# iwbn/flow-supervisor

Measured on AMD Instinct MI355X. Metric: image-pairs/s fwd+bwd, 12 GRU iters, 436x1024, higher is better.
Workload: dtype f32 (bf16x3 products); 1 GPU; RAFT full, 440x1024 (Sintel 436x1024 padded), 12 GRU iters, 4 pairs/GPU, train step = fwd + sequence loss + bwd + RCCL all-reduce + clip + AdamW; global_batch=4, parallelism=dp1, launch=hipGraph replay of the whole step

## Files before the change

flow_supervisor_amd/_lib.py:

```python
import ctypes
import functools
import os
from ctypes import POINTER, Structure, c_double, c_float, c_int, c_int64, c_void_p

import torch

_HERE = os.path.dirname(os.path.abspath(__file__))
LIB_PATH = os.environ.get("FSRAFT_LIB_PATH") or os.path.join(_HERE, "libfsraft.so")
_lib = None

c_float_p = c_void_p


class ConvDesc(Structure):
    _fields_ = [
        ("src", c_void_p * 3), ("srcC", c_int * 3), ("srcld", c_int * 3), ("nsrc", c_int),
        ("wpk", c_void_p), ("bias", c_void_p), ("wpk_split", c_void_p),
        ("B", c_int), ("H", c_int), ("W", c_int), ("KH", c_int), ("KW", c_int), ("N", c_int),
        ("dst", c_void_p * 3), ("dst_bs", c_int64 * 3), ("dst_ps", c_int64 * 3), ("dst_cs", c_int64 * 3),
        ("dst_n0", c_int * 3), ("dst_acc", c_int * 3), ("ndst", c_int),
        ("relu", c_int), ("alpha", c_float),
        ("epi", c_int),
        ("h", c_void_p), ("ldh", c_int), ("z", c_void_p), ("ldz", c_int),
        ("aux1", c_void_p), ("ld1", c_int), ("aux2", c_void_p), ("ld2", c_int), ("hid", c_int),
        ("pre", c_void_p), ("ldpre", c_int),
        ("rmask", c_void_p * 3), ("ldmask", c_int * 3), ("maskc", c_int * 3),
        ("wpk_frag", c_void_p), ("pad_h1", c_int), ("pad_w1", c_int),
        ("ws", c_void_p), ("ws_floats", c_int64),
    ]


class PackJob(Structure):
    _fields_ = [
        ("w", c_void_p * 3), ("rows", c_int * 3), ("npiece", c_int),
        ("wpk", c_void_p),
        ("cin_full", c_int), ("kh", c_int), ("kw", c_int),
        ("srcC", c_int * 3), ("srcOff", c_int * 3), ("nsrc", c_int),
        ("mode", c_int), ("flags", c_int),
        ("scale", c_float), ("accumulate", c_int),
    ]


_PP = POINTER(c_void_p)
_IP = POINTER(c_int)
_S = c_void_p

SIGNATURES = {
    "fsraft_corr_build": [c_void_p, c_void_p, _PP, c_int, c_int, c_int, c_int, c_int, _S],
    "fsraft_corr_unpool_bwd": [_PP, c_int, c_int, c_int, c_int, _S],
    "fsraft_corr_lookup_fwd": [_PP, c_int, c_void_p, c_int64, c_int64, c_int64, c_void_p, c_int, c_int, c_int, c_int, c_int, _S],
    "fsraft_corr_lookup_bwd": [_PP, c_int, c_void_p, c_int64, c_int64, c_int64, c_void_p, c_int, c_int, c_int, c_int, c_int, _S],
    "fsraft_altcorr_fwd": [c_void_p, c_void_p, c_void_p, c_void_p, c_int, c_int, c_int, c_int, c_int, c_int, c_int, c_int, _S],
    "fsraft_altcorr_bwd": [c_void_p, c_void_p, c_void_p, c_void_p, c_void_p, c_void_p, c_int, c_int, c_int, c_int, c_int, c_int, c_int, c_int, _S],
    "fsraft_upsample_fwd": [c_void_p, c_int64, c_int64, c_int64, c_void_p, c_void_p, c_int, c_int, c_int, _S],
    "fsraft_upsample_bwd": [c_void_p, c_int64, c_int64, c_int64, c_void_p, c_void_p, c_void_p, c_void_p, c_void_p, c_int, c_int, c_int, _S],
    "fsraft_upflow8_fwd": [c_void_p, c_void_p, c_int, c_int, c_int, c_int, _S],
    "fsraft_upflow8_bwd": [c_void_p, c_void_p, c_int, c_int, c_int, c_int, _S],
    "fsraft_conv_ktot": [_IP, c_int, c_int, c_int],
    "fsraft_conv_forward": [POINTER(ConvDesc), _S],
    "fsraft_conv_forward_stats": [POINTER(ConvDesc), c_void_p, c_void_p, c_int, POINTER(c_int), _S],
    "fsraft_conv_wgrad": [c_void_p, c_int, c_int, _PP, _IP, _IP, c_int, c_void_p, c_void_p, c_int, c_int, c_int, c_int, c_int, _S],
    "fsraft_conv_wgrad_multi": [_PP, c_int, c_int, c_int, _PP, _IP, _IP, c_int, c_void_p, c_void_p, c_int, c_int, c_int, c_int, c_int, _S],
    "fsraft_conv_small_fwd": [c_void_p, c_int, c_int, c_void_p, c_void_p, c_void_p, c_int64, c_int64, c_int64, c_int, c_int, c_int, c_int, c_int, c_int, _S],
    "fsraft_conv_small_wgrad": [_PP, _PP, c_int, c_int, c_int, c_int, c_void_p, c_void_p, c_int, c_int, c_int, c_int, c_int, c_int, _S],
    "fsraft_conv_small_dgrad": [c_void_p, c_int, c_void_p, c_void_p, c_int, c_void_p, c_int, c_int, c_int, c_int, c_int, c_int, c_int, c_int, _S],
    "fsraft_pack_conv_weights": [POINTER(PackJob), c_int, _S],
    "fsraft_pack_conv_weight": [c_void_p, c_void_p, c_int, c_int, c_int, c_int, _IP, c_int, c_int, c_int, _S],
    "fsraft_set_rec_mfma16": [c_int],
    "fsraft_set_build_kernel": [c_int],
    "fsraft_set_dvol_policy": [c_int],
    "fsraft_set_dvol_box": [c_int],
    "fsraft_set_ktile_exact": [c_int],
    "fsraft_set_lookup_policy": [c_int],
    "fsraft_set_upsample_kernel": [c_int],
    "fsraft_conv_workspace": [c_void_p, c_int64],
    "fsraft_set_arithmetic": [c_int],
    "fsraft_get_arithmetic": [],
    "fsraft_set_tuning": [c_int, c_int],
    "fsraft_adamw_flat": [c_void_p, c_void_p, c_void_p, c_void_p, c_int64, c_void_p, c_void_p, c_float, c_void_p, c_double, c_double, c_float,
                          c_float, c_void_p, c_void_p, _S],
    "fsraft_stream_capture_id": [_S, c_void_p],
    "fsraft_stem_slots": [],
    "fsraft_stem7x7s2_fwd": [c_void_p, c_void_p, c_void_p, c_void_p, c_int, c_int, c_int, c_int, _S],
    "fsraft_stem7x7s2_wgrad": [c_void_p, c_void_p, c_void_p, c_void_p, c_int, c_int, c_int, c_int, _S],
    "fsraft_set_lookup_qb": [c_int],
    "fsraft_set_build_split": [c_int],
    "fsraft_set_gemm_split": [c_int],
    "fsraft_gemm_tn_split": [c_void_p, c_int64, c_int64, c_void_p, c_int64, c_int64, c_void_p, c_int64, c_int64, c_int, c_int, c_int, c_int, c_float, c_int, _S],
    "fsraft_gemm_f32": [c_void_p, c_int64, c_int64, c_void_p, c_int64, c_int64, c_void_p, c_int64, c_int64, c_int, c_int, c_int, c_int, c_int, c_float, c_int, _S],
    "fsraft_nchw_to_nhwc": [c_void_p, c_void_p, c_int, c_int, c_int, c_int, c_int, c_int, _S],
    "fsraft_nhwc_to_nchw": [c_void_p, c_void_p, c_int, c_int, c_int, c_int, c_int, c_int, _S],
    "fsraft_im2col7": [c_void_p, c_int64, c_int64, c_int64, c_void_p, c_int, c_int, c_int, c_int, _S],
    "fsraft_col2im7": [c_void_p, c_int, c_void_p, c_int, c_int, c_int, c_int, _S],
    "fsraft_flow_to_nhwc": [c_void_p, c_int64, c_int64, c_int64, c_void_p, c_int, c_int, c_int, c_int, _S],
    "fsraft_nhwc_to_flow": [c_void_p, c_int, c_int, c_void_p, c_int, c_int, c_int, _S],
    "fsraft_relu_bwd": [c_void_p, c_int, c_void_p, c_int, c_int64, c_int, _S],
    "fsraft_gru_bwd1": [c_void_p, c_void_p, c_void_p, c_void_p, c_void_p, c_void_p, c_int, c_void_p, c_void_p, c_void_p, c_void_p, c_int64, c_int, _S],
    "fsraft_gru_bwd2": [c_void_p, c_void_p, c_void_p, c_void_p, c_int, c_void_p, c_void_p, c_int64, c_int, _S],
    "fsraft_col_sum": [c_void_p, c_int, c_int64, c_int, c_void_p, c_float, _S],
    "fsraft_softmax_rows": [c_void_p, c_int64, c_int, _S],
    "fsraft_softmax_rows_bwd": [c_void_p, c_void_p, c_int64, c_int, _S],
    "fsraft_softmax_rows_rec": [c_void_p, c_int64, c_int, _S],
    "fsraft_softmax_rows_bwd_rec": [c_void_p, c_void_p, c_int64, c_int, _S],
    "fsraft_softmax_rows_pos": [c_void_p, c_void_p, c_int64, c_int64, c_int, c_int, c_int, c_int, c_int, _S],
    "fsraft_softmax_rows_pos_bwd": [c_void_p, c_void_p, c_void_p, c_int64, c_int64, c_int, c_int, c_int, c_int, _S],
    "fsraft_gma_mix_fwd": [c_void_p, c_int, c_void_p, c_int, c_void_p, c_void_p, c_int, c_int64, c_int, _S],
    "fsraft_gma_mix_bwd": [c_void_p, c_int, c_void_p, c_int, c_void_p, c_void_p, c_int, c_void_p, c_int, c_void_p, c_int64, c_int, _S],
    "fsraft_inorm_relu_fwd": [c_void_p, c_void_p, c_void_p, c_int64, c_int, c_float, c_int, _S],
    "fsraft_inorm_relu_bwd": [c_void_p, c_void_p, c_void_p, c_void_p, c_int64, c_int, c_int, _S],
    "fsraft_affine_relu_fwd": [c_void_p, c_void_p, c_void_p, c_void_p, c_int64, c_int, c_int, c_int, _S],
    "fsraft_affine_relu_bwd": [c_void_p, c_void_p, c_void_p, c_void_p, c_void_p, c_void_p, c_void_p, c_int64, c_int, c_int, c_int, _S],
    "fsraft_sequence_loss": [_PP, _PP, POINTER(c_float), c_int, c_int, c_void_p, c_void_p, c_float, c_float, c_int, c_int, c_int, c_void_p, _S],
    "fsraft_corr_pool_pyramid": [_PP, c_int, c_int64, c_int, c_int, _S],
    "fsraft_corr_pool_pyramid_same": [_PP, c_int, c_int64, c_int, c_int, _S],
    "fsraft_corr_lookup_fwd_same": [_PP, c_int, c_void_p, c_int64, c_int64, c_int64, c_void_p, c_int, c_int, c_int, c_int, c_int, _S],
    "fsraft_corr_unpool_same_bwd": [_PP, c_int, c_int64, c_int, c_int, _S],
    "fsraft_corr_lookup_bwd_same": [_PP, c_int, c_void_p, c_int64, c_int64, c_int64, c_void_p, c_int, c_int, c_int, c_int, c_int, _S],
    "fsraft_corr_lookup_dcoords_same": [_PP, c_int, c_void_p, c_int64, c_int64, c_int64, c_void_p, c_int, c_void_p, c_int64, c_int64, c_int64,
                                        c_int, c_int, c_int, c_int, _S],
    "fsraft_set_norm_blocks": [c_int],
    "fsraft_get_tuning": [c_int],
    "fsraft_conv_last_route": [c_int],
    "fsraft_set_wgrad_wide": [c_int],
    "fsraft_conv_wgrad_last_tile": [],
    "fsraft_space_to_depth2": [c_void_p, c_void_p, c_int, c_int, c_int, c_int, c_int, _S],
    "fsraft_forward_interpolate": [c_void_p, c_void_p, c_int, c_int, _S],
    "fsraft_flow_metrics_scratch_bytes": [c_int, c_int, c_int],
    "fsraft_flow_metrics": [c_void_p, c_int64, c_int64, c_int64, c_void_p, c_int64, c_int64, c_int64, c_void_p, c_int64, c_int64,
                            c_int, c_int, c_int, c_void_p, c_void_p, c_void_p, c_int64, _S],
    "fsraft_range_map_scratch_bytes": [c_int, c_int, c_int],
    "fsraft_range_map": [c_void_p, c_int64, c_int64, c_int64, c_int, c_int, c_int, c_int, c_void_p, c_void_p, c_int64, _S],
    "fsraft_census_scratch_bytes": [c_int, c_int, c_int],
    "fsraft_census_fwd": [c_void_p, c_int64, c_int64, c_int64, c_int, c_void_p, c_int64, c_int64, c_int64, c_int, c_int, _IP,
                          c_void_p, c_int64, c_int64, c_int64, c_void_p, c_int64, c_int64, c_int, c_int, c_int,
                          c_void_p, c_void_p, c_void_p, c_void_p, c_int64, _S],
    "fsraft_census_bwd": [c_void_p, c_int64, c_int64, c_int64, c_int, c_void_p, c_int64, c_int64, c_int64, c_int, c_int, _IP,
                          c_void_p, c_int64, c_int64, c_int64, c_void_p, c_void_p, c_void_p, c_void_p, c_int, c_int, c_int,
                          c_void_p, _S],
    "fsraft_smoothness_scratch_bytes": [c_int, c_int, c_int],
    "fsraft_smoothness": [c_void_p, c_int64, c_int64, c_int64, c_int, c_int, _IP, c_void_p, c_int64, c_int64, c_int64,
                          c_int, c_int, c_int, c_int, c_float, c_int, c_void_p, c_void_p, c_void_p, c_int64, _S],
    "fsraft_inorm_relu_cl_fwd": [c_void_p, c_void_p, c_void_p, c_void_p, c_void_p, c_void_p, c_int, c_int, c_int, c_float, c_int, c_int, c_int, _S],
    "fsraft_inorm_relu_cl_bwd": [c_void_p, c_void_p, c_void_p, c_void_p, c_void_p, c_void_p, c_void_p, c_void_p, c_int, c_int, c_int,
                                 c_int, c_int, _S],
    "fsraft_affine_relu_cl_fwd": [c_void_p, c_void_p, c_void_p, c_void_p, c_void_p, c_int64, c_int, c_int, c_int, c_int, _S],
    "fsraft_affine_relu_cl_bwd": [c_void_p, c_void_p, c_void_p, c_void_p, c_void_p, c_void_p, c_void_p, c_void_p, c_void_p, c_int, c_int,
                                  c_int, c_int, c_int, _S],
    "fsraft_axpby": [c_void_p, c_void_p, c_float, c_float, c_int64, _S],
    "fsraft_sum_n": [_PP, c_int, c_void_p, c_int64, c_int, _S],
    "fsraft_bn_fold": [c_void_p, c_void_p, c_void_p, c_void_p, c_void_p, c_float, c_int, c_void_p, c_void_p, c_void_p, c_void_p, _S],
    "fsraft_bn_fold_bwd": [c_void_p, c_int, c_int, c_void_p, c_void_p, c_void_p, c_void_p, c_void_p, c_void_p, _S],
    "fsraft_vol_layout": [c_int, c_int, c_int, _IP],
    "fsraft_corr_build_tiled": [c_void_p, c_void_p, c_void_p, c_int, c_int, c_int, c_int, c_int, _S],
    "fsraft_corr_build_rec": [c_void_p, c_void_p, c_void_p, c_int, c_int, c_int, c_int, c_int, _S],
    "fsraft_corr_lookup_tiled_fwd": [c_void_p, c_int, c_void_p, c_int64, c_int64, c_int64, c_void_p, c_int, c_int, c_int, c_int, c_int, _S],
    "fsraft_corr_lookup_tiled_dcoords": [c_void_p, c_int, c_void_p, c_int64, c_int64, c_int64, c_void_p, c_void_p, c_int64, c_int64, c_int64,
                                         c_int, c_int, c_int, c_int, c_int, _S],
    "fsraft_corr_lookup_dcoords": [_PP, c_int, c_void_p, c_int64, c_int64, c_int64, c_void_p, c_int, c_void_p, c_int64, c_int64, c_int64,
                                   c_int, c_int, c_int, c_int, _S],
    "fsraft_corr_dvol_build": [_PP, _PP, POINTER(c_int64), c_int, c_void_p, c_int, c_int, c_int, c_int, c_int, c_int, c_int, c_int, c_int64,
                               c_int64, c_void_p, c_void_p, _S],
    "fsraft_set_alt_tile": [c_int],
    "fsraft_altcorr_fused_fwd": [c_void_p, _PP, c_int, c_void_p, c_int64, c_int64, c_int64, c_int, c_void_p, c_int, c_int, c_int, c_int, c_int, _S],
    "fsraft_altcorr_fused_dcoords": [c_void_p, _PP, c_int, c_void_p, c_int64, c_int64, c_int64, c_int, c_void_p, c_void_p, c_int64, c_int64,
                                     c_int64, c_int, c_int, c_int, c_int, c_int, _S],
    "fsraft_altcorr_mfma_fwd": [c_void_p, _PP, c_void_p, _PP, c_int, c_void_p, c_int64, c_int64, c_int64, c_int, c_void_p, c_int, c_int, c_int, c_int, c_int, _S],
    "fsraft_corr_f2cat": [c_void_p, c_void_p, c_int, c_int, c_int, c_int, c_int, _S],
    "fsraft_corr_dfmap2": [c_void_p, c_void_p, c_int, c_int, c_int, c_int, c_int, _S],
    "fsraft_corr_f2cat_rec": [c_void_p, c_void_p, c_int, c_int, c_int, c_int, c_int, _S],
    "fsraft_to_records": [c_void_p, c_int64, c_void_p, c_int64, c_int64, c_int, _S],
    "fsraft_gemm_rec_tn": [c_void_p, c_int64, c_int64, c_void_p, c_int64, c_int64, c_void_p, c_int64, c_int64, c_int, c_int, c_int, c_int,
                           c_float, c_int, c_int, _S],
    "fsraft_gemm_rec_nt": [c_void_p, c_int64, c_int64, c_void_p, c_int64, c_int64, c_void_p, c_int64, c_int64, c_int, c_int, c_int, c_int,
                           c_float, c_int, c_int, _S],
    "fsraft_gemm_rec_nt_list": [c_void_p, c_int64, c_int64, c_void_p, c_int64, c_int64, c_void_p, c_int64, c_int64, c_int, c_int, c_int, c_int,
                                c_float, c_int, c_int, c_void_p, c_void_p, c_int, c_int, _S],
    "fsraft_gemm_rec_tn_list": [c_void_p, c_int64, c_int64, c_void_p, c_int64, c_int64, c_void_p, c_int64, c_int64, c_int, c_int, c_int, c_int,
# ... 119 lines not shown
```

flow_supervisor_amd/core/extractor.py:

```python
import torch
import torch.nn as nn
import torch.nn.functional as F

from .. import ops
from .._lib import on_tensor_device


class _InstNormRelu(torch.autograd.Function):

    @staticmethod
    def forward(ctx, x, eps, relu):
        from .. import _lib as L
        x = x.contiguous()
        N, C, H, W = x.shape
        y = torch.empty_like(x)
        stats = torch.empty(N * C, 2, device=x.device, dtype=torch.float32)
        L.check(L.load().fsraft_inorm_relu_fwd(L.ptr(x), L.ptr(y), L.ptr(stats), N * C, H * W, float(eps), int(relu),
                                               L.stream()), "inorm_relu_fwd")
        ctx.save_for_backward(x, stats)
        ctx.relu = relu
        return y

    @staticmethod
    def backward(ctx, g):
# ... 181 lines not shown

def _conv_key(conv):
    from .. import ops
    w = conv.weight
    return (w.data_ptr(), w._version, ops.exact_mode())


def _queue_conv_packs(plan, conv):
    from .. import ops
    wd = conv.weight.detach()
    N, C, KH, KW = wd.shape
    exact = ops.exact_mode()
    fs = plan.pack([wd], [C], 10)
    f = plan.pack([wd], [C], 0) if (exact or N <= 32) else fs
    ds = plan.pack([wd], [C], 11)
    d = plan.pack([wd], [C], 1) if (exact or C <= 32) else ds
    ff = plan.pack([wd], [C], 10, frag=True) if (KH, KW) == (3, 3) and 32 < C <= 64 else None
    df = plan.pack([wd], [C], 11, frag=True) if (KH, KW) == (3, 3) and 32 < N <= 64 else None
    return (f, fs, d, ds, ff, df)


def _prepare_packs(root):
    from .. import ops
    todo = []
    for m in root.modules():
        if isinstance(m, _Block) and _pair_shape_ok(m):
            w3, wsc = m.conv1.weight, m.downsample[0].weight
            key = (w3.data_ptr(), w3._version, wsc.data_ptr(), wsc._version, ops.exact_mode())
            c = m.__dict__.get("_fs_pair_packs")
            if (c is None or c[0] != key) and w3.is_cuda and w3.dtype == torch.float32:
                todo.append(("pair", m, key))
        if (isinstance(m, nn.Conv2d) and m.stride == (1, 1) and m.kernel_size in ((1, 1), (3, 3)) and m.groups == 1
                and m.weight.is_cuda and m.weight.dtype == torch.float32):
            c = m.__dict__.get("_fs_packs")
            key = _conv_key(m)
            if c is None or c[0] != key:
                todo.append(("conv", m, key))
    if not todo:
        return
    with torch.no_grad():
        plan = ops.PackPlan(todo[0][1].conv1.weight.device if todo[0][0] == "pair" else todo[0][1].weight.device)
        hs = []
        exact = ops.exact_mode()
        for kind, m, key in todo:
            if kind == "conv":
                hs.append(_queue_conv_packs(plan, m))
                continue
            w3, ws = m.conv1.weight.detach(), m.downsample[0].weight.detach()
            N, C = w3.shape[:2]
            a = plan.pack([w3], [4 * C], 10, cin_full=C, s2d=True)
            b = plan.pack([w3], [4 * C], 11, cin_full=C, s2d=True)
            a0 = plan.pack([w3], [4 * C], 0, cin_full=C, s2d=True) if (exact or N <= 32) else a
            b0 = plan.pack([w3], [4 * C], 1, cin_full=C, s2d=True) if (exact or 4 * C <= 32) else b
            Ns, Cs = ws.shape[:2]
            c_ = plan.pack([ws], [Cs], 10)
            d_ = plan.pack([ws], [Cs], 11)
            c0 = plan.pack([ws], [Cs], 0) if (exact or Ns <= 32) else c_
            d0 = plan.pack([ws], [Cs], 1) if (exact or Cs <= 32) else d_
            hs.append(((a0, a, b0, b), (c0, c_, d0, d_)))
        out = plan.run()
        for (kind, m, key), h in zip(todo, hs):
            if kind == "conv":
                m.__dict__["_fs_packs"] = (key,) + tuple(None if i is None else out[i] for i in h)
            else:
                m.__dict__["_fs_pair_packs"] = (key, tuple(out[i] for i in h[0]), tuple(out[i] for i in h[1]))


def _weight_packs(conv):
    c = conv.__dict__.get("_fs_packs")
    if c is None or c[0] != _conv_key(conv):
        _prepare_packs(conv)
        c = conv.__dict__["_fs_packs"]
    return c


class _ConvCL(torch.autograd.Function):

    @staticmethod
    def forward(ctx, x, weight, bias, packs, link=None, sums=None):
        from .. import ops
        ctx.link = link if _is_cl(x) else None
        if ctx.link is not None:
            ctx.link.armed = True
        x = _as_cl(x)
        B, C, H, W = x.shape
        N, _, KH, KW = weight.shape
        out = torch.empty(B, H, W, N, device=x.device, dtype=torch.float32)
        acc = ops.zeros(2, B * 8, N, device=x.device) if (sums is not None and bias is None and STATS_IN_EPILOGUE) else None
        carried = ops.conv_forward([ops.V(x.permute(0, 2, 3, 1), C)], packs[1], bias, B, H, W, KH, KW, N, [ops.Dst.nhwc(out)],
                                   wpk_split=packs[2], wpk_frag=packs[5], stats=acc)
        if sums is not None:
            sums.acc = acc if carried else None
        ctx.save_for_backward(x, weight)
        ctx.packs = packs
        ctx.has_bias = bias is not None
        return out.permute(0, 3, 1, 2)

    @staticmethod
    def backward(ctx, g):
        from .. import ops
        x, weight = ctx.saved_tensors
        B, C, H, W = x.shape
        N, _, KH, KW = weight.shape
        g = _as_cl(g)
        gv = ops.V(g.permute(0, 2, 3, 1), N)
        dx = dw = db = None
        if ctx.needs_input_grad[0]:
            dres = ctx.link.dres if ctx.link is not None else None
            if dres is not None and dres.shape == x.shape and _is_cl(dres) and dres.dtype == torch.float32:
                ctx.link.dres = None
                ops.conv_forward([gv], ctx.packs[3], None, B, H, W, KH, KW, C, [ops.Dst.nhwc(dres.permute(0, 2, 3, 1), acc=True)],
                                 wpk_split=ctx.packs[4], wpk_frag=ctx.packs[6])
                dx = dres
            else:
                if dres is not None:
                    ctx.link.dres = None
                dxb = torch.empty(B, H, W, C, device=x.device, dtype=torch.float32)
                ops.conv_forward([gv], ctx.packs[3], None, B, H, W, KH, KW, C, [ops.Dst.nhwc(dxb)], wpk_split=ctx.packs[4],
# ... 68 lines not shown
    for ky, (ty, sy) in enumerate(_S2D_TAP):
        for kx, (tx, sx) in enumerate(_S2D_TAP):
            w[:, sy, sx, :, ty, tx] = w3[:, :, ky, kx]
    return w.reshape(N, 4 * C, 2, 2)


def _s2d_weight_grad(dw, C):
    N = dw.shape[0]
    d = dw.reshape(N, 2, 2, C, 2, 2)
    out = dw.new_empty(N, C, 3, 3)
    for ky, (ty, sy) in enumerate(_S2D_TAP):
        for kx, (tx, sx) in enumerate(_S2D_TAP):
            out[:, :, ky, kx] = d[:, sy, sx, :, ty, tx]
    return out


def _pair_shape_ok(block):
    c1 = getattr(block, "conv1", None)
    ds = block.downsample[0] if getattr(block, "downsample", None) is not None else None
    return (block.n == 2 and c1 is not None and ds is not None and c1.kernel_size == (3, 3) and c1.stride == (2, 2)
            and c1.padding == (1, 1) and c1.dilation == (1, 1) and c1.groups == 1 and ds.kernel_size == (1, 1)
            and ds.stride == (2, 2) and ds.padding == (0, 0) and ds.groups == 1)


def _pair_packs(block):
    from .. import ops
    w3, wsc = block.conv1.weight, block.downsample[0].weight
    key = (w3.data_ptr(), w3._version, wsc.data_ptr(), wsc._version, ops.exact_mode())
    c = block.__dict__.get("_fs_pair_packs")
    if c is None or c[0] != key:
        _prepare_packs(block)
        c = block.__dict__["_fs_pair_packs"]
    return c


class _StridedPairFn(torch.autograd.Function):

    @staticmethod
    def forward(ctx, x, w3, wsc, packs, pre=False):
        from .. import ops
        x = _as_cl(x)
        ctx.pre = pre
        if pre:
            B, C4, h, w = x.shape
            C, H, W = C4 // 4, 2 * h, 2 * w
            xs = x.permute(0, 2, 3, 1)
        else:
            B, C, H, W = x.shape
            h, w = H // 2, W // 2
            xs = ops.space_to_depth2(x.permute(0, 2, 3, 1))
        N, Ns = w3.shape[0], wsc.shape[0]
        y1 = torch.empty(B, h, w, N, device=x.device, dtype=torch.float32)
        ys = torch.empty(B, h, w, Ns, device=x.device, dtype=torch.float32)
        p, q = packs[1], packs[2]
        ops.conv_forward([ops.V(xs, 4 * C)], p[0], None, B, h, w, 2, 2, N, [ops.Dst.nhwc(y1)], wpk_split=p[1])
        ops.conv_forward([ops.V(xs, C, 0)], q[0], None, B, h, w, 1, 1, Ns, [ops.Dst.nhwc(ys)], wpk_split=q[1])
        ctx.save_for_backward(xs, w3, wsc)
        ctx.packs = packs
        return y1.permute(0, 3, 1, 2), ys.permute(0, 3, 1, 2)

    @staticmethod
    def backward(ctx, g1, gs):
        from .. import ops
        xs, w3, wsc = ctx.saved_tensors
        B, h, w, C4 = xs.shape
        C, N, Ns = C4 // 4, w3.shape[0], wsc.shape[0]
        p, q = ctx.packs[1], ctx.packs[2]
        g1v = ops.V(_as_cl(g1).permute(0, 2, 3, 1), N)
        gsv = ops.V(_as_cl(gs).permute(0, 2, 3, 1), Ns)
        dx = dw3 = dwsc = None
        if ctx.needs_input_grad[0]:
            dxs = torch.empty(B, h, w, C4, device=xs.device, dtype=torch.float32)
            ops.conv_forward([g1v], p[2], None, B, h, w, 2, 2, C4, [ops.Dst.nhwc(dxs)], wpk_split=p[3], pad=(0, 0))
            ops.conv_forward([gsv], q[2], None, B, h, w, 1, 1, C, [ops.Dst.nhwc(dxs, 0, 0, True)], wpk_split=q[3])
            dx = (dxs if ctx.pre else ops.space_to_depth2(dxs, inverse=True)).permute(0, 3, 1, 2)
        items = []
        if ctx.needs_input_grad[1]:
            dwpk = ops.zeros(N, ops.conv_ktot([C4], 2, 2), device=xs.device)
            ops.conv_wgrad(g1v, [ops.V(xs, C4)], dwpk, B, h, w, 2, 2)
            dw3 = torch.empty(N, C, 3, 3, device=xs.device, dtype=torch.float32)
            items.append((dwpk, [dw3], [C4], [0], C, 2, 2, 1.0, True))
        if ctx.needs_input_grad[2]:
            dwpk = ops.zeros(Ns, ops.conv_ktot([C], 1, 1), device=xs.device)
            ops.conv_wgrad(gsv, [ops.V(xs, C, 0)], dwpk, B, h, w, 1, 1)
            dwsc = torch.empty(Ns, C, 1, 1, device=xs.device, dtype=torch.float32)
            items.append((dwpk, [dwsc], [C], [0], C, 1, 1, 1.0, False))
        ops.unpack_weight_grads(items, xs.device)
        return dx, dw3, dwsc, None, None


def _norm_act(norm, y, cbias, relu, res=None):
    if isinstance(norm, nn.InstanceNorm2d):
        return _InstNormReluCL.apply(y, norm.eps, relu, res)
    return _FrozenBNReluCL.apply(y, cbias, norm.weight, norm.bias, norm.running_mean, norm.running_var, norm.eps, relu, res)


def _pair_ok_shape(block, C, H, W):
    import os
    return (S2D_UNITS and _pair_shape_ok(block) and H % 2 == 0
            and W % 2 == 0 and C % 4 == 0 and _cl_norm_ok(torch.empty(0, block.conv1.out_channels)))


def _pair_ok(block, x):
    return _pair_ok_shape(block, x.shape[1], x.shape[2], x.shape[3])


S2D_EMIT = True


class _S2D:
    __slots__ = ("t",)

    def __init__(self, t):
        self.t = t


def _conv_norm(conv, norm, x, relu, to_cl=False, res=None, link=None, res_link=None, s2d=False):
    fused = x.is_cuda and x.dtype == torch.float32 and not torch.is_autocast_enabled()
    if isinstance(norm, nn.InstanceNorm2d) and not norm.affine and not norm.track_running_stats:
        if fused:
            sums = _NormSums() if (to_cl or _is_cl(x)) else None
            y = _conv(conv, x, None, link, stem_cl=to_cl, sums=sums)
            if (to_cl or _is_cl(x)) and _cl_norm_ok(y):
                return _InstNormReluCL.apply(y, norm.eps, relu, res, res_link, sums, s2d)
            assert not s2d
            y = _InstNormRelu.apply(y, norm.eps, relu)
            return y if res is None else F.relu(res + y)
        y = F.conv2d(x, conv.weight, None, conv.stride, conv.padding, conv.dilation, conv.groups) if conv.bias is not None else conv(x)
        y = norm(y)
    elif isinstance(norm, nn.BatchNorm2d) and not norm.training and norm.track_running_stats and norm.affine and fused:
        y = _conv(conv, x, None, link, stem_cl=to_cl)
        if (to_cl or _is_cl(x)) and _cl_norm_ok(y):
            return _FrozenBNReluCL.apply(y, conv.bias, norm.weight, norm.bias, norm.running_mean, norm.running_var, norm.eps, relu, res,
                                         res_link, s2d)
# ... 162 lines not shown
```

flow_supervisor_amd/csrc/conv_common.hpp:

```cpp
#pragma once
#include "gemm_core.hpp"
#include "gemm_core_split.hpp"
#include "gemm_rec.hpp"
#include <cstddef>
#include <type_traits>

struct ConvKnobs {
  int conv_tile = 0;
  int wgrad_tile = 0;
  int wgrad_blocks = 512;
  int conv_split = 1;
  int wgrad_split = 2;
  int conv_buf = 1;
  int xcd_swizzle = 0;
  int wgrad_buf = 1;
  int conv_n256 = 0;
  int wgrad_multi = 1;
  int wgrad_blocks_multi = 2048;
  int conv_uniform = 1;
  int conv_w8 = 1;
  int conv_w8_min = 64;
  int wgrad_w8 = 0;
  int wgrad_pack = 1;
  int wgrad_blocks_pack = 1024;
  int conv_n64 = 1;
  int conv_n64_min_m = 65536;
  int conv_halo = 1;
  int conv_halo_min_m = 65536;
  int wgrad_xcd = 1;
  int conv_patch = 1;
  int wgrad_patch = 1;
  int conv_patch64 = 1;
  int wgrad_patch1 = 8192;
  int conv_patch_min_m = 8192;
  int conv_ksplit = -1;
};
__attribute__((visibility("hidden"))) extern ConvKnobs knob;
__attribute__((visibility("hidden"))) extern __thread int t_route[2];

namespace {
struct Src { const float* p; int C; int ld; };
struct Dst { float* p; int64_t bs, ps, cs; int n0; int accumulate; };

struct ConvArgs {
  Src src[3]; int nsrc;
  const float* wpk; int Ktot;
  const float* bias;
  int B, H, W, KH, KW, N;
  int PH, PW;
  Dst dst[3]; int ndst;
  int relu; float alpha;
  const float* h; int ldh;
  const float* z; int ldz;
  float* aux1; int ld1;
  float* aux2; int ld2;
  int hid;
  const float* pre; int ldpre;
  const float* rmask[3]; int ldmask[3]; int maskc[3];
  float* st_sum; float* st_sq; int st_slots;
  int swz;
  int ksplit;
};

constexpr int KTAB_MAX = 512;
struct ConvArgsT {
  ConvArgs a;
  const float* ubase; int uld;
  unsigned ktab[KTAB_MAX];
};

enum { EPI_PLAIN = 0, EPI_ZR = 2, EPI_Q = 3 };

#define FS_RSRC_FLAGS 0x00020000
#define FS_OOB 0x80000000u

__device__ __forceinline__ unsigned uni(unsigned v) { return __builtin_amdgcn_readfirstlane(v); }
template <class T>
__device__ __forceinline__ const T* uni_ptr(const T* p) {
  const uint64_t u = reinterpret_cast<uint64_t>(p);
  return reinterpret_cast<const T*>((uint64_t)uni((unsigned)(u >> 32)) << 32 | uni((unsigned)u));
}
__device__ __forceinline__ __amdgpu_buffer_rsrc_t make_rsrc(const void* p, unsigned bytes) {
  const uint64_t u = reinterpret_cast<uint64_t>(p);
  const unsigned lo = __builtin_amdgcn_readfirstlane((unsigned)u), hi = __builtin_amdgcn_readfirstlane((unsigned)(u >> 32));
  void* q = reinterpret_cast<void*>((uint64_t)hi << 32 | lo);
  return __builtin_amdgcn_make_buffer_rsrc(q, 0, __builtin_amdgcn_readfirstlane(bytes), FS_RSRC_FLAGS);
}

using SWCfg128 = SplitTnCfg<128, 128, 2, 2, 2>;
using SWCfg128S = SplitTnCfg<128, 128, 2, 2, 1>;
using SWCfg128W8 = SplitTnCfg<128, 128, 2, 4, 1, 512>;
using SWCfgPack = SplitTnCfg<64, 192, 2, 2, 1>;
using SWCfgW256 = SplitTnCfg<256, 256, 2, 4, 2, 512>;
using SWCfgW128 = SplitTnCfg<128, 256, 2, 4, 2, 512>;
using Cfg128 = GemmCfg<128, 128, 32, 2, 2, 2, 2>;
using Cfg64 = GemmCfg<128, 64, 32, 4, 1, 2, 2>;
using CfgM64 = GemmCfg<64, 128, 32, 1, 4, 2, 2>;
using Cfg6464 = GemmCfg<64, 64, 32, 2, 2, 2, 2>;
using WCfg6464 = GemmCfg<64, 64, 32, 2, 2, 0, 0>;
using Cfg6464K16 = GemmCfg<64, 64, 16, 2, 2, 2, 2>;
using CfgM64K16 = GemmCfg<64, 128, 16, 1, 4, 2, 2>;

using SCfg128 = SplitCfg<128, 128, 2, 2>;
using SCfgN256 = SplitCfg<64, 256, 1, 4, 2, true>;
using SCfg256W16 = SplitCfg<256, 128, 4, 4, 2, true, 1024>;
using SCfg128W8 = SplitCfg<128, 128, 2, 4, 2, true, 512>;
using SCfg256N64 = SplitCfg<256, 64, 4, 2, 2, true, 512>;
using SCfgM64 = SplitCfg<64, 128, 1, 4, 2, true>;
using Cfg32 = GemmCfg<128, 32, 32, 4, 1, 2, 2>;
using WCfg128 = GemmCfg<128, 128, 32, 2, 2, 0, 0>;
using WCfg32 = GemmCfg<32, 128, 32, 1, 4, 0, 0>;

template <class Cfg>
constexpr int route_gemm() {
  return std::is_same_v<Cfg, Cfg32> ? 1 : std::is_same_v<Cfg, Cfg64> ? 2 : std::is_same_v<Cfg, CfgM64> ? 3 :
         std::is_same_v<Cfg, Cfg128> ? 4 : std::is_same_v<Cfg, Cfg6464> ? 5 : std::is_same_v<Cfg, Cfg6464K16> ? 6 :
         std::is_same_v<Cfg, CfgM64K16> ? 7 : 0;
}
template <class Cfg>
constexpr int route_split() {
  return std::is_same_v<Cfg, SCfgN256> ? 30 : std::is_same_v<Cfg, SCfg256N64> ? 31 : std::is_same_v<Cfg, SCfg256W16> ? 32 :
         std::is_same_v<Cfg, SCfg128W8> ? 33 : std::is_same_v<Cfg, SCfgM64> ? 34 : std::is_same_v<Cfg, SCfg128> ? 35 : 0;
}

int conv_ktot(const int* C, int nsrc, int taps) {
  int k = 0;
  for (int s = 0; s < nsrc; ++s) k += taps * (((C[s] + 31) / 32) * 32);
  return k;
}

template <class F>
void with_epi(int epi, F&& f) {
  if (epi == EPI_PLAIN) f(std::integral_constant<int, EPI_PLAIN>{});
  else if (epi == EPI_ZR) f(std::integral_constant<int, EPI_ZR>{});
  else f(std::integral_constant<int, EPI_Q>{});
}

bool fill_srcs(Src (&dst)[3], const float* const* p, const int* C, const int* ld, int nsrc) {
  for (int s = 0; s < 3; ++s) {
    dst[s] = Src{s < nsrc ? p[s] : p[0], s < nsrc ? C[s] : 0, s < nsrc ? ld[s] : 4};
    if (s < nsrc && (!p[s] || ld[s] % 4 != 0)) return false;
  }
  return true;
}

int64_t wgrad_chunk(int target, int64_t tiles, int64_t M, int words) {
  int64_t want = (target + tiles - 1) / tiles;
  if (want < 1) want = 1;
  int64_t chunk = (M + want - 1) / want;
  if (chunk < 256) chunk = 256;
  if (chunk > 32 * (words - 2)) chunk = 32 * (words - 2);
  return (chunk + 31) / 32 * 32;
}

}
```

flow_supervisor_amd/csrc/conv_igemm.hip:

```cpp
#include "conv_common.hpp"

namespace {

__device__ __forceinline__ void tile_of_block(int swz, int& bx, int& by) {
  if (!swz) return;
  const int nx = gridDim.x, T = nx * gridDim.y, i = by * nx + bx;
  const int x = i & 7, q = T >> 3, r = T & 7;
  const int t = x * q + (x < r ? x : r) + (i >> 3);
  bx = t % nx; by = t / nx;
}

template <class Cfg>
struct ConvALoader {
  static constexpr int BM = Cfg::BM, BK = Cfg::BK, LD = Cfg::LDA;
  static constexpr int F4 = BK / 4;
  static constexpr int NF4 = BM * F4 / 256;
  static constexpr int NREG = NF4 * 4;
  static constexpr int NCH = NF4;
  const float* p0; const float* p1; const float* p2;
  int C0, C1, C2, ld0, ld1, ld2;
  int cpt0, cpt1, cpt2;
  int taps, KW, PH, PW, H, W;
  int py[NF4], px[NF4];
  int64_t pb[NF4];
// ... 446 lines not shown
#pragma unroll
  for (int i = 0; i < Cfg::TM; ++i)
#pragma unroll
    for (int j = 0; j < Cfg::TN; ++j)
#pragma unroll
      for (int r = 0; r < 16; ++r) acc[i][j][r] = 0.f;
  gemm_mainloop<Cfg>(lds, a.Ktot / Cfg::BK, la, lb, acc);
  conv_epilogue<Cfg, EPI>(a, acc, m0, n0);
}

template <class Cfg, int EPI, int BUF = 0>
__global__ __launch_bounds__(Cfg::NT) void conv_igemm_split_kernel(const std::conditional_t<BUF != 0, ConvArgsT, ConvArgs> args) {
  static_assert(Cfg::NT == 256 || BUF != 0, "wider workgroups use the buffer-addressed loaders");
  __shared__ __attribute__((aligned(16))) char lds[Cfg::LDS_ALLOC];
  const ConvArgs& a = [&]() -> const ConvArgs& { if constexpr (BUF != 0) return args.a; else return args; }();
  const int HW = a.H * a.W;
  const int M = a.B * HW;
  int bx = blockIdx.x, by = blockIdx.y;
  tile_of_block(a.swz, bx, by);
  const int n0 = bx * Cfg::BN, m0 = by * Cfg::BM;
  f32x16 acc[Cfg::TM][Cfg::TN];
#pragma unroll
  for (int i = 0; i < Cfg::TM; ++i)
#pragma unroll
    for (int j = 0; j < Cfg::TN; ++j)
#pragma unroll
      for (int r = 0; r < 16; ++r) acc[i][j][r] = 0.f;
  if constexpr (BUF != 0) {
    const int PH = a.PH, PW = a.PW, taps = a.KH * a.KW;
    const auto* ktab = (const unsigned __attribute__((address_space(4)))*)(
        (const char __attribute__((address_space(4)))*)__builtin_amdgcn_kernarg_segment_ptr() + offsetof(ConvArgsT, ktab));
    int kt0 = 0, KTs = a.Ktot / 32;
    if (a.ksplit > 1) {
      const int per = (KTs + a.ksplit - 1) / a.ksplit;
      kt0 = (int)blockIdx.z * per;
      KTs = min(per, KTs - kt0);
      ktab += kt0 * (BUF >= 2 ? 2 : 1);
    }
    unsigned tapmask[Cfg::NCH_A], pofs[Cfg::NCH_A];
#pragma unroll
    for (int j = 0; j < Cfg::NCH_A; ++j) {
      const int m = m0 + ((threadIdx.x + Cfg::NT * j) >> 3);
      unsigned mask = 0;
      if (m < M) {
        const int pix = m % HW, y = pix / a.W, x = pix % a.W;
        for (int t = 0; t < taps; ++t) {
          const int yy = y + t / a.KW - PH, xx = x + t % a.KW - PW;
          if ((unsigned)yy < (unsigned)a.H && (unsigned)xx < (unsigned)a.W) mask |= 1u << t;
        }
      }
      tapmask[j] = mask; pofs[j] = m < M ? m : 0;
    }
    BufWeightLoader<Cfg> lb;
    lb.base = uni_ptr(reinterpret_cast<const char*>(a.wpk) + (int64_t)n0 * a.Ktot * 4 + (int64_t)kt0 * 128);
    lb.nbytes = 0x7fffffffu;
#pragma unroll
    for (int j = 0; j < BufWeightLoader<Cfg>::NCH; ++j) {
      const int e = threadIdx.x + Cfg::NT * j;
      lb.voff[j] = (e >> 3) < a.N - n0 ? (unsigned)((e >> 3) * a.Ktot * 4 + (e & 7) * 16) : FS_OOB;
    }
    if constexpr (BUF >= 2) {
      BufConvALoaderU<Cfg> la;
      la.base = uni_ptr(args.ubase); la.ktab = ktab; la.kq16 = (threadIdx.x & 7) * 16;
      const unsigned ldb = uni((unsigned)args.uld * 4u);
#pragma unroll
      for (int j = 0; j < Cfg::NCH_A; ++j) { la.tapmask[j] = tapmask[j]; la.voff0[j] = pofs[j] * ldb + la.kq16; }
      split_mainloop<Cfg, BufConvALoaderU<Cfg>, BufWeightLoader<Cfg>, true>(lds, KTs, la, lb, acc);
    } else {
      BufConvALoader<Cfg> la;
      la.ld0x4 = uni(a.src[0].ld * 4); la.ld1x4 = uni(a.src[1].ld * 4); la.ld2x4 = uni(a.src[2].ld * 4);
      la.b0 = uni_ptr(a.src[0].p - (int64_t)(PH * a.W + PW) * a.src[0].ld); la.nb0 = 0x7fffffffu;
      la.b1 = uni_ptr(a.src[1].p - (int64_t)(PH * a.W + PW) * a.src[1].ld); la.nb1 = 0x7fffffffu;
      la.b2 = uni_ptr(a.src[2].p - (int64_t)(PH * a.W + PW) * a.src[2].ld); la.nb2 = 0x7fffffffu;
      la.ktab = ktab;
      la.kq16 = (threadIdx.x & 7) * 16;
#pragma unroll
      for (int j = 0; j < Cfg::NCH_A; ++j) { la.tapmask[j] = tapmask[j]; la.pofs[j] = pofs[j]; }
      split_mainloop<Cfg, BufConvALoader<Cfg>, BufWeightLoader<Cfg>, true>(lds, KTs, la, lb, acc);
    }
    if constexpr (EPI == EPI_PLAIN && Cfg::LDS_ALLOC >= Cfg::BM * (Cfg::BN + 4) * 4) {
      if (a.ksplit > 1) {
        conv_epilogue_lds<Cfg, EPI_PLAIN>(a, acc, m0, n0, reinterpret_cast<float*>(lds), true, 0, 0, 0, (int64_t)blockIdx.z * M);
        return;
      }
    }
  } else {
  SplitConvALoader<Cfg> la;
  la.p0 = a.src[0].p; la.C0 = a.src[0].C; la.ld0 = a.src[0].ld; la.cpt0 = (a.src[0].C + 31) / 32;
  la.p1 = a.src[1].p; la.C1 = a.src[1].C; la.ld1 = a.src[1].ld; la.cpt1 = a.nsrc > 1 ? (a.src[1].C + 31) / 32 : 0;
  la.p2 = a.src[2].p; la.C2 = a.src[2].C; la.ld2 = a.src[2].ld; la.cpt2 = a.nsrc > 2 ? (a.src[2].C + 31) / 32 : 0;
  if (a.nsrc < 2) { la.p1 = a.src[0].p; la.C1 = 0; la.ld1 = 4; la.cpt1 = 1; }
  if (a.nsrc < 3) { la.p2 = a.src[0].p; la.C2 = 0; la.ld2 = 4; la.cpt2 = 1; }
  la.taps = a.KH * a.KW; la.KW = a.KW; la.PH = a.PH; la.PW = a.PW; la.H = a.H; la.W = a.W;
#pragma unroll
  for (int j = 0; j < SplitConvALoader<Cfg>::NCH; ++j) {
    const int m = m0 + ((threadIdx.x + 256 * j) >> 3);
    if (m < M) {
      const int pix = m % HW;
      la.py[j] = pix / a.W; la.px[j] = pix % a.W; la.pofs[j] = m;
    } else {
      la.py[j] = -(1 << 20); la.px[j] = 0; la.pofs[j] = 0;
    }
  }
  SplitWeightLoader<Cfg> lb{reinterpret_cast<const char*>(a.wpk) + (int64_t)n0 * a.Ktot * 4, (int64_t)a.Ktot * 4, a.N - n0};
  split_mainloop<Cfg>(lds, a.Ktot / 32, la, lb, acc);
  }
  if constexpr (Cfg::LDS_ALLOC >= Cfg::BM * (Cfg::BN + 4) * 4) {
    if (EPI != EPI_PLAIN || epilogue_rows_ok(a)) {
      conv_epilogue_lds<Cfg, EPI>(a, acc, m0, n0, reinterpret_cast<float*>(lds));
      return;
    }
  }
// ... 119 lines not shown
          const int px = x0 + (r & 3) + 8 * (r >> 2) + 4 * lh;
          const float v = (py < a.H && px < a.W) ? acc[mt][nt][r] : 0.f;
          s1 += v; s2 += v * v;
        }
      }
      s1 += __shfl_xor(s1, 32, 64); s2 += __shfl_xor(s2, 32, 64);
      const int col = wn * (32 * TN) + nt * 32 + l31;
      if (lh == 0) { red[(wm * 2 + 0) * (64 * TN) + col] = s1; red[(wm * 2 + 1) * (64 * TN) + col] = s2; }
    }
    __syncthreads();
    if ((int)threadIdx.x < 64 * TN && (int)threadIdx.x < a.N) {
      const int col = threadIdx.x;
      const int slot = (int)((blockIdx.y * gridDim.x + blockIdx.x) % (unsigned)a.st_slots);
      const int64_t o = ((int64_t)b * a.st_slots + slot) * a.N + col;
      atomicAdd(a.st_sum + o, red[col] + red[2 * (64 * TN) + col]);
      atomicAdd(a.st_sq + o, red[(64 * TN) + col] + red[3 * (64 * TN) + col]);
    }
  }
  float* outb = a.out + (int64_t)b * a.obs;
#pragma unroll
  for (int mt = 0; mt < 2; ++mt) {
    const int py = y0 + 2 * wm + mt;
    if (py >= a.H) continue;
#pragma unroll
    for (int nt = 0; nt < TN; ++nt) {
      const int n = wn * (32 * TN) + nt * 32 + l31;
      if (n >= a.N) continue;
      const float bv = a.bias ? a.bias[n] : 0.f;
      float old[16];
#pragma unroll
      for (int r = 0; r < 16; ++r) {
        const int px = x0 + (r & 3) + 8 * (r >> 2) + 4 * lh, pc = px < a.W ? px : a.W - 1;
        old[r] = a.acc ? outb[(int64_t)(py * a.W + pc) * a.ops + n] : 0.f;
      }
#pragma unroll
      for (int r = 0; r < 16; ++r) {
        const int px = x0 + (r & 3) + 8 * (r >> 2) + 4 * lh;
        if (px >= a.W) continue;
        float v = acc[mt][nt][r] + bv;
        if (a.relu) v = fmaxf(v, 0.f);
        outb[(int64_t)(py * a.W + px) * a.ops + n] = v + old[r];
      }
    }
  }
}

template <int CG, int TN>
int launch_halo(const HaloArgs& h, hipStream_t s) {
  dim3 grid(ceil_div(h.W, HALO_TW), ceil_div(h.H, HALO_TH), h.B);
  hipLaunchKernelGGL((conv3x3_halo_kernel<CG, TN>), grid, dim3(256), 0, s, h);
  return fs_launch_status();
}

bool build_ktab(const ConvArgs& a, ConvArgsT& t) {
  const int taps = a.KH * a.KW, KT = a.Ktot / 32;
  const int64_t M = (int64_t)a.B * a.H * a.W;
  if (KT > KTAB_MAX || taps > 15) return false;
  int kt = 0;
  for (int s = 0; s < a.nsrc; ++s) {
    const int C = a.src[s].C, ld = a.src[s].ld, cpt = (C + 31) / 32;
    if (M * ld * 4 >= (int64_t)FS_OOB) return false;
    for (int i = 0; i < taps * cpt; ++i, ++kt) {
        const int tap = i / cpt, c = i % cpt;
        const int64_t soff = ((int64_t)((tap / a.KW) * a.W + tap % a.KW) * ld + c * 32) * 4;
        if (soff % 16 != 0 || soff / 16 > 0xffff) return false;
        const int crem = C - c * 32 < 32 ? C - c * 32 : 32;
        t.ktab[kt] = (unsigned)(soff / 16) | (unsigned)tap << 16 | (unsigned)s << 20 | (unsigned)crem << 22;
      }
  }
  if (kt != KT) return false;
  t.a = a;
  return true;
}

bool build_ktab_uniform(const ConvArgs& a, ConvArgsT& t) {
  const int taps = a.KH * a.KW, KT = a.Ktot / 32, PH = a.PH, PW = a.PW;
  const int64_t M = (int64_t)a.B * a.H * a.W;
  if (!knob.conv_uniform || 2 * KT > KTAB_MAX || taps > 15) return false;
  const int ld = a.src[0].ld;
  const float* lo = a.src[0].p;
  for (int s = 0; s < a.nsrc; ++s) {
    if (a.src[s].ld != ld) return false;
    if (a.src[s].p < lo) lo = a.src[s].p;
  }
  const float* base = lo - (int64_t)(PH * a.W + PW) * ld;
  int kt = 0;
  for (int s = 0; s < a.nsrc; ++s) {
    const int C = a.src[s].C, cpt = (C + 31) / 32;
    const int64_t delta = (a.src[s].p - lo) * 4;
    for (int tap = 0; tap < taps; ++tap)
      for (int c = 0; c < cpt; ++c, ++kt) {
        const int64_t soff = delta + ((int64_t)((tap / a.KW) * a.W + tap % a.KW) * ld + c * 32) * 4;
        if (soff + M * ld * 4 + 256 >= (int64_t)FS_OOB) return false;
        const int crem = C - c * 32 < 32 ? C - c * 32 : 32;
        t.ktab[2 * kt] = (unsigned)soff;
        t.ktab[2 * kt + 1] = (unsigned)tap | (unsigned)crem << 4;
      }
  }
  if (kt != KT) return false;
  t.a = a; t.ubase = base; t.uld = ld;
  return true;
}


template <int EPI>
__global__ __launch_bounds__(256) void conv_finish_kernel(const ConvArgs a, const float* __restrict__ ws, int S, int ldw) {
  const int HW = a.H * a.W;
  const int64_t M = (int64_t)a.B * HW;
  const int C4 = (a.N + 3) / 4;
  for (int64_t e = (int64_t)blockIdx.x * 256 + threadIdx.x; e < M * C4; e += (int64_t)gridDim.x * 256) {
    const int64_t m = e / C4;
    const int n = (int)(e % C4) * 4;
    const int nv = a.N - n < 4 ? a.N - n : 4;
    f32x4 v = {0.f, 0.f, 0.f, 0.f};
    if (a.bias) {
#pragma unroll
      for (int i = 0; i < 4; ++i) v[i] = i < nv ? a.bias[n + i] : 0.f;
    }
    for (int s = 0; s < S; ++s) {
      const f32x4 p = gload4(ws + ((int64_t)s * M + m) * ldw + n);
#pragma unroll
      for (int i = 0; i < 4; ++i) v[i] += p[i];
    }
    if (EPI == EPI_PLAIN) {
      int di = 0;
      if (a.ndst > 1 && n >= a.dst[1].n0) di = 1;
      if (a.ndst > 2 && n >= a.dst[2].n0) di = 2;
      float* dp = di == 0 ? a.dst[0].p : di == 1 ? a.dst[1].p : a.dst[2].p;
      const int64_t dbs = di == 0 ? a.dst[0].bs : di == 1 ? a.dst[1].bs : a.dst[2].bs;
      const int64_t dps = di == 0 ? a.dst[0].ps : di == 1 ? a.dst[1].ps : a.dst[2].ps;
      const int64_t dcs = di == 0 ? a.dst[0].cs : di == 1 ? a.dst[1].cs : a.dst[2].cs;
      const int dn0 = di == 0 ? a.dst[0].n0 : di == 1 ? a.dst[1].n0 : a.dst[2].n0;
      const bool dacc = (di == 0 ? a.dst[0].accumulate : di == 1 ? a.dst[1].accumulate : a.dst[2].accumulate) != 0;
      const float* mk = di == 0 ? a.rmask[0] : di == 1 ? a.rmask[1] : a.rmask[2];
      const int ldm = di == 0 ? a.ldmask[0] : di == 1 ? a.ldmask[1] : a.ldmask[2];
      const int mkc = di == 0 ? a.maskc[0] : di == 1 ? a.maskc[1] : a.maskc[2];
      const int64_t b = m / HW, pix = m - b * HW;
      float* o = dp + b * dbs + pix * dps + (int64_t)(n - dn0) * dcs;
      for (int i = 0; i < nv; ++i) {
        float r = v[i] * a.alpha;
        if (a.relu) r = fmaxf(r, 0.f);
        if (dacc) r += o[i * dcs];
        if (mk && n - dn0 + i < mkc && mk[m * ldm + (n - dn0) + i] <= 0.f) r = 0.f;
        o[i * dcs] = r;
      }
    } else if (EPI == EPI_ZR) {
      const bool isz = n < a.hid;
      const int c = isz ? n : n - a.hid;
      if (a.pre) v += gload4(a.pre + m * a.ldpre + n);
#pragma unroll
      for (int i = 0; i < 4; ++i) v[i] = 1.0f / (1.0f + expf(-v[i]));
      if (isz) {
        *reinterpret_cast<f32x4*>(a.dst[0].p + m * a.dst[0].ps + c) = v;
// ... 37 lines not shown
  if (S > 1) {
    const int per = (KT + S - 1) / S;
    S = (KT + per - 1) / per;
  }
  return S < 2 ? 1 : S;
}

template <class Cfg>
int launch_conv_split(const ConvArgs& a, int epi, hipStream_t s) {
  const int M = a.B * a.H * a.W;
  dim3 grid(ceil_div(a.N, Cfg::BN), ceil_div(M, Cfg::BM));
  ConvArgsT t;
  const int swz = knob.xcd_swizzle || (grid.x >= 2 && (int64_t)grid.x * grid.y >= 2048);
  const bool buf = knob.conv_buf == 2 || (knob.conv_buf == 1 && Cfg::BM == 64) || Cfg::BN == 256 || Cfg::NT != 256;
  if constexpr (Cfg::LDS_ALLOC >= Cfg::BM * (Cfg::BN + 4) * 4) {
    const int ldw = (a.N + 3) / 4 * 4;
    const bool gru_ok = epi == EPI_PLAIN || (a.N % 4 == 0 && (!a.pre || a.ldpre % 4 == 0));
    const int S = (buf && g_conv_ws && gru_ok && (Cfg::BM == 64 || (Cfg::BM == 128 && Cfg::NT == 512) || knob.conv_ksplit >= 2)) ? pick_ksplit((int64_t)grid.x * grid.y, a.Ktot / 32, a.N, M, ldw, Cfg::BM) : 1;
    if (S > 1) {
      const bool uni_tab = build_ktab_uniform(a, t);
      if (uni_tab || build_ktab(a, t)) {
        ConvArgs& p = t.a;
        p.swz = 0;
        p.ksplit = S;
        p.dst[0] = Dst{g_conv_ws, (int64_t)a.H * a.W * ldw, ldw, 1, 0, 0};
        p.dst[1] = p.dst[2] = p.dst[0];
        p.ndst = 1; p.bias = nullptr; p.relu = 0; p.alpha = 1.0f;
        for (int i = 0; i < 3; ++i) p.rmask[i] = nullptr;
        dim3 g3(grid.x, grid.y, S);
        t_route[0] = route_split<Cfg>() + 100;
        if (uni_tab) hipLaunchKernelGGL((conv_igemm_split_kernel<Cfg, EPI_PLAIN, 2>), g3, dim3(Cfg::NT), 0, s, t);
        else hipLaunchKernelGGL((conv_igemm_split_kernel<Cfg, EPI_PLAIN, 1>), g3, dim3(Cfg::NT), 0, s, t);
        int rc = fs_launch_status();
        if (rc) return rc;
        const int64_t work = (int64_t)M * (ldw / 4);
        const int fb = (int)((work + 255) / 256 < 4096 ? (work + 255) / 256 : 4096);
        with_epi(epi, [&](auto e) { hipLaunchKernelGGL(conv_finish_kernel<decltype(e)::value>, dim3(fb), dim3(256), 0, s, a, g_conv_ws, S, ldw); });
        return fs_launch_status();
      }
    }
  }
  if (buf && build_ktab_uniform(a, t)) {
    t.a.swz = swz;
    t_route[0] = route_split<Cfg>();
    with_epi(epi, [&](auto e) { hipLaunchKernelGGL((conv_igemm_split_kernel<Cfg, decltype(e)::value, 2>), grid, dim3(Cfg::NT), 0, s, t); });
    return fs_launch_status();
  }
  if (buf && build_ktab(a, t)) {
    t.a.swz = swz;
    t_route[0] = route_split<Cfg>();
    with_epi(epi, [&](auto e) { hipLaunchKernelGGL((conv_igemm_split_kernel<Cfg, decltype(e)::value, 1>), grid, dim3(Cfg::NT), 0, s, t); });
    return fs_launch_status();
  }
  if constexpr (Cfg::NT != 256) {
    return -1;
  } else {
  t_route[0] = route_split<Cfg>();
  with_epi(epi, [&](auto e) { hipLaunchKernelGGL((conv_igemm_split_kernel<Cfg, decltype(e)::value>), grid, dim3(256), 0, s, a); });
  return fs_launch_status();
  }
}

template <class Cfg>
int launch_conv_split_plain(const ConvArgs& a, hipStream_t s) {
  const int M = a.B * a.H * a.W;
  dim3 grid(ceil_div(a.N, Cfg::BN), ceil_div(M, Cfg::BM));
  ConvArgsT t;
  if (build_ktab_uniform(a, t)) {
    t_route[0] = route_split<Cfg>();
    hipLaunchKernelGGL((conv_igemm_split_kernel<Cfg, EPI_PLAIN, 2>), grid, dim3(Cfg::NT), 0, s, t);
    return fs_launch_status();
  }
  if (build_ktab(a, t)) {
    t_route[0] = route_split<Cfg>();
    hipLaunchKernelGGL((conv_igemm_split_kernel<Cfg, EPI_PLAIN, 1>), grid, dim3(Cfg::NT), 0, s, t);
    return fs_launch_status();
  }
  return -1;
}

template <class Cfg>
int launch_conv(const ConvArgs& a, int epi, hipStream_t s) {
  const int M = a.B * a.H * a.W;
  dim3 grid(ceil_div(a.N, Cfg::BN), ceil_div(M, Cfg::BM));
  t_route[0] = route_gemm<Cfg>();
  with_epi(epi, [&](auto e) { hipLaunchKernelGGL((conv_igemm_kernel<Cfg, decltype(e)::value>), grid, dim3(256), 0, s, a); });
  return fs_launch_status();
}

#include "conv_patch.inc"

}

extern "C" int fsraft_conv_ktot(const int* srcC, int nsrc, int KH, int KW) {
  if (!srcC || nsrc < 1 || nsrc > 3) return -1;
  return conv_ktot(srcC, nsrc, KH * KW);
}

namespace {
struct StatReq { float* sum; float* sq; int slots; bool done; };
thread_local StatReq t_stat{nullptr, nullptr, 0, false};
template <class Args>
void attach_stats(Args& p, bool want) {
  if (want) { p.st_sum = t_stat.sum; p.st_sq = t_stat.sq; p.st_slots = t_stat.slots; }
}
}

extern "C" int fsraft_conv_forward(const fsraft_conv_desc* d, hipStream_t stream) {
  if (!d || d->nsrc < 1 || d->nsrc > 3 || d->ndst < 1 || d->ndst > 3 || !d->wpk || d->N < 1) return FS_ERR_ARG;
  const bool want_stats = t_stat.sum != nullptr && d->epi == EPI_PLAIN && d->ndst == 1 && !d->relu && d->alpha == 1.0f && !d->dst_acc[0] &&
                          !d->rmask[0] && !d->bias && d->dst_n0[0] == 0 && d->N % 4 == 0;
  if (d->ws && (((uintptr_t)d->ws & 15) || d->ws_floats < 0)) return FS_ERR_ARG;
  t_route[0] = 0;
  g_conv_ws = d->ws ? d->ws : t_reg_ws;
  g_conv_ws_floats = d->ws ? d->ws_floats : t_reg_ws_floats;
  ConvArgs a{};
  if (!fill_srcs(a.src, d->src, d->srcC, d->srcld, d->nsrc)) return FS_ERR_ARG;
  for (int s = 0; s < d->nsrc; ++s) if (d->srcC[s] < 1) return FS_ERR_ARG;
  a.nsrc = d->nsrc;
  a.wpk = d->wpk; a.Ktot = conv_ktot(d->srcC, d->nsrc, d->KH * d->KW); a.bias = d->bias;
  a.B = d->B; a.H = d->H; a.W = d->W; a.KH = d->KH; a.KW = d->KW; a.N = d->N;
  a.PH = d->pad_h1 ? d->pad_h1 - 1 : d->KH / 2; a.PW = d->pad_w1 ? d->pad_w1 - 1 : d->KW / 2;
  if (a.PH < 0 || a.PH >= d->KH || a.PW < 0 || a.PW >= d->KW) return FS_ERR_ARG;
  for (int i = 0; i < 3; ++i) {
    const int j = i < d->ndst ? i : 0;
    a.dst[i] = Dst{d->dst[j], d->dst_bs[j], d->dst_ps[j], d->dst_cs[j], d->dst_n0[j], d->dst_acc[j]};
    if (i < d->ndst && !d->dst[i]) return FS_ERR_ARG;
  }
  a.ndst = d->ndst; a.relu = d->relu; a.alpha = d->alpha;
  a.h = d->h; a.ldh = d->ldh; a.z = d->z; a.ldz = d->ldz; a.aux1 = d->aux1; a.ld1 = d->ld1; a.aux2 = d->aux2; a.ld2 = d->ld2;
  a.hid = d->hid;
  a.pre = d->epi == EPI_PLAIN ? nullptr : d->pre; a.ldpre = d->ldpre;
  if (a.pre && (d->ldpre % 4 != 0 || ((uintptr_t)d->pre & 15))) return FS_ERR_ARG;
  for (int i = 0; i < 3; ++i) {
    const bool on = d->epi == EPI_PLAIN && i < d->ndst && d->rmask[i] != nullptr;
    a.rmask[i] = on ? d->rmask[i] : nullptr; a.ldmask[i] = d->ldmask[i]; a.maskc[i] = d->maskc[i];
    if (on && (d->ldmask[i] % 4 != 0 || ((uintptr_t)d->rmask[i] & 15))) return FS_ERR_ARG;
  }
  a.swz = knob.xcd_swizzle;
  if (d->epi == EPI_ZR && (!d->h || !d->aux1 || !d->aux2 || d->hid * 2 != d->N)) return FS_ERR_ARG;
  if (d->epi == EPI_Q && (!d->h || !d->z || !d->aux1)) return FS_ERR_ARG;
  if (d->epi != EPI_PLAIN && d->epi != EPI_ZR && d->epi != EPI_Q) return FS_ERR_ARG;
  if (knob.conv_patch && knob.conv_patch64 && knob.conv_split == 1 && d->wpk_split && d->epi == EPI_PLAIN && d->KH == 3 && d->KW == 3 &&
      d->N > 32 && d->N <= 64 && (int64_t)d->B * d->H * d->W >= knob.conv_patch_min_m) {
    ConvArgs p = a;
    p.wpk = d->wpk_split;
    attach_stats(p, want_stats);
    const int rc = launch_conv_patch(p, d->epi, stream);
    if (rc >= 0) { t_stat.done = want_stats; return rc; }
  }
  if (knob.conv_halo && knob.conv_split == 1 && d->wpk_frag && d->epi == EPI_PLAIN && d->nsrc == 1 && d->KH == 3 && d->KW == 3 &&
      a.PH == 1 && a.PW == 1 &&
      d->srcC[0] % 4 == 0 && d->srcC[0] > 32 && d->srcC[0] <= 64 && d->N <= 128 && d->N > 32 && d->ndst == 1 &&
      d->dst_cs[0] == 1 && d->dst_n0[0] == 0 && !(d->dst_acc[0] && d->relu) && !a.rmask[0] && d->alpha == 1.0f &&
      (int64_t)d->B * d->H * d->W >= knob.conv_halo_min_m && (int64_t)d->H * d->W * d->srcld[0] * 4 < 0x7fffffff) {
    HaloArgs h{d->src[0], d->srcld[0], d->srcC[0], reinterpret_cast<const char*>(d->wpk_frag), d->bias,
               d->dst[0], d->dst_bs[0], d->dst_ps[0], d->N, d->B, d->H, d->W, d->relu, d->dst_acc[0], nullptr, nullptr, 0};
    attach_stats(h, want_stats);
    t_stat.done = want_stats;
    t_route[0] = d->N > 64 ? 21 : 20;
    return d->N > 64 ? launch_halo<2, 2>(h, stream) : launch_halo<2, 1>(h, stream);
  }
  if (d->N <= 32 && d->epi == EPI_PLAIN) return launch_conv<Cfg32>(a, d->epi, stream);
  if (d->N <= 64 && d->epi == EPI_PLAIN && !(knob.conv_split && d->wpk_split && knob.conv_buf)) return launch_conv<Cfg64>(a, d->epi, stream);
  const int M = d->B * d->H * d->W;
  if (knob.conv_split && d->wpk_split && d->N > 32) {
    a.wpk = d->wpk_split;
    const bool narrow = knob.conv_buf != 0 || (int64_t)ceil_div(d->N, 128) * ceil_div(M, 128) < 400;
    if (knob.conv_patch && knob.conv_split == 1 && d->KH * d->KW > 1 && d->N > 64 && M >= knob.conv_patch_min_m) {
      ConvArgs p = a;
      attach_stats(p, want_stats);
      const int rc = launch_conv_patch(p, d->epi, stream);
      if (rc >= 0) { t_stat.done = want_stats; return rc; }
    }
    if (knob.conv_split == 5 || (knob.conv_split == 1 && knob.conv_n256 && d->N >= 256 &&
                              ceil_div(d->N, 256) * 256 <= ceil_div(d->N, 128) * 128))
      return launch_conv_split<SCfgN256>(a, d->epi, stream);
    if (knob.conv_split == 1 && knob.conv_n64 && d->N <= 64 && d->epi == EPI_PLAIN && M >= knob.conv_n64_min_m) {
      const int rc = launch_conv_split_plain<SCfg256N64>(a, stream);
      if (rc >= 0) return rc;
    }
    if (knob.conv_split == 1 && ((knob.conv_w8 == 1 && d->N >= 192 && d->N <= 512 && M >= 16384) || knob.conv_w8 == 2) && d->N >= 192) {
      const int rc = launch_conv_split<SCfg256W16>(a, d->epi, stream);
      if (rc >= 0) return rc;
    }
    if (knob.conv_w8 && knob.conv_split == 1 && (int64_t)ceil_div(d->N, 128) * ceil_div(M, 128) >= knob.conv_w8_min) {
      const int rc = launch_conv_split<SCfg128W8>(a, d->epi, stream);
      if (rc >= 0) return rc;
    }
    if (knob.conv_split == 3) return launch_conv_split<SCfgM64>(a, d->epi, stream);
    if (knob.conv_split == 4) return launch_conv_split<SCfg128>(a, d->epi, stream);
    return narrow ? launch_conv_split<SCfgM64>(a, d->epi, stream) : launch_conv_split<SCfg128>(a, d->epi, stream);
  }
  if (knob.conv_tile == 3) return launch_conv<Cfg6464>(a, d->epi, stream);
  if (knob.conv_tile == 4) return launch_conv<Cfg6464K16>(a, d->epi, stream);
  if (knob.conv_tile == 5) return launch_conv<CfgM64K16>(a, d->epi, stream);
  if (knob.conv_tile == 2) return launch_conv<CfgM64>(a, d->epi, stream);
  if (knob.conv_tile == 1) return launch_conv<Cfg128>(a, d->epi, stream);
  if ((int64_t)ceil_div(d->N, 128) * ceil_div(M, 128) < 512) return launch_conv<CfgM64>(a, d->epi, stream);
  return launch_conv<Cfg128>(a, d->epi, stream);
}

extern "C" int fsraft_conv_forward_stats(const fsraft_conv_desc* d, float* sum, float* sq, int slots, int* done, hipStream_t stream) {
  if (!sum || !sq || slots < 1 || !done) return FS_ERR_ARG;
  t_stat = StatReq{sum, sq, slots, false};
  const int rc = fsraft_conv_forward(d, stream);
  *done = (rc == FS_OK && t_stat.done) ? 1 : 0;
  t_stat = StatReq{nullptr, nullptr, 0, false};
  return rc;
}


extern "C" int fsraft_conv_workspace(float* ws, int64_t floats) {
  if (ws && (((uintptr_t)ws & 15) || floats < 0)) return FS_ERR_ARG;
  t_reg_ws = ws;
  t_reg_ws_floats = ws ? floats : 0;
  return FS_OK;
}
```

flow_supervisor_amd/csrc/conv_pack.hip:

```cpp
#include "conv_common.hpp"

namespace {

struct PackArgs {
  float* w;
  float* wpk;
  int Cout, Cin, taps;
  int C[3]; int nsrc;
  int Ktot, rows;
  int mode, accumulate;
  int split;
};

__device__ __forceinline__ void store_packed(const PackArgs& a, int64_t e, float v) {
  if (!a.split) { a.wpk[e] = v; return; }
  const __bf16 h = (__bf16)v;
  const __bf16 l = (__bf16)(v - (float)h);
  __bf16* rec = reinterpret_cast<__bf16*>(a.wpk) + (e >> 5) * 64;
  rec[e & 31] = h;
  rec[32 + (e & 31)] = l;
}

__global__ __launch_bounds__(256) void pack_weight_kernel(PackArgs a) {
  const int64_t total = (int64_t)a.rows * a.Ktot;
// ... 31 lines not shown
struct PackJobs { fsraft_pack_job j[PACK_JOBS]; };

__device__ __forceinline__ float* pack_elem(const PackJob& j, int n, int s, int c, int t) {
  int p = 0;
  while (p + 1 < j.npiece && n >= j.rows[p]) { n -= j.rows[p]; ++p; }
  float* w = j.w[p];
  if (j.flags & 2) {
    const int C = j.cin_full;
    const int sp = c / C, c0 = c % C;
    const int ky = 2 * (t >> 1) + (sp >> 1) - 1, kx = 2 * (t & 1) + (sp & 1) - 1;
    if (ky < 0 || kx < 0) return nullptr;
    return w + ((int64_t)n * C + c0) * 9 + ky * 3 + kx;
  }
  return w + ((int64_t)n * j.cin_full + j.srcOff[s] + c) * (j.kh * j.kw) + t;
}

__device__ __forceinline__ void pack_store(const PackJob& j, int Ktot, int rows, int n, int k, float v) {
  const int64_t e = (int64_t)n * Ktot + k;
  if (j.mode < 10) { j.wpk[e] = v; return; }
  const __bf16 h = (__bf16)v;
  const __bf16 l = (__bf16)(v - (float)h);
  __bf16* out = reinterpret_cast<__bf16*>(j.wpk);
  if (!(j.flags & 1)) {
    __bf16* rec = out + (e >> 5) * 64;
    rec[e & 31] = h;
    rec[32 + (e & 31)] = l;
    return;
  }
  const int nb = (rows + 31) / 32, kt = k >> 5, q = k & 31;
  const int64_t base = (((int64_t)kt * nb + (n >> 5)) * 2) ;
  const int sidx = (q >> 4) & 1, kh2 = (q >> 3) & 1, dw = (q >> 1) & 3, half = q & 1;
  const int64_t dh = ((((base + 0) * 2 + sidx) * 2 + kh2) * 32 + (n & 31)) * 4 + dw;
  const int64_t dl = ((((base + 1) * 2 + sidx) * 2 + kh2) * 32 + (n & 31)) * 4 + dw;
  out[dh * 2 + half] = h;
  out[dl * 2 + half] = l;
}

__global__ __launch_bounds__(256) void pack_jobs_kernel(PackJobs tab) {
  const PackJob& j = tab.j[blockIdx.y];
  const int taps = j.kh * j.kw;
  int cout = 0;
  for (int p = 0; p < j.npiece; ++p) cout += j.rows[p];
  if (j.mode == 3) {
    for (int e = blockIdx.x * 256 + threadIdx.x; e < cout; e += gridDim.x * 256) {
      int n = e, p = 0;
      while (p + 1 < j.npiece && n >= j.rows[p]) { n -= j.rows[p]; ++p; }
      j.wpk[e] = j.w[p][n];
    }
    return;
  }
  int cin = 0;
  for (int s = 0; s < j.nsrc; ++s) cin += j.srcC[s];
  const int m = j.mode % 10;
  int Ktot, rows;
  if (m == 1) { Ktot = taps * ((cout + 31) / 32 * 32); rows = cin; }
  else { Ktot = 0; for (int s = 0; s < j.nsrc; ++s) Ktot += taps * ((j.srcC[s] + 31) / 32 * 32); rows = cout; }
  const int rows_out = (j.flags & 1) ? (rows + 31) / 32 * 32 : rows;
  const int64_t total = (int64_t)rows_out * Ktot;
  for (int64_t e = (int64_t)blockIdx.x * 256 + threadIdx.x; e < total; e += (int64_t)gridDim.x * 256) {
    const int n = (int)(e / Ktot);
    int k = (int)(e % Ktot);
    if (m == 1) {
      const int cpad = (cout + 31) / 32 * 32;
      const int tp = k / cpad, c = k % cpad;
      float v = 0.f;
      if (c < cout && n < rows) {
        int s = 0, cs = n;
        while (s + 1 < j.nsrc && cs >= j.srcC[s]) { cs -= j.srcC[s]; ++s; }
        const float* q = pack_elem(j, c, s, cs, taps - 1 - tp);
        if (q) v = *q;
      }
      pack_store(j, Ktot, rows, n, k, v);
    } else {
      const int k0 = k;
      int s = 0;
      for (; s < j.nsrc; ++s) {
        const int span = taps * ((j.srcC[s] + 31) / 32 * 32);
        if (k < span) break;
        k -= span;
      }
      const int cpad = (j.srcC[s] + 31) / 32 * 32;
      const int t = k / cpad, c = k % cpad;
      const bool ok = c < j.srcC[s] && n < rows;
      float* q = ok ? pack_elem(j, n, s, c, t) : nullptr;
      if (m == 0) pack_store(j, Ktot, rows, n, k0, q ? *q : 0.f);
      else if (q) *q = j.accumulate ? *q + j.scale * j.wpk[e] : j.scale * j.wpk[e];
    }
  }
}

}

extern "C" int fsraft_pack_conv_weights(const fsraft_pack_job* jobs, int njobs, hipStream_t stream) {
  if (njobs < 0 || (njobs && !jobs)) return FS_ERR_ARG;
  for (int i = 0; i < njobs; ++i) {
    const fsraft_pack_job& j = jobs[i];
    const int m = j.mode;
    if (!(m == 0 || m == 1 || m == 2 || m == 3 || m == 10 || m == 11) || !j.wpk || j.npiece < 1 || j.npiece > 3) return FS_ERR_ARG;
    for (int p = 0; p < j.npiece; ++p) if (!j.w[p] || j.rows[p] < 1) return FS_ERR_ARG;
    if (m == 3) continue;
    if (j.nsrc < 1 || j.nsrc > 3 || j.kh < 1 || j.kw < 1 || j.cin_full < 1) return FS_ERR_ARG;
    if ((j.flags & 1) && m < 10) return FS_ERR_ARG;
    if ((j.flags & 2) && (j.kh != 2 || j.kw != 2 || j.nsrc != 1 || j.srcC[0] != 4 * j.cin_full || j.srcOff[0] != 0)) return FS_ERR_ARG;
    if (!(j.flags & 2)) for (int s = 0; s < j.nsrc; ++s) if (j.srcC[s] < 1 || j.srcOff[s] < 0 || j.srcOff[s] + j.srcC[s] > j.cin_full) return FS_ERR_ARG;
  }
  for (int i0 = 0; i0 < njobs; i0 += PACK_JOBS) {
    PackJobs tab{};
    const int n = njobs - i0 < PACK_JOBS ? njobs - i0 : PACK_JOBS;
    int64_t most = 0;
    for (int i = 0; i < n; ++i) {
      tab.j[i] = jobs[i0 + i];
      const fsraft_pack_job& j = tab.j[i];
      int64_t cout = 0, cin = 0;
      for (int p = 0; p < j.npiece; ++p) cout += j.rows[p];
      for (int s = 0; s < j.nsrc; ++s) cin += (j.srcC[s] + 31) / 32 * 32;
      const int64_t tot = j.mode == 3 ? cout : ((cout + 31) / 32 * 32) * ((cin + 31) / 32 * 32) * j.kh * j.kw;
      most = tot > most ? tot : most;
    }
    int blocks = (int)((most + 1023) / 1024);
    blocks = blocks < 1 ? 1 : (blocks > 512 ? 512 : blocks);
    hipLaunchKernelGGL(pack_jobs_kernel, dim3(blocks, n), dim3(256), 0, stream, tab);
  }
  return fs_launch_status();
}

extern "C" int fsraft_pack_conv_weight(float* w_oihw, float* wpk, int Cout, int Cin, int KH, int KW, const int* srcC,
                                       int nsrc, int mode, int accumulate, hipStream_t stream) {
  if (!w_oihw || !wpk || mode < 0 || (mode > 2 && mode != 10 && mode != 11)) return FS_ERR_ARG;
  PackArgs a{};
  a.split = mode >= 10;
  if (mode >= 10) mode -= 10;
  if (a.split && mode > 1) return FS_ERR_ARG;
  a.w = w_oihw; a.wpk = wpk; a.Cout = Cout; a.Cin = Cin; a.taps = KH * KW; a.mode = mode; a.accumulate = accumulate;
  if (mode == 1) {
    a.nsrc = 1; a.C[0] = Cout; a.C[1] = a.C[2] = 0;
    a.Ktot = a.taps * (((Cout + 31) / 32) * 32);
    a.rows = Cin;
  } else {
    if (!srcC || nsrc < 1 || nsrc > 3) return FS_ERR_ARG;
    int tot = 0;
    for (int s = 0; s < 3; ++s) { a.C[s] = s < nsrc ? srcC[s] : 0; tot += a.C[s]; }
    if (tot != Cin) return FS_ERR_ARG;
    a.nsrc = nsrc;
    a.Ktot = conv_ktot(srcC, nsrc, a.taps);
    a.rows = Cout;
  }
  const int64_t total = (int64_t)a.rows * a.Ktot;
  int blocks = (int)((total + 255) / 256 < 4096 ? (total + 255) / 256 : 4096);
  hipLaunchKernelGGL(pack_weight_kernel, dim3(blocks), dim3(256), 0, stream, a);
  return fs_launch_status();
}
```

flow_supervisor_amd/csrc/conv_tuning.hip:

```cpp
#include "conv_common.hpp"
#include <climits>

ConvKnobs knob;
__thread int t_route[2] = {0, 0};

namespace {
const struct { int key; int ConvKnobs::*member; } KNOB_TABLE[] = {
    {FSRAFT_KEY_CONV_TILE, &ConvKnobs::conv_tile},
    {FSRAFT_KEY_WGRAD_TILE, &ConvKnobs::wgrad_tile},
    {FSRAFT_KEY_WGRAD_BLOCKS, &ConvKnobs::wgrad_blocks},
    {FSRAFT_KEY_CONV_ARITH, &ConvKnobs::conv_split},
    {FSRAFT_KEY_WGRAD_ARITH, &ConvKnobs::wgrad_split},
    {FSRAFT_KEY_CONV_BUF, &ConvKnobs::conv_buf},
    {FSRAFT_KEY_XCD_SWIZZLE, &ConvKnobs::xcd_swizzle},
    {FSRAFT_KEY_WGRAD_BUF, &ConvKnobs::wgrad_buf},
    {FSRAFT_KEY_CONV_N256, &ConvKnobs::conv_n256},
    {FSRAFT_KEY_WGRAD_MULTI, &ConvKnobs::wgrad_multi},
    {FSRAFT_KEY_WGRAD_BLOCKS_MULTI, &ConvKnobs::wgrad_blocks_multi},
    {FSRAFT_KEY_CONV_UNIFORM, &ConvKnobs::conv_uniform},
    {FSRAFT_KEY_CONV_W8, &ConvKnobs::conv_w8},
    {FSRAFT_KEY_CONV_W8_MIN, &ConvKnobs::conv_w8_min},
    {FSRAFT_KEY_WGRAD_W8, &ConvKnobs::wgrad_w8},
    {FSRAFT_KEY_WGRAD_PACK, &ConvKnobs::wgrad_pack},
    {FSRAFT_KEY_WGRAD_BLOCKS_PACK, &ConvKnobs::wgrad_blocks_pack},
    {FSRAFT_KEY_CONV_N64, &ConvKnobs::conv_n64},
    {FSRAFT_KEY_CONV_N64_MIN_M, &ConvKnobs::conv_n64_min_m},
    {FSRAFT_KEY_CONV_HALO, &ConvKnobs::conv_halo},
    {FSRAFT_KEY_CONV_HALO_MIN_M, &ConvKnobs::conv_halo_min_m},
    {FSRAFT_KEY_WGRAD_XCD, &ConvKnobs::wgrad_xcd},
    {FSRAFT_KEY_CONV_PATCH, &ConvKnobs::conv_patch},
    {FSRAFT_KEY_WGRAD_PATCH, &ConvKnobs::wgrad_patch},
    {FSRAFT_KEY_CONV_PATCH64, &ConvKnobs::conv_patch64},
    {FSRAFT_KEY_WGRAD_PATCH1, &ConvKnobs::wgrad_patch1},
    {FSRAFT_KEY_CONV_PATCH_MIN_M, &ConvKnobs::conv_patch_min_m},
    {FSRAFT_KEY_CONV_KSPLIT, &ConvKnobs::conv_ksplit},
};

int* knob_of(int key) {
  for (const auto& e : KNOB_TABLE)
    if (e.key == key) return &(knob.*e.member);
  return nullptr;
}
}

extern "C" int fsraft_set_tuning(int key, int value) {
  int* k = knob_of(key);
  if (!k) return FS_ERR_ARG;
  *k = value;
  return FS_OK;
}

extern "C" int fsraft_get_tuning(int key) {
  const int* k = knob_of(key);
  return k ? *k : INT_MIN;
}

extern "C" int fsraft_conv_last_route(int which) {
  return which == 0 || which == 1 ? t_route[which] : -1;
}

extern "C" int fsraft_set_arithmetic(int mode) {
  if (mode != 0 && mode != 1) return FS_ERR_ARG;
  knob.conv_split = mode ? 1 : 0;
  knob.wgrad_split = mode ? 2 : 0;
  fsraft_set_build_split(mode);
  fsraft_set_gemm_split(mode);
  return FS_OK;
}
extern "C" int fsraft_get_arithmetic(void) { return knob.conv_split != 0 ? 1 : 0; }
```

flow_supervisor_amd/csrc/conv_wgrad.hip:

```cpp
#include "conv_common.hpp"

namespace {

struct WgradArgs {
  const float* dy; int ldy; int Cout;
  Src src[3]; int nsrc;
  float* dwpk; int Ktot;
  int B, H, W, KH, KW;
  int kchunk;
  float* dbias;
  int xcd_xt, xcd_yt, xcd_groups;
  int bx0, by0;
};

constexpr int WGRAD_MAX_SEG = 16;
struct WgradArgsM {
  WgradArgs a;
  int nseg, zs;
  const float* dys[WGRAD_MAX_SEG];
  const float* srcs[3][WGRAD_MAX_SEG];
};

template <class Cfg>
struct ShiftedXLoader {
  static constexpr int BN = Cfg::BN, BK = Cfg::BK, LD = Cfg::LDB;
  static constexpr int F4 = BN / 4;
  static constexpr int NF4 = BK * F4 / 256;
  static constexpr int NREG = NF4 * 4;
  static constexpr int NCH = NF4;
  const float* p; int ld, cvalid;
  int dy, dx, H, W, HW; int64_t M; int64_t m_begin, m_end;
  __device__ __forceinline__ bool fetch_chunk(int kt, float (&r)[NREG], int j) const {
    const int e = threadIdx.x + 256 * j;
    const int k = e / F4, c4 = e % F4;
    const int64_t m = m_begin + (int64_t)kt * BK + k;
    const int64_t mm = m < m_end ? m : m_begin;
    const int64_t b = mm / HW; const int pix = (int)(mm % HW);
    const int yy = pix / W + dy, xx = pix % W + dx;
    const bool ok = m < m_end && c4 * 4 < cvalid && yy >= 0 && yy < H && xx >= 0 && xx < W;
    const f32x4 v = gload4(p + (ok ? (b * HW + (int64_t)yy * W + xx) * ld + c4 * 4 : 0));
    r[4 * j + 0] = v[0]; r[4 * j + 1] = v[1]; r[4 * j + 2] = v[2]; r[4 * j + 3] = v[3];
    return ok;
  }
  __device__ __forceinline__ void store_chunk(float* t, const float (&r)[NREG], int j, bool ok) const {
    const int e = threadIdx.x + 256 * j;
    const int k = e / F4, c4 = e % F4;
    f32x4 v = {r[4 * j + 0], r[4 * j + 1], r[4 * j + 2], r[4 * j + 3]};
    const f32x4 z = {0.f, 0.f, 0.f, 0.f};
    *reinterpret_cast<f32x4*>(t + k * LD + c4 * 4) = ok ? v : z;
  }
};

template <class Cfg>
struct DyLoader {
  static constexpr int BM = Cfg::BM, BK = Cfg::BK, LD = Cfg::LDA;
  static constexpr int F4 = BM / 4;
  static constexpr int NF4 = BK * F4 / 256;
  static constexpr int NREG = NF4 * 4;
  static_assert((BK * F4) % 256 == 0, "dy tile must divide over 256 threads");
  static constexpr int NCH = NF4;
  const float* p; int ld, cvalid; int64_t m_begin, m_end;
  __device__ __forceinline__ bool fetch_chunk(int kt, float (&r)[NREG], int j) const {
    const int e = threadIdx.x + 256 * j;
    const int k = e / F4, c4 = e % F4;
    const int64_t m = m_begin + (int64_t)kt * BK + k;
// ... 40 lines not shown
    const f32x4 v = gload4(ok ? p + (mm + dy * W + dx) * ld + c4 * 4 : g_fsraft_zero16);
    r[4 * j + 0] = v[0]; r[4 * j + 1] = v[1]; r[4 * j + 2] = v[2]; r[4 * j + 3] = v[3];
  }
};

constexpr int WGRAD_MASK_WORDS = 2048;
template <class Cfg>
struct BufDyLoader {
  static constexpr int NCH = Cfg::NCH_A, NREG = NCH * 4;
  const float* base; unsigned ld4; int npix;
  unsigned voff[NCH]; int krow[NCH];
  __device__ __forceinline__ void fetch_tile(int kt, float (&r)[NREG]) const {
    const int ku = __builtin_amdgcn_readfirstlane(kt);
    const __amdgpu_buffer_rsrc_t rs = make_rsrc(base, 0x7fffffffu);
    const unsigned soff = (unsigned)ku * 32u * ld4;
    const int left = npix - ku * 32;
#pragma unroll
    for (int j = 0; j < NCH; ++j) {
      const unsigned voffj = voff[j] | (krow[j] < left ? 0u : FS_OOB);
      const u32x4 v = __builtin_amdgcn_raw_buffer_load_b128(rs, voffj, soff, 0);
      const f32x4 f = __builtin_bit_cast(f32x4, v);
      r[4 * j + 0] = f[0]; r[4 * j + 1] = f[1]; r[4 * j + 2] = f[2]; r[4 * j + 3] = f[3];
    }
  }
};
template <class Cfg>
struct BufShiftedXLoader {
  static constexpr int NCH = Cfg::NCH_B, NREG = NCH * 4;
  const float* base; unsigned ld4; const unsigned* mask;
  unsigned voff[NCH]; int krow[NCH];
  __device__ __forceinline__ void fetch_tile(int kt, float (&r)[NREG]) const {
    const int ku = __builtin_amdgcn_readfirstlane(kt);
    const unsigned w = __builtin_amdgcn_readfirstlane(mask[ku]);
    const __amdgpu_buffer_rsrc_t rs = make_rsrc(base, 0x7fffffffu);
    const unsigned soff = (unsigned)ku * 32u * ld4;
#pragma unroll
    for (int j = 0; j < NCH; ++j) {
      const unsigned voffj = voff[j] | ((__builtin_amdgcn_ubfe(w, (unsigned)krow[j], 1u) ^ 1u) << 31);
      const u32x4 v = __builtin_amdgcn_raw_buffer_load_b128(rs, voffj, soff, 0);
      const f32x4 f = __builtin_bit_cast(f32x4, v);
      r[4 * j + 0] = f[0]; r[4 * j + 1] = f[1]; r[4 * j + 2] = f[2]; r[4 * j + 3] = f[3];
    }
  }
};


constexpr int WGRAD_WIDE_WORDS = 512;
template <class Cfg>
struct BufWideXLoader : BufShiftedXLoader<Cfg> {
  int e0;
  __device__ __forceinline__ int elem(int c) const { return e0 + 8 * (Cfg::BN / 4) * c; }
};

struct XGroup { int s, tap, ci0, kofs, cpad; };
template <int GW>
__device__ __forceinline__ XGroup wgrad_xgroup(const WgradArgs& a, int t, int taps) {
  int s = 0, kofs = 0;
  for (;; ++s) {
    const int ct = (a.src[s].C + GW - 1) / GW;
    if (t < taps * ct) break;
    t -= taps * ct;
    kofs += taps * ((a.src[s].C + 31) / 32) * 32;
  }
  const int C = s == 0 ? a.src[0].C : s == 1 ? a.src[1].C : a.src[2].C;
  const int ct = (C + GW - 1) / GW, cpad = ((C + 31) / 32) * 32;
  const int tap = t / ct, ci0 = (t % ct) * GW;
  return XGroup{s, tap, ci0, kofs + tap * cpad + ci0, cpad};
}

template <class Cfg, bool BUF = false, bool MULTI = false>
__global__ __launch_bounds__(Cfg::NT) void conv_wgrad_split_kernel(const std::conditional_t<MULTI, WgradArgsM, WgradArgs> args) {
  static_assert(Cfg::NT == 256 || BUF, "512-thread workgroups use the buffer-addressed loaders");
  constexpr bool WIDE = Cfg::BN == 256;
  static_assert(!WIDE || (BUF && Cfg::NT == 512), "the 256-column x tile is loaded by two halves of 256 threads");
  constexpr int GW = WIDE ? 128 : Cfg::BN;
  __shared__ __attribute__((aligned(16))) char lds[Cfg::LDS_BYTES];
  __shared__ unsigned pixmask[BUF ? (WIDE ? 2 * WGRAD_WIDE_WORDS : WGRAD_MASK_WORDS) : 1];
  const WgradArgs& a = [&]() -> const WgradArgs& { if constexpr (MULTI) return args.a; else return args; }();
  int bx = blockIdx.x, by = blockIdx.y, zblock = blockIdx.z, seg = 0;
  if (a.xcd_xt > 0) {
    const int span = 8 * a.xcd_xt, r = blockIdx.x / span, rem = blockIdx.x - r * span;
    const int g = r * 8 + (rem & 7);
    if (g >= a.xcd_groups) return;
    if (a.xcd_yt > 0) { bx = rem >> 3; by = g % a.xcd_yt; zblock = g / a.xcd_yt; }
    else { const int tile = rem >> 3, x0 = -a.xcd_yt; bx = tile % x0; by = tile / x0; zblock = g; }
  }
  if constexpr (MULTI) { seg = zblock / args.zs; zblock -= seg * args.zs; seg = __builtin_amdgcn_readfirstlane(seg); }
  bx += a.bx0; by += a.by0;
  const int HW = a.H * a.W;
  const int64_t M = (int64_t)a.B * HW;
  const int taps = a.KH * a.KW;
  const int wave = __builtin_amdgcn_readfirstlane((int)(threadIdx.x >> 6));
  const int xh = WIDE ? wave >> 2 : 0, oh = WIDE ? ((wave % Cfg::WN) * (Cfg::TN * 32)) >> 7 : 0;
  const XGroup gl = wgrad_xgroup<GW>(a, WIDE ? 2 * bx + xh : bx, taps);
  const XGroup go = WIDE ? wgrad_xgroup<GW>(a, 2 * bx + oh, taps) : gl;
  const int s = gl.s;
  Src sc = s == 0 ? a.src[0] : s == 1 ? a.src[1] : a.src[2];
  const float* dyp = a.dy;
  if constexpr (MULTI) {
    typedef const float* fptr;
    const auto* karg = (const char __attribute__((address_space(4)))*)__builtin_amdgcn_kernarg_segment_ptr();
    dyp = ((const fptr __attribute__((address_space(4)))*)(karg + offsetof(WgradArgsM, dys)))[seg];
    sc.p = ((const fptr __attribute__((address_space(4)))*)(karg + offsetof(WgradArgsM, srcs)))[s * WGRAD_MAX_SEG + seg];
  }
  const int tap = gl.tap, ci0 = gl.ci0;
  const int co0 = by * Cfg::BM;
  const int64_t mb = (int64_t)zblock * a.kchunk;
  const int64_t me = mb + a.kchunk < M ? mb + a.kchunk : M;
  if (mb >= M) return;
  const int coleft = ((a.Cout + 3) / 4) * 4 - co0;
  const int cleft = ((sc.C + 3) / 4) * 4 - ci0;
  const int dyy = tap / a.KW - a.KH / 2, dxx = tap % a.KW - a.KW / 2;
  const int KT = (int)((me - mb + 31) / 32);
  f32x16 acc[Cfg::TM][Cfg::TN];
#pragma unroll
  for (int i = 0; i < Cfg::TM; ++i)
#pragma unroll
    for (int j = 0; j < Cfg::TN; ++j)
#pragma unroll
      for (int r = 0; r < 16; ++r) acc[i][j][r] = 0.f;
  float colsum[4] = {0.f, 0.f, 0.f, 0.f};
  const bool want_bias = a.dbias != nullptr && bx == 0;
  if constexpr (BUF) {
    constexpr int MT = WIDE ? 256 : Cfg::NT;
    unsigned* pm = pixmask + xh * WGRAD_WIDE_WORDS;
    for (int i = threadIdx.x % MT; i < KT * 32; i += MT) {
      const int64_t m = mb + i;
      bool ok = m < me;
      if (ok) {
        const int pix = (int)(m % HW), yy = pix / a.W + dyy, xx = pix % a.W + dxx;
        ok = (unsigned)yy < (unsigned)a.H && (unsigned)xx < (unsigned)a.W;
      }
      const unsigned long long bal = __ballot(ok);
      if ((threadIdx.x & 63) == 0) { pm[i >> 5] = (unsigned)bal; pm[(i >> 5) + 1] = (unsigned)(bal >> 32); }
    }
    __syncthreads();
    BufDyLoader<Cfg> la;
    la.base = uni_ptr(dyp + co0 + mb * a.ldy); la.ld4 = uni((unsigned)a.ldy * 4u); la.npix = (int)(me - mb);
    const int cva = coleft < Cfg::BM ? coleft : Cfg::BM;
#pragma unroll
    for (int j = 0; j < BufDyLoader<Cfg>::NCH; ++j) {
      const int e = threadIdx.x + Cfg::NT * j, k = e / (Cfg::BM / 4), c4 = e % (Cfg::BM / 4);
      la.krow[j] = k; la.voff[j] = c4 * 4 < cva ? (unsigned)(k * a.ldy + c4 * 4) * 4u : FS_OOB;
    }
    std::conditional_t<WIDE, BufWideXLoader<Cfg>, BufShiftedXLoader<Cfg>> lb;
    lb.base = uni_ptr(sc.p + ci0 + (mb + dyy * a.W + dxx) * sc.ld); lb.ld4 = uni((unsigned)sc.ld * 4u); lb.mask = pm;
    const int cvb = cleft < GW ? cleft : GW;
    if constexpr (WIDE) {
      const int t8 = threadIdx.x & 255, c4 = t8 & 31;
#pragma unroll
      for (int j = 0; j < BufShiftedXLoader<Cfg>::NCH; ++j) {
        const int k = (t8 >> 5) + 8 * j;
        lb.krow[j] = k; lb.voff[j] = c4 * 4 < cvb ? (unsigned)(k * sc.ld + c4 * 4) * 4u : FS_OOB;
      }
      lb.e0 = (t8 >> 5) * (Cfg::BN / 4) + xh * 32 + c4;
    } else {
#pragma unroll
      for (int j = 0; j < BufShiftedXLoader<Cfg>::NCH; ++j) {
        const int e = threadIdx.x + Cfg::NT * j, k = e / (Cfg::BN / 4), c4 = e % (Cfg::BN / 4);
        lb.krow[j] = k; lb.voff[j] = c4 * 4 < cvb ? (unsigned)(k * sc.ld + c4 * 4) * 4u : FS_OOB;
      }
    }
    if (want_bias) split_mainloop_tn<Cfg, BufDyLoader<Cfg>, decltype(lb), true, WIDE>(lds, KT, la, lb, acc, colsum);
    else split_mainloop_tn<Cfg, BufDyLoader<Cfg>, decltype(lb), false, WIDE>(lds, KT, la, lb, acc);
  } else {
  SplitDyLoader<Cfg> la{dyp + co0, a.ldy, coleft < Cfg::BM ? coleft : Cfg::BM, mb, me};
  SplitShiftedXLoader<Cfg> lb{sc.p + ci0, sc.ld, cleft < Cfg::BN ? cleft : Cfg::BN, dyy, dxx, a.H, a.W, HW, mb, me};
  if (want_bias) split_mainloop_tn<Cfg, SplitDyLoader<Cfg>, SplitShiftedXLoader<Cfg>, true>(lds, KT, la, lb, acc, colsum);
  else split_mainloop_tn<Cfg>(lds, KT, la, lb, acc);
  }
  if (want_bias) {
    constexpr int Q = Cfg::BM / 4, G = Cfg::NT / Q;
    float* part = reinterpret_cast<float*>(lds);
    __syncthreads();
#pragma unroll
    for (int q = 0; q < 4; ++q) part[(threadIdx.x / Q) * Cfg::BM + 4 * (threadIdx.x % Q) + q] = colsum[q];
    __syncthreads();
    if (threadIdx.x < Cfg::BM) {
      float s = 0.f;
#pragma unroll
      for (int g = 0; g < G; ++g) s += part[g * Cfg::BM + threadIdx.x];
      if (co0 + threadIdx.x < a.Cout) atomicAdd(a.dbias + co0 + threadIdx.x, s);
    }
  }
#pragma unroll
  for (int nt = 0; nt < Cfg::TN; ++nt) {
    const int n = acc_col<Cfg>(nt) & (GW - 1);
    if (go.ci0 + n >= go.cpad) continue;
#pragma unroll
    for (int mt = 0; mt < Cfg::TM; ++mt)
#pragma unroll
      for (int r = 0; r < 16; ++r) {
        const int co = co0 + acc_row<Cfg>(mt, r);
        if (co < a.Cout) atomicAdd(a.dwpk + (int64_t)co * a.Ktot + go.kofs + n, acc[mt][nt][r]);
      }
  }
}

constexpr int WGRAD_PACK_WORDS = 256;
constexpr int WGRAD_PACK_SLOTS = 8;

template <class Cfg>
struct BufPackedXLoader {
  static constexpr int NCH = Cfg::NCH_B, NREG = NCH * 4;
  const float* base; unsigned ld4; const unsigned* mask;
  unsigned voff[NCH]; int krow[NCH]; int slot[NCH];
  __device__ __forceinline__ void fetch_tile(int kt, float (&r)[NREG]) const {
    const int ku = __builtin_amdgcn_readfirstlane(kt);
    const __amdgpu_buffer_rsrc_t rs = make_rsrc(base, 0x7fffffffu);
    const unsigned soff = (unsigned)ku * 32u * ld4;
#pragma unroll
    for (int j = 0; j < NCH; ++j) {
      const unsigned w = mask[ku * WGRAD_PACK_SLOTS + slot[j]];
      const unsigned voffj = voff[j] | ((__builtin_amdgcn_ubfe(w, (unsigned)krow[j], 1u) ^ 1u) << 31);
      const u32x4 v = __builtin_amdgcn_raw_buffer_load_b128(rs, voffj, soff, 0);
      const f32x4 f = __builtin_bit_cast(f32x4, v);
      r[4 * j + 0] = f[0]; r[4 * j + 1] = f[1]; r[4 * j + 2] = f[2]; r[4 * j + 3] = f[3];
    }
  }
};

template <class Cfg>
__global__ __launch_bounds__(Cfg::NT) void conv_wgrad_pack_kernel(const WgradArgs a) {
  __shared__ __attribute__((aligned(16))) char lds[Cfg::LDS_BYTES];
  __shared__ unsigned pixmask[WGRAD_PACK_WORDS * WGRAD_PACK_SLOTS];
  const int HW = a.H * a.W;
  const int64_t M = (int64_t)a.B * HW;
  const int taps = a.KH * a.KW;
  const Src sc = a.src[0];
  const int cpad = ((sc.C + 31) / 32) * 32;
  int TP = Cfg::BN / cpad;
  if (TP > WGRAD_PACK_SLOTS) TP = WGRAD_PACK_SLOTS;
  int bx = blockIdx.x, by = blockIdx.y, bz = blockIdx.z;
  if (a.xcd_xt > 0) {
    const int span = 8 * a.xcd_xt, r = blockIdx.x / span, rem = blockIdx.x - r * span;
    const int g = r * 8 + (rem & 7);
    if (g >= a.xcd_groups) return;
    bx = rem >> 3; by = g % a.xcd_yt; bz = g / a.xcd_yt;
  }
  const int tap0 = bx * TP;
  const int ntap = taps - tap0 < TP ? taps - tap0 : TP;
// ... 97 lines not shown
  const int tap = t / ct, ci0 = (t % ct) * Cfg::BN;
  const int cpad = ((sc.C + 31) / 32) * 32;
  kofs += tap * cpad + ci0;
  const int co0 = blockIdx.y * Cfg::BM;
  const int64_t mb = (int64_t)blockIdx.z * a.kchunk;
  const int64_t me = mb + a.kchunk < M ? mb + a.kchunk : M;
  if (mb >= M) return;

  const int coleft = ((a.Cout + 3) / 4) * 4 - co0;
  DyLoader<Cfg> la{a.dy + co0, a.ldy, coleft < Cfg::BM ? coleft : Cfg::BM, mb, me};
  const int cleft = ((sc.C + 3) / 4) * 4 - ci0;
  ShiftedXLoader<Cfg> lb{sc.p + ci0, sc.ld, cleft < Cfg::BN ? cleft : Cfg::BN,
                         tap / a.KW - a.KH / 2, tap % a.KW - a.KW / 2, a.H, a.W, HW, M, mb, me};

  f32x16 acc[Cfg::TM][Cfg::TN];
#pragma unroll
  for (int i = 0; i < Cfg::TM; ++i)
#pragma unroll
    for (int j = 0; j < Cfg::TN; ++j)
#pragma unroll
      for (int r = 0; r < 16; ++r) acc[i][j][r] = 0.f;

  gemm_mainloop<Cfg>(lds, (int)((me - mb + Cfg::BK - 1) / Cfg::BK), la, lb, acc);

#pragma unroll
  for (int nt = 0; nt < Cfg::TN; ++nt) {
    const int n = acc_col<Cfg>(nt);
    if (ci0 + n >= cpad) continue;
#pragma unroll
    for (int mt = 0; mt < Cfg::TM; ++mt)
#pragma unroll
      for (int r = 0; r < 16; ++r) {
        const int co = co0 + acc_row<Cfg>(mt, r);
        if (co < a.Cout) atomicAdd(a.dwpk + (int64_t)co * a.Ktot + kofs + n, acc[mt][nt][r]);
      }
  }
}

}

#include "wgrad_patch.inc"

namespace {
int g_wgrad_wide = 1;
__thread int t_wgrad_tile = 0;

struct WidePlan {
  int bm;
  int pairs, groups;
  int yw;
  int64_t chunk;
};

WidePlan wide_plan(int Cout, const int* srcC, int nsrc, int taps, int64_t M, int nseg, int64_t chunk128) {
  WidePlan p{};
  if (g_wgrad_wide == 0 || Cout <= 32) return p;
  for (int s = 0; s < nsrc; ++s) p.groups += taps * ceil_div(srcC[s], 128);
  p.pairs = p.groups / 2;
  if (p.pairs == 0) return p;
  const int bm = Cout >= 256 ? 256 : 128;
  const int yw = bm == 256 ? Cout / 256 : ceil_div(Cout, 128);
  const int64_t tiles = (int64_t)p.pairs * yw * nseg, s128 = (M + chunk128 - 1) / chunk128;
  int64_t want = 512 / tiles;
  if (want > s128) want = s128;
  if (tiles * want > 256) want = 256 * (tiles * want / 256) / tiles;
  if (want < 1) want = 1;
  int64_t chunk = (M + want - 1) / want;
  if (chunk < 256) chunk = 256;
  chunk = (chunk + 31) / 32 * 32;
  if (chunk > 32 * (WGRAD_WIDE_WORDS - 2) || chunk * 4 * 2048 >= 0x7fffffff) return p;
  if (g_wgrad_wide == 1) {
    if (tiles * ((M + chunk - 1) / chunk) < 192 || chunk < 512) return p;
  }
  p.bm = bm; p.yw = yw; p.chunk = chunk;
  return p;
}

template <class Cfg, bool MULTI, class A>
int launch_split(A m, int xt, int yt, int zs, int nseg, int bx0, int by0, int64_t chunk, int xcd, hipStream_t stream) {
  WgradArgs& a = [&]() -> WgradArgs& { if constexpr (MULTI) return m.a; else return m; }();
  a.kchunk = (int)chunk; a.bx0 = bx0; a.by0 = by0;
  a.xcd_xt = a.xcd_yt = a.xcd_groups = 0;
  if constexpr (MULTI) { m.zs = zs; m.nseg = nseg; }
  dim3 grid(xt, yt, zs * nseg);
  if (xcd == 3) {
    a.xcd_xt = xt * yt; a.xcd_yt = -xt; a.xcd_groups = zs * nseg;
    grid = dim3((unsigned)(ceil_div(a.xcd_groups, 8) * 8 * xt * yt), 1, 1);
  } else if (xcd) {
    a.xcd_xt = xt; a.xcd_yt = yt; a.xcd_groups = yt * zs * nseg;
    grid = dim3((unsigned)(ceil_div(a.xcd_groups, 8) * 8 * xt), 1, 1);
  }
  hipLaunchKernelGGL((conv_wgrad_split_kernel<Cfg, true, MULTI>), grid, dim3(Cfg::NT), 0, stream, m);
  return fs_launch_status();
}

template <bool MULTI, class A>
int launch_wide(const A& m, const WidePlan& p, int Cout, int64_t M, int nseg, int64_t chunk128, int xcd, hipStream_t stream) {
  const int zsw = (int)((M + p.chunk - 1) / p.chunk), zs = (int)((M + chunk128 - 1) / chunk128);
  int rc = p.bm == 256 ? launch_split<SWCfgW256, MULTI>(m, p.pairs, p.yw, zsw, nseg, 0, 0, p.chunk, xcd, stream)
                       : launch_split<SWCfgW128, MULTI>(m, p.pairs, p.yw, zsw, nseg, 0, 0, p.chunk, xcd, stream);
  if (rc) return rc;
  const int y128 = ceil_div(Cout, 128), ydone = p.bm == 256 ? 2 * p.yw : p.yw;
  if (ydone < y128) rc = launch_split<SWCfg128S, MULTI>(m, p.groups, y128 - ydone, zs, nseg, 0, ydone, chunk128, xcd, stream);
  if (rc) return rc;
  if (p.groups & 1) rc = launch_split<SWCfg128S, MULTI>(m, 1, ydone, zs, nseg, p.groups - 1, 0, chunk128, xcd, stream);
  t_wgrad_tile = p.bm << 16 | 256;
  return rc;
}
}

extern "C" int fsraft_set_wgrad_wide(int mode) {
  if (mode < 0 || mode > 2) return FS_ERR_ARG;
  g_wgrad_wide = mode;
  return FS_OK;
}
extern "C" int fsraft_conv_wgrad_last_tile(void) { return t_wgrad_tile; }

extern "C" int fsraft_conv_wgrad(const float* dy, int ldy, int Cout, const float* const* src, const int* srcC,
                                 const int* srcld, int nsrc, float* dwpk, float* dbias, int B, int H, int W, int KH,
                                 int KW, hipStream_t stream) {
  if (!dy || !src || !dwpk || nsrc < 1 || nsrc > 3 || ldy % 4 != 0) return FS_ERR_ARG;
  t_route[1] = 0; t_wgrad_tile = 0;
  WgradArgs a{};
  a.dy = dy; a.ldy = ldy; a.Cout = Cout;
  const bool small_m = Cout <= 32;
  const bool t64 = !small_m && knob.wgrad_tile == 3;
  const int bn = t64 ? 64 : 128, bm = small_m ? 32 : (t64 ? 64 : 128);
  if (!fill_srcs(a.src, src, srcC, srcld, nsrc)) return FS_ERR_ARG;
  int xt128 = 0;
  for (int s = 0; s < nsrc; ++s) xt128 += KH * KW * ceil_div(srcC[s], bn);
  a.nsrc = nsrc; a.dwpk = dwpk; a.Ktot = conv_ktot(srcC, nsrc, KH * KW);
  a.B = B; a.H = H; a.W = W; a.KH = KH; a.KW = KW;
  const int64_t M = (int64_t)B * H * W;
  if (knob.wgrad_patch && knob.wgrad_patch1 && knob.wgrad_split != 0 && KH == 3 && KW == 3 && Cout > 32 && M >= knob.wgrad_patch1) {
    WgradArgsM m{};
    m.a = a; m.a.dbias = dbias;
    m.nseg = 1;
    m.dys[0] = dy;
    for (int s = 0; s < nsrc; ++s) m.srcs[s][0] = src[s];
    const int rc = launch_wgrad_patch(m, stream);
    if (rc >= 0) return rc;
  }
  if (knob.wgrad_pack && knob.wgrad_split != 0 && knob.wgrad_buf && nsrc == 1 && srcC[0] <= 96 && KH * KW > 1 &&
      (int64_t)(32 * (WGRAD_PACK_WORDS - 2) + 2 * W + 2) * srcld[0] * 4 < 0x7fffffff) {
    const int cpad = ceil_div(srcC[0], 32) * 32;
    int tp = SWCfgPack::BN / cpad;
    if (tp > WGRAD_PACK_SLOTS) tp = WGRAD_PACK_SLOTS;
    const int xt = ceil_div(KH * KW, tp), yt = ceil_div(Cout, SWCfgPack::BM);
    const int64_t chunk = wgrad_chunk(knob.wgrad_blocks_pack, (int64_t)xt * yt, M, WGRAD_PACK_WORDS);
    a.kchunk = (int)chunk;
    a.dbias = dbias;
    dim3 grid(xt, yt, (unsigned)((M + chunk - 1) / chunk));
    if (knob.wgrad_xcd == 2) {
      a.xcd_xt = xt; a.xcd_yt = yt; a.xcd_groups = yt * (int)grid.z;
      grid = dim3((unsigned)(ceil_div(a.xcd_groups, 8) * 8 * xt), 1, 1);
    }
    t_route[1] = 6; t_wgrad_tile = SWCfgPack::BM << 16 | SWCfgPack::BN;
    hipLaunchKernelGGL((conv_wgrad_pack_kernel<SWCfgPack>), grid, dim3(SWCfgPack::NT), 0, stream, a);
    return fs_launch_status();
  }
  const int ytiles = ceil_div(Cout, bm);
  const int64_t chunk = wgrad_chunk(knob.wgrad_blocks, (int64_t)xt128 * ytiles, M, WGRAD_MASK_WORDS);
  a.kchunk = (int)chunk;
  const int zs = (int)((M + chunk - 1) / chunk);
  dim3 grid(xt128, ytiles, zs);
  a.dbias = dbias;
  const bool wbuf = knob.wgrad_buf && chunk <= 32 * (WGRAD_MASK_WORDS - 2) && (int64_t)chunk * 4 * 2048 < 0x7fffffff;
  if (!small_m && !t64 && knob.wgrad_split == 1) {
    t_route[1] = 4; t_wgrad_tile = 128 << 16 | 128;
    if (wbuf) hipLaunchKernelGGL((conv_wgrad_split_kernel<SWCfg128, true>), grid, dim3(256), 0, stream, a);
    else hipLaunchKernelGGL((conv_wgrad_split_kernel<SWCfg128>), grid, dim3(256), 0, stream, a);
    return fs_launch_status();
  }
  if (!small_m && !t64 && knob.wgrad_split == 2) {
    t_route[1] = 5;
    t_wgrad_tile = 128 << 16 | 128;
    if (wbuf) {
      const WidePlan p = wide_plan(Cout, srcC, nsrc, KH * KW, M, 1, chunk);
      if (p.bm) return launch_wide<false>(a, p, Cout, M, 1, chunk, 0, stream);
    }
    if (wbuf)hipLaunchKernelGGL((conv_wgrad_split_kernel<SWCfg128S, true>), grid, dim3(256), 0, stream, a);
    else hipLaunchKernelGGL((conv_wgrad_split_kernel<SWCfg128S>), grid, dim3(256), 0, stream, a);
    return fs_launch_status();
  }
  if (dbias) { const int rc = fsraft_col_sum(dy, ldy, M, Cout, dbias, 1.0f, stream); if (rc) return rc; }
  t_route[1] = small_m ? 1 : t64 ? 2 : 3;
  t_wgrad_tile = bm << 16 | bn;
  if (small_m) hipLaunchKernelGGL((conv_wgrad_kernel<WCfg32>), grid, dim3(256), 0, stream, a);
  else if (t64) hipLaunchKernelGGL((conv_wgrad_kernel<WCfg6464>), grid, dim3(256), 0, stream, a);
  else hipLaunchKernelGGL((conv_wgrad_kernel<WCfg128>), grid, dim3(256), 0, stream, a);
  return fs_launch_status();
}

extern "C" int fsraft_conv_wgrad_multi(const float* const* dy, int nseg, int ldy, int Cout, const float* const* src,
                                       const int* srcC, const int* srcld, int nsrc, float* dwpk, float* dbias, int B,
                                       int H, int W, int KH, int KW, hipStream_t stream) {
  if (!dy || !src || !dwpk || nseg < 1 || nsrc < 1 || nsrc > 3 || ldy % 4 != 0) return FS_ERR_ARG;
  t_route[1] = 0; t_wgrad_tile = 0;
  const int64_t M = (int64_t)B * H * W;
  const bool fast = knob.wgrad_multi && nseg > 1 && Cout > 32 && knob.wgrad_tile != 3 && knob.wgrad_split == 2 && knob.wgrad_buf;
  for (int base = 0; base < nseg; base += WGRAD_MAX_SEG) {
    const int n = nseg - base < WGRAD_MAX_SEG ? nseg - base : WGRAD_MAX_SEG;
    if (!fast || n == 1) {
      for (int i = 0; i < n; ++i) {
        const int rc = fsraft_conv_wgrad(dy[base + i], ldy, Cout, src + (size_t)(base + i) * nsrc, srcC, srcld, nsrc, dwpk,
                                         dbias, B, H, W, KH, KW, stream);
        if (rc) return rc;
      }
      continue;
    }
    WgradArgsM m{};
    WgradArgs& a = m.a;
    a.dy = dy[base]; a.ldy = ldy; a.Cout = Cout;
    if (!fill_srcs(a.src, src + (size_t)base * nsrc, srcC, srcld, nsrc)) return FS_ERR_ARG;
    int xt128 = 0;
    for (int s = 0; s < nsrc; ++s) xt128 += KH * KW * ceil_div(srcC[s], 128);
    for (int i = 0; i < n; ++i) {
      if (!dy[base + i]) return FS_ERR_ARG;
      m.dys[i] = dy[base + i];
      for (int s = 0; s < nsrc; ++s) {
        if (!src[(size_t)(base + i) * nsrc + s]) return FS_ERR_ARG;
        m.srcs[s][i] = src[(size_t)(base + i) * nsrc + s];
      }
    }
    a.nsrc = nsrc; a.dwpk = dwpk; a.Ktot = conv_ktot(srcC, nsrc, KH * KW);
    a.B = B; a.H = H; a.W = W; a.KH = KH; a.KW = KW; a.dbias = dbias;
    if (knob.wgrad_patch && KH * KW > 1) {
      m.nseg = n;
      const int rc = launch_wgrad_patch(m, stream);
      if (rc == 0) continue;
      if (rc > 0) return rc;
    }
    const int ytiles = ceil_div(Cout, 128);
    const int64_t chunk = wgrad_chunk(knob.wgrad_blocks_multi, (int64_t)xt128 * ytiles * n, M, WGRAD_MASK_WORDS);
    if ((int64_t)chunk * 4 * 2048 >= 0x7fffffff) return FS_ERR_ARG;
    if (!knob.wgrad_w8) {
      const WidePlan p = wide_plan(Cout, srcC, nsrc, KH * KW, M, n, chunk);
      if (p.bm) {
        t_route[1] = 8;
        const int rc = launch_wide<true>(m, p, Cout, M, n, chunk, knob.wgrad_xcd, stream);
        if (rc) return rc;
        continue;
      }
    }
    t_wgrad_tile = 128 << 16 | 128;
    a.kchunk = (int)chunk;
    m.zs = (int)((M + chunk - 1) / chunk);
    m.nseg = n;
    dim3 grid(xt128, ytiles, m.zs * n);
    if (knob.wgrad_xcd == 3) {
      m.a.xcd_xt = xt128 * ytiles; m.a.xcd_yt = -xt128; m.a.xcd_groups = m.zs * n;
      grid = dim3((unsigned)(ceil_div(m.a.xcd_groups, 8) * 8 * xt128 * ytiles), 1, 1);
    } else if (knob.wgrad_xcd) {
      m.a.xcd_xt = xt128; m.a.xcd_yt = ytiles; m.a.xcd_groups = ytiles * m.zs * n;
      grid = dim3((unsigned)(ceil_div(m.a.xcd_groups, 8) * 8 * xt128), 1, 1);
    }
    t_route[1] = knob.wgrad_w8 ? 9 : 8;
    if (knob.wgrad_w8) hipLaunchKernelGGL((conv_wgrad_split_kernel<SWCfg128W8, true, true>), grid, dim3(512), 0, stream, m);
    else hipLaunchKernelGGL((conv_wgrad_split_kernel<SWCfg128S, true, true>), grid, dim3(256), 0, stream, m);
    const int rc = fs_launch_status();
    if (rc) return rc;
  }
  return FS_OK;
}
```

flow_supervisor_amd/ops.py:

```python
import ctypes
import math
import os

import torch
import torch.optim.optimizer as _optimizer_module

from . import _lib as L


def _lib():
    return L.load()


def parameters_updated(params):
    ps = [p for p in params if isinstance(p, torch.Tensor)]
    if ps:
        torch._C._autograd._unsafe_set_version_counter(ps, [p._version + 1 for p in ps])


def _after_optimizer_step(opt, args, kwargs):
    parameters_updated([p for g in opt.param_groups if g.get("fused") for p in g["params"]])


_optimizer_module.register_optimizer_step_post_hook(_after_optimizer_step)
# ... 918 lines not shown
    L.check(_lib().fsraft_flow_to_nhwc(L.ptr(flow), bs, cs, ps, L.ptr(dst), dst.shape[-1], coff, B, H * W, L.stream()),
            "flow_to_nhwc")


def nhwc_to_flow(src, coff, dflow, accumulate):
    B, _, H, W = dflow.shape
    L.check(_lib().fsraft_nhwc_to_flow(L.ptr(src), src.shape[-1], coff, L.ptr(dflow), B, H * W, int(accumulate),
                                       L.stream()), "nhwc_to_flow")


def relu_bwd_(g, y, C):
    M = g.numel() // g.shape[-1]
    L.check(_lib().fsraft_relu_bwd(L.ptr(g), g.shape[-1], L.ptr(y), y.shape[-1], M, C, L.stream()), "relu_bwd")


def gru_bwd1(dhn, z, q, h, dzr, dq, dh, hid, dzr_sum=None, dq_sum=None, dhn2=None):
    M = dhn.numel() // hid
    L.check(_lib().fsraft_gru_bwd1(L.ptr(dhn), L.ptr(dhn2), L.ptr(z), L.ptr(q), L.ptr(h), L.ptr(dzr), dzr.shape[-1], L.ptr(dq),
                                   L.ptr(dh), L.ptr(dzr_sum), L.ptr(dq_sum), M, hid, L.stream()), "gru_bwd1")


def gru_bwd2(drh, r, h, dzr, dh, hid, dzr_sum=None):
    M = drh.numel() // hid
    L.check(_lib().fsraft_gru_bwd2(L.ptr(drh), L.ptr(r), L.ptr(h), L.ptr(dzr), dzr.shape[-1], L.ptr(dh), L.ptr(dzr_sum), M, hid,
                                   L.stream()), "gru_bwd2")


def col_sum_(x, C, out, scale=1.0):
    M = x.numel() // x.shape[-1]
    L.check(_lib().fsraft_col_sum(L.ptr(x), x.shape[-1], M, C, L.ptr(out), float(scale), L.stream()), "col_sum")


def sum_n_(tensors, out, accumulate=False):
    n = tensors[0].numel()
    for t in tensors:
        L.require_cuda_f32(t)
        if t.numel() != n or not t.is_contiguous():
            raise ValueError("sum_n_: contiguous tensors of one size")
    if out.numel() < n or not out.is_contiguous():
        raise ValueError("sum_n_: out too small / not contiguous")
    pp, keep = L.ptr_array(tensors)
    L.check(_lib().fsraft_sum_n(pp, len(tensors), L.ptr(out), n, int(accumulate), L.stream()), "sum_n")
    return out


def axpby_(x, y, a=1.0, b=1.0):
    L.check(_lib().fsraft_axpby(L.ptr(x), L.ptr(y), float(a), float(b), x.numel(), L.stream()), "axpby")


def conv_ktot(srcC, KH, KW):
    return _lib().fsraft_conv_ktot(L.int_array(srcC), len(srcC), KH, KW)


def pack_weight(w, srcC, mode):
    L.require_cuda_f32(w)
    w = w.contiguous()
    Cout, Cin, KH, KW = w.shape
    if mode % 10 == 0:
        rows, kt = Cout, conv_ktot(srcC, KH, KW)
    else:
        rows, kt = Cin, conv_ktot([Cout], KH, KW)
    wpk = torch.empty(rows, kt, device=w.device, dtype=torch.float32)
    L.check(_lib().fsraft_pack_conv_weight(L.ptr(w), L.ptr(wpk), Cout, Cin, KH, KW, L.int_array(srcC), len(srcC), mode,
                                           0, L.stream()), "pack_conv_weight")
    return wpk


class PackPlan:

    def __init__(self, device):
        self.device = device
        self.jobs = []
        self.total = 0
        self.keep = []

    def _job(self, ws, cin_full, kh, kw, srcC, srcOff, mode, flags=0, scale=1.0, accumulate=False):
        j = L.PackJob()
        for i, w in enumerate(ws):
            L.require_cuda_f32(w)
            assert w.is_contiguous()
            j.w[i] = w.data_ptr()
            j.rows[i] = w.shape[0]
        j.npiece = len(ws)
        j.cin_full, j.kh, j.kw = cin_full, kh, kw
        for i, (c, o) in enumerate(zip(srcC, srcOff)):
            j.srcC[i], j.srcOff[i] = c, o
        j.nsrc = len(srcC)
        j.mode, j.flags, j.scale, j.accumulate = mode, flags, scale, int(accumulate)
        self.keep.append(ws)
        return j

    def pack(self, ws, srcC, mode, srcOff=None, kh=None, kw=None, cin_full=None, frag=False, s2d=False):
        w0 = ws[0]
        cin_full = w0.shape[1] if cin_full is None else cin_full
        kh = (2 if s2d else w0.shape[2]) if kh is None else kh
        kw = (2 if s2d else w0.shape[3]) if kw is None else kw
        srcOff = [sum(srcC[:i]) for i in range(len(srcC))] if srcOff is None else srcOff
        cout = sum(w.shape[0] for w in ws)
        if mode % 10 == 0:
            rows, kt = cout, conv_ktot(srcC, kh, kw)
        else:
            rows, kt = sum(srcC), conv_ktot([cout], kh, kw)
        if frag:
            rows = (rows + 31) // 32 * 32
        j = self._job(ws, cin_full, kh, kw, srcC, srcOff, mode, (1 if frag else 0) | (2 if s2d else 0))
        self.jobs.append((j, self.total, (rows, kt)))
        self.total += (rows * kt + 63) // 64 * 64
        return len(self.jobs) - 1

    def bias(self, bs):
        j = self._job(bs, 1, 1, 1, [1], [0], 3)
        n = sum(b.shape[0] for b in bs)
        self.jobs.append((j, self.total, (n,)))
        self.total += (n + 63) // 64 * 64
        return len(self.jobs) - 1

    def run(self):
        buf = torch.empty(max(self.total, 1), device=self.device, dtype=torch.float32)
        arr = (L.PackJob * max(len(self.jobs), 1))()
        outs = []
        for i, (j, off, shape) in enumerate(self.jobs):
            n = 1
            for v in shape:
                n *= v
            t = buf[off:off + n].view(shape)
            j.wpk = t.data_ptr()
            arr[i] = j
            outs.append(t)
        if self.jobs:
            L.check(_lib().fsraft_pack_conv_weights(arr, len(self.jobs), L.stream()), "pack_conv_weights")
        self.keep = []
        return outs


def unpack_weight_grads(items, device):
    if not items:
        return
    arr = (L.PackJob * len(items))()
    plan = PackPlan(device)
    for i, (dwpk, gs, srcC, srcOff, cin_full, kh, kw, scale, s2d) in enumerate(items):
        j = plan._job(gs, cin_full, kh, kw, srcC, srcOff, 2, 2 if s2d else 0, scale)
        j.wpk = dwpk.data_ptr()
        arr[i] = j
    L.check(_lib().fsraft_pack_conv_weights(arr, len(items), L.stream()), "unpack_conv_weights")


def exact_mode():
    return _lib().fsraft_get_tuning(3) == 0


def set_arithmetic(split):
    global SPLIT_VOLUME_BWD
    L.check(_lib().fsraft_set_arithmetic(1 if split else 0), "set_arithmetic")
    SPLIT_VOLUME_BWD = bool(split)


def pack_pair(w, srcC, dgrad=False):
    m = 1 if dgrad else 0
    split = pack_weight(w, srcC, 10 + m)
    rows = w.shape[1] if dgrad else w.shape[0]
    return (pack_weight(w, srcC, m) if (exact_mode() or rows <= 32) else split), split


def fragment_order(wps):
    N, ktot = wps.shape
    kt, nb = ktot // 32, (N + 31) // 32
    w = wps.contiguous().view(torch.int32)
    if nb * 32 != N:
        w = torch.cat([w, w.new_zeros(nb * 32 - N, ktot)])
    w = w.view(nb, 32, kt, 2, 2, 2, 4).permute(2, 0, 3, 4, 5, 1, 6).contiguous()
    return w.view(torch.float32).view(kt, nb, 4, 64, 4)


def unpack_weight_grad(dwpk, shape, srcC, out=None, accumulate=False):
    Cout, Cin, KH, KW = shape
    if out is None:
        out = torch.empty(shape, device=dwpk.device, dtype=torch.float32)
        accumulate = False
    L.check(_lib().fsraft_pack_conv_weight(L.ptr(out), L.ptr(dwpk), Cout, Cin, KH, KW, L.int_array(srcC), len(srcC), 2,
                                           int(accumulate), L.stream()), "unpack_conv_weight")
    return out


class V:
    __slots__ = ("t", "off", "C", "ld")

    def __init__(self, t, C=None, off=0):
        self.t, self.off, self.ld = t, off, t.shape[-1]
        self.C = (t.shape[-1] - off) if C is None else C
        assert off % 4 == 0 and self.ld % 4 == 0, "channel slices must stay 16-byte aligned"

    @property
    def ptr(self):
        return self.t.data_ptr() + 4 * self.off


class Dst:
    __slots__ = ("t", "off", "bs", "ps", "cs", "n0", "acc", "mask")

    def __init__(self, t, off, bs, ps, cs, n0=0, acc=False):
        self.t, self.off, self.bs, self.ps, self.cs, self.n0, self.acc = t, off, bs, ps, cs, n0, acc
        self.mask = None

    def masked(self, v):
        self.mask = v
        return self

    @staticmethod
    def nhwc(buf, coff=0, n0=0, acc=False):
        B, H, W, ld = buf.shape
        return Dst(buf, coff, H * W * ld, ld, 1, n0, acc)

    @staticmethod
    def nchw(buf, n0=0, acc=False):
        B, C, H, W = buf.shape
        return Dst(buf, 0, C * H * W, 1, H * W, n0, acc)


_CONV_WS = {}
CONV_WS_FLOATS = 24 << 20
CONV_WS_MAX_PIXELS = 16384


def _conv_workspace(device, pixels):
    if pixels > CONV_WS_MAX_PIXELS:
        return None
    key = (torch.device(device).index or 0, torch.cuda.current_stream(device).cuda_stream)
    ws = _CONV_WS.get(key)
    if ws is None:
        ws = _CONV_WS.setdefault(key, torch.empty(CONV_WS_FLOATS, device=device, dtype=torch.float32))
    return ws


def conv_forward(srcs, wpk, bias, B, H, W, KH, KW, N, dsts, relu=False, alpha=1.0, epi=0, h=None, z=None,
                 aux1=None, aux2=None, hid=0, wpk_split=None, pre=None, wpk_frag=None, pad=None, stats=None):
    d = L.ConvDesc()
    for i, v in enumerate(srcs):
        d.src[i] = v.ptr; d.srcC[i] = v.C; d.srcld[i] = v.ld
    d.nsrc = len(srcs)
    d.wpk = wpk.data_ptr()
    d.wpk_split = wpk_split.data_ptr() if wpk_split is not None else None
    d.wpk_frag = wpk_frag.data_ptr() if wpk_frag is not None else None
    if pad is not None:
        d.pad_h1, d.pad_w1 = pad[0] + 1, pad[1] + 1
    d.bias = bias.data_ptr() if bias is not None else None
    d.B, d.H, d.W, d.KH, d.KW, d.N = B, H, W, KH, KW, N
    for i, ds in enumerate(dsts):
        d.dst[i] = ds.t.data_ptr() + 4 * ds.off
        d.dst_bs[i], d.dst_ps[i], d.dst_cs[i] = ds.bs, ds.ps, ds.cs
        d.dst_n0[i] = ds.n0; d.dst_acc[i] = int(ds.acc)
        if ds.mask is not None:
            d.rmask[i] = ds.mask.ptr; d.ldmask[i] = ds.mask.ld; d.maskc[i] = ds.mask.C
    d.ndst = len(dsts)
    d.relu = int(relu); d.alpha = float(alpha); d.epi = epi
    if h is not None:
        d.h = h.data_ptr(); d.ldh = h.shape[-1]
    if z is not None:
        d.z = z.data_ptr(); d.ldz = z.shape[-1]
    if aux1 is not None:
        d.aux1 = aux1.data_ptr(); d.ld1 = aux1.shape[-1]
    if aux2 is not None:
        d.aux2 = aux2.data_ptr(); d.ld2 = aux2.shape[-1]
    d.hid = hid
    if pre is not None:
        d.pre = pre.data_ptr(); d.ldpre = pre.shape[-1]
    ws = _conv_workspace(dsts[0].t.device, B * H * W)
    if ws is not None:
        d.ws = ws.data_ptr(); d.ws_floats = ws.numel()
    t = TIMER
    e0 = t.begin() if t else None
    carried = None
    if stats is not None:
        done = ctypes.c_int(0)
        L.check(_lib().fsraft_conv_forward_stats(ctypes.byref(d), L.ptr(stats[0]), L.ptr(stats[1]), stats.shape[1] // B, ctypes.byref(done),
                                                 L.stream()), "conv_forward_stats")
        carried = bool(done.value)
    else:
        L.check(_lib().fsraft_conv_forward(ctypes.byref(d), L.stream()), "conv_forward")
    if t:
        cin = sum(v.C for v in srcs)
        t.end("conv_igemm", e0, 2.0 * B * H * W * N * cin * KH * KW, 4.0 * B * H * W * (cin + N),
              tag=f"{B}x{H}x{W} {KH}x{KW} {'+'.join(str(v.C) for v in srcs)}->{N} epi{epi}{' relu' if relu else ''}{' masked' if any(ds.mask is not None for ds in dsts) else ''}")
    return carried


def conv_wgrad(dy, srcs, dwpk, B, H, W, KH, KW, dbias=None):
    arr = (ctypes.c_void_p * len(srcs))(*[v.ptr for v in srcs])
    pp = ctypes.cast(arr, L._PP)
    e0w = TIMER.begin() if TIMER else None
    L.check(_lib().fsraft_conv_wgrad(ctypes.c_void_p(dy.ptr), dy.ld, dy.C, pp, L.int_array([v.C for v in srcs]),
                                     L.int_array([v.ld for v in srcs]), len(srcs), L.ptr(dwpk), L.ptr(dbias), B, H, W,
                                     KH, KW, L.stream()), "conv_wgrad")
    if TIMER:
        cin = sum(v.C for v in srcs)
        TIMER.end("conv_wgrad", e0w, 2.0 * B * H * W * dy.C * cin * KH * KW, 4.0 * B * H * W * (cin + dy.C),
                  tag=f"{B}x{H}x{W} {KH}x{KW} {'+'.join(str(v.C) for v in srcs)}->{dy.C} x1")


def conv_wgrad_multi(dys, srcs, dwpk, B, H, W, KH, KW, dbias=None):
    n, nsrc = len(dys), len(srcs[0])
    dy0 = dys[0]
    a_dy = (ctypes.c_void_p * n)(*[v.ptr for v in dys])
    a_src = (ctypes.c_void_p * (n * nsrc))(*[v.ptr for sl in srcs for v in sl])
    e0w = TIMER.begin() if TIMER else None
    L.check(_lib().fsraft_conv_wgrad_multi(ctypes.cast(a_dy, L._PP), n, dy0.ld, dy0.C, ctypes.cast(a_src, L._PP),
                                           L.int_array([v.C for v in srcs[0]]), L.int_array([v.ld for v in srcs[0]]), nsrc,
                                           L.ptr(dwpk), L.ptr(dbias), B, H, W, KH, KW, L.stream()), "conv_wgrad_multi")
    if TIMER:
        cin = sum(v.C for v in srcs[0])
        TIMER.end("conv_wgrad", e0w, 2.0 * n * B * H * W * dy0.C * cin * KH * KW, 4.0 * n * B * H * W * (cin + dy0.C),
                  tag=f"{B}x{H}x{W} {KH}x{KW} {'+'.join(str(v.C) for v in srcs[0])}->{dy0.C} x{n}")


def stem_fwd(x, w, bias=None):
    L.require_cuda_f32(x, w)
    B, C, H, W = x.shape
    N = w.shape[0]
    if C != 3 or tuple(w.shape[1:]) != (3, 7, 7) or not x.is_contiguous():
        raise RuntimeError("stem_fwd: x [B,3,H,W] contiguous and w [N,3,7,7] expected")
    out = torch.empty(B, (H - 1) // 2 + 1, (W - 1) // 2 + 1, N, device=x.device, dtype=torch.float32)
    t = TIMER
    e0 = t.begin() if t else None
    L.check(_lib().fsraft_stem7x7s2_fwd(L.ptr(x), L.ptr(w.contiguous()), L.ptr(bias), L.ptr(out), B, H, W, N, L.stream()), "stem7x7s2_fwd")
    if t:
        t.end("stem", e0, 2.0 * out.numel() * 147, 4.0 * (x.numel() + out.numel()))
    return out


def stem_wgrad(x, dy):
    L.require_cuda_f32(x, dy)
    B, C, H, W = x.shape
    N = dy.shape[-1]
    if not (x.is_contiguous() and dy.is_contiguous()) or tuple(dy.shape[:3]) != (B, (H - 1) // 2 + 1, (W - 1) // 2 + 1):
        raise RuntimeError("stem_wgrad: contiguous x [B,3,H,W] and dy [B,Ho,Wo,N] expected")
    lib = _lib()
    scratch = torch.empty(lib.fsraft_stem_slots() * 64 * 192, device=x.device, dtype=torch.float32)
    dw = torch.empty(N, 3, 7, 7, device=x.device, dtype=torch.float32)
    t = TIMER
    e0 = t.begin() if t else None
    L.check(lib.fsraft_stem7x7s2_wgrad(L.ptr(x), L.ptr(dy), L.ptr(dw), L.ptr(scratch), B, H, W, N, L.stream()), "stem7x7s2_wgrad")
    if t:
        t.end("stem", e0, 2.0 * dy.numel() * 147, 4.0 * (x.numel() + dy.numel()))
    return dw


def conv_small_fwd(x, w_oihw, bias, out_nchw):
    B, N, H, W = out_nchw.shape
    t = TIMER
    e0 = t.begin() if t else None
# ... 149 lines not shown
```

include/fsraft.h:

```cpp
#ifndef FSRAFT_H
#define FSRAFT_H

#include <stdint.h>

#ifdef __cplusplus
extern "C" {
#endif

#ifndef __HIP_PLATFORM_AMD__
typedef struct ihipStream_t* hipStream_t;
#endif

#define FSRAFT_OK 0
#define FSRAFT_ERR_ARG 1
#define FSRAFT_ERR_LAUNCH 2

int fsraft_corr_build(const float* fmap1, const float* fmap2, float* const* levels, int num_levels,
                      int B, int C, int H, int W, hipStream_t stream);

int fsraft_corr_pool_pyramid(float* const* levels, int num_levels, int64_t rows, int H2, int W2, hipStream_t stream);
int fsraft_corr_pool_pyramid_same(float* const* levels, int num_levels, int64_t rows, int H2, int W2, hipStream_t stream);
int fsraft_corr_lookup_fwd_same(float* const* levels, int num_levels, const float* coords, int64_t coords_bs,
                                int64_t coords_cs, int64_t coords_ps, float* out, int nhwc_out, int B, int H, int W,
                                int radius, hipStream_t stream);
// ... 26 lines not shown

int fsraft_corr_lookup_fwd(float* const* levels, int num_levels, const float* coords, int64_t coords_bs,
                           int64_t coords_cs, int64_t coords_ps, float* out, int nhwc_out, int B, int H, int W,
                           int radius, hipStream_t stream);
int fsraft_corr_lookup_bwd(float* const* dlevels, int num_levels, const float* coords, int64_t coords_bs,
                           int64_t coords_cs, int64_t coords_ps, const float* dout, int nhwc_in, int B, int H, int W,
                           int radius, hipStream_t stream);
int fsraft_corr_lookup_dcoords(float* const* levels, int num_levels, const float* coords, int64_t coords_bs, int64_t coords_cs,
                               int64_t coords_ps, const float* dout, int nhwc_in, float* dcoords, int64_t dbs, int64_t dcs,
                               int64_t dps, int B, int H, int W, int radius, hipStream_t stream);

int fsraft_altcorr_fwd(const float* fmap1, const float* fmap2, const float* coords, float* corr, int B, int N, int H1,
                       int W1, int H2, int W2, int C, int radius, hipStream_t stream);
int fsraft_altcorr_bwd(const float* fmap1, const float* fmap2, const float* coords, const float* corr_grad,
                       float* fmap1_grad, float* fmap2_grad, int B, int N, int H1, int W1, int H2, int W2, int C,
                       int radius, hipStream_t stream);

int fsraft_altcorr_fused_fwd(const float* fmap1, const float* const* fmap2_levels, int num_levels, const float* coords,
                             int64_t coords_bs, int64_t coords_cs, int64_t coords_ps, int add_grid, float* out, int B, int H, int W,
                             int C, int radius, hipStream_t stream);
int fsraft_altcorr_fused_dcoords(const float* fmap1, const float* const* fmap2_levels, int num_levels, const float* coords,
                                 int64_t coords_bs, int64_t coords_cs, int64_t coords_ps, int add_grid, const float* dout,
                                 float* dcoords, int64_t dbs, int64_t dcs, int64_t dps, int B, int H, int W, int C, int radius,
                                 hipStream_t stream);

int fsraft_altcorr_mfma_fwd(const void* f1r, const void* const* f2r_levels, const float* fmap1, const float* const* fmap2_levels,
                            int num_levels, const float* coords, int64_t coords_bs, int64_t coords_cs, int64_t coords_ps,
                            int add_grid, float* out, int B, int H, int W, int C, int radius, hipStream_t stream);

int fsraft_upsample_fwd(const float* flow, int64_t flow_bs, int64_t flow_cs, int64_t flow_ps,
                        const float* mask_nhwc, float* up, int N, int H, int W, hipStream_t stream);
int fsraft_upsample_bwd(const float* flow, int64_t flow_bs, int64_t flow_cs, int64_t flow_ps,
                        const float* mask_nhwc, const float* dup, float* dmask_nhwc, float* dflow, float* scratch,
                        int N, int H, int W, hipStream_t stream);
int fsraft_upflow8_fwd(const float* flow, float* up, int N, int C, int H, int W, hipStream_t stream);
int fsraft_upflow8_bwd(const float* dup, float* dflow, int N, int C, int H, int W, hipStream_t stream);

typedef struct fsraft_conv_desc {
  const float* src[3]; int srcC[3]; int srcld[3]; int nsrc;
  const float* wpk; const float* bias;
  const float* wpk_split;
  int B, H, W, KH, KW, N;
  float* dst[3]; int64_t dst_bs[3]; int64_t dst_ps[3]; int64_t dst_cs[3];
  int dst_n0[3]; int dst_acc[3]; int ndst;
  int relu; float alpha;
  int epi;
  const float* h; int ldh; const float* z; int ldz;
  float* aux1; int ld1; float* aux2; int ld2; int hid;
  const float* pre; int ldpre;
  const float* rmask[3]; int ldmask[3]; int maskc[3];
  const float* wpk_frag;
  int pad_h1, pad_w1;
  float* ws; int64_t ws_floats;
} fsraft_conv_desc;

int fsraft_conv_ktot(const int* srcC, int nsrc, int KH, int KW);
int fsraft_conv_forward(const fsraft_conv_desc* d, hipStream_t stream);
int fsraft_conv_forward_stats(const fsraft_conv_desc* d, float* sum, float* sq, int slots, int* done, hipStream_t stream);
int fsraft_conv_wgrad(const float* dy, int ldy, int Cout, const float* const* src, const int* srcC,
                      const int* srcld, int nsrc, float* dwpk, float* dbias, int B, int H, int W, int KH, int KW,
                      hipStream_t stream);
int fsraft_conv_wgrad_multi(const float* const* dy, int nseg, int ldy, int Cout, const float* const* src,
                            const int* srcC, const int* srcld, int nsrc, float* dwpk, float* dbias, int B, int H, int W,
                            int KH, int KW, hipStream_t stream);
int fsraft_pack_conv_weight(float* w_oihw, float* wpk, int Cout, int Cin, int KH, int KW, const int* srcC,
                            int nsrc, int mode, int accumulate, hipStream_t stream);

typedef struct {
  float* w[3]; int rows[3]; int npiece;
  float* wpk;
  int cin_full, kh, kw;
  int srcC[3], srcOff[3], nsrc;
  int mode, flags;
  float scale; int accumulate;
} fsraft_pack_job;
int fsraft_pack_conv_weights(const fsraft_pack_job* jobs, int njobs, hipStream_t stream);

int fsraft_conv_small_fwd(const float* x, int ld, int C, const float* w_oihw, const float* bias, float* out, int64_t obs,
                          int64_t ocs, int64_t ops, int N, int B, int H, int W, int KH, int KW, hipStream_t stream);
int fsraft_conv_small_wgrad(const float* const* dy, const float* const* x, int nseg, int ldy, int ldx, int C, float* dwpk,
                            float* dbias, int N, int B, int H, int W, int KH, int KW, hipStream_t stream);
int fsraft_conv_small_dgrad(const float* dy, int ldy, const float* w_oihw, float* dx, int lddx, const float* relu_src, int ldm,
                            int C, int N, int B, int H, int W, int KH, int KW, hipStream_t stream);

int fsraft_conv_workspace(float* ws, int64_t floats);

int fsraft_set_arithmetic(int mode);
int fsraft_get_arithmetic(void);

int fsraft_gemm_f32(const float* A, int64_t lda, int64_t sA, const float* Bm, int64_t ldb, int64_t sB, float* C,
                    int64_t ldc, int64_t sC, int batch, int M, int N, int K, int trans_b, float alpha,
                    int accumulate, hipStream_t stream);

int fsraft_gemm_tn_split(const float* A, int64_t lda, int64_t sA, const float* Bm, int64_t ldb, int64_t sB, float* C,
                         int64_t ldc, int64_t sC, int batch, int M, int N, int K, float alpha, int accumulate,
                         hipStream_t stream);

int fsraft_to_records(const float* src, int64_t ld, void* dst, int64_t dst_ld, int64_t rows, int K, hipStream_t stream);
int fsraft_gemm_rec_nt(const void* A, int64_t lda, int64_t sA, const void* Bm, int64_t ldb, int64_t sB, float* C, int64_t ldc,
                       int64_t sC, int batch, int M, int N, int K, float alpha, int ksplit, int accumulate, hipStream_t stream);
int fsraft_gemm_rec_tn(const void* A, int64_t lda, int64_t sA, const void* Bm, int64_t ldb, int64_t sB, float* C, int64_t ldc,
                       int64_t sC, int batch, int M, int N, int K, float alpha, int ksplit, int accumulate, hipStream_t stream);

int fsraft_gemm_rec_nt_list(const void* A, int64_t lda, int64_t sA, const void* Bm, int64_t ldb, int64_t sB, float* C, int64_t ldc,
                            int64_t sC, int batch, int M, int N, int K, float alpha, int ksplit, int accumulate, const int* klist,
                            const int* kcount, int kl_stride, int kl_by_n, hipStream_t stream);
int fsraft_gemm_rec_tn_list(const void* A, int64_t lda, int64_t sA, const void* Bm, int64_t ldb, int64_t sB, float* C, int64_t ldc,
                            int64_t sC, int batch, int M, int N, int K, float alpha, int ksplit, int accumulate, const int* klist,
                            const int* kcount, int kl_stride, int kl_by_n, hipStream_t stream);
int fsraft_corr_bwd_ktiles(const float* const* coords, const int64_t* coords_str, int n, int num_levels, int B, int H, int W,
                           int radius, int add_grid, int64_t q0, int64_t nq, int* nt_list, int* nt_count, int nt_stride, unsigned* tn_bits,
                           int* tn_list, int* tn_count, int tn_stride, unsigned* wmask, hipStream_t stream);

int fsraft_softmax_rows(float* S, int64_t rows, int n, hipStream_t stream);
// ... 96 lines not shown
```

include/fsraft_tuning.h:

```cpp
#ifndef FSRAFT_TUNING_H
#define FSRAFT_TUNING_H

#ifdef __cplusplus
extern "C" {
#endif

enum fsraft_tuning_key {
  FSRAFT_KEY_CONV_TILE = 0,
  FSRAFT_KEY_WGRAD_TILE = 1,
  FSRAFT_KEY_WGRAD_BLOCKS = 2,
  FSRAFT_KEY_CONV_ARITH = 3,
  FSRAFT_KEY_WGRAD_ARITH = 4,
  FSRAFT_KEY_CONV_BUF = 5,
  FSRAFT_KEY_XCD_SWIZZLE = 7,
  FSRAFT_KEY_WGRAD_BUF = 8,
  FSRAFT_KEY_CONV_N256 = 9,
  FSRAFT_KEY_WGRAD_MULTI = 10,
  FSRAFT_KEY_WGRAD_BLOCKS_MULTI = 11,
  FSRAFT_KEY_CONV_UNIFORM = 12,
  FSRAFT_KEY_CONV_W8 = 13,
  FSRAFT_KEY_CONV_W8_MIN = 14,
  FSRAFT_KEY_WGRAD_W8 = 15,
  FSRAFT_KEY_WGRAD_PACK = 16,
  FSRAFT_KEY_WGRAD_BLOCKS_PACK = 17,
  FSRAFT_KEY_CONV_N64 = 18,
  FSRAFT_KEY_CONV_N64_MIN_M = 19,
  FSRAFT_KEY_CONV_HALO = 20,
  FSRAFT_KEY_CONV_HALO_MIN_M = 21,
  FSRAFT_KEY_WGRAD_XCD = 22,
  FSRAFT_KEY_CONV_PATCH = 26,
  FSRAFT_KEY_WGRAD_PATCH = 27,
  FSRAFT_KEY_CONV_PATCH64 = 28,
  FSRAFT_KEY_WGRAD_PATCH1 = 29,
  FSRAFT_KEY_CONV_PATCH_MIN_M = 31,
  FSRAFT_KEY_CONV_KSPLIT = 32
};
int fsraft_set_tuning(int key, int value);
int fsraft_get_tuning(int key);
int fsraft_conv_last_route(int which);
int fsraft_set_wgrad_wide(int mode);
int fsraft_conv_wgrad_last_tile(void);
int fsraft_set_build_split(int on);
int fsraft_set_build_kernel(int which);
int fsraft_set_lookup_policy(int aux);
int fsraft_set_ktile_exact(int levels);
int fsraft_set_upsample_kernel(int v4);
int fsraft_set_dvol_box(int on);
int fsraft_set_dvol_policy(int policy);
int fsraft_set_gemm_split(int on);
int fsraft_set_lookup_qb(int qb);
int fsraft_set_norm_blocks(int target_workgroups);
int fsraft_set_rec_mfma16(int on);
int fsraft_set_alt_tile(int on);

#ifdef __cplusplus
}
#endif
#endif
```

Baseline: 115.4 image-pairs/s.

## Skip structurally-zero K-tiles in space-to-depth stride-2 conv forward, dgrad and wgrad

A stride-2 3x3 conv rewritten as a 2x2 conv over space-to-depth input has zero weight slots: only 9 of the 16 tap/subpixel combinations are live. This adds per-tap chunk masks so the implicit-GEMM k-table holds only live 32-channel K tiles. It uses a compact weight pack for forward, a masked wgrad, and column-tiled dgrad with fewer taps. This cuts roughly 7/16 of the MACs for these layers, but excludes the patch and halo fast paths and adds fallbacks to the dense path.

```diff
diff --git a/flow_supervisor_amd/_lib.py b/flow_supervisor_amd/_lib.py
--- a/flow_supervisor_amd/_lib.py
+++ b/flow_supervisor_amd/_lib.py
@@ -27,6 +27,7 @@
         ("rmask", c_void_p * 3), ("ldmask", c_int * 3), ("maskc", c_int * 3),
         ("wpk_frag", c_void_p), ("pad_h1", c_int), ("pad_w1", c_int),
         ("ws", c_void_p), ("ws_floats", c_int64),
+        ("tap_chunks", ctypes.c_uint32 * 16), ("wpk_ld", c_int),
     ]
 
 
@@ -57,9 +58,11 @@
     "fsraft_upflow8_fwd": [c_void_p, c_void_p, c_int, c_int, c_int, c_int, _S],
     "fsraft_upflow8_bwd": [c_void_p, c_void_p, c_int, c_int, c_int, c_int, _S],
     "fsraft_conv_ktot": [_IP, c_int, c_int, c_int],
+    "fsraft_conv_ktot_s2d": [c_int, POINTER(ctypes.c_uint32)],
     "fsraft_conv_forward": [POINTER(ConvDesc), _S],
     "fsraft_conv_forward_stats": [POINTER(ConvDesc), c_void_p, c_void_p, c_int, POINTER(c_int), _S],
     "fsraft_conv_wgrad": [c_void_p, c_int, c_int, _PP, _IP, _IP, c_int, c_void_p, c_void_p, c_int, c_int, c_int, c_int, c_int, _S],
+    "fsraft_conv_wgrad_masked": [c_void_p, c_int, c_int, c_void_p, c_int, c_int, POINTER(ctypes.c_uint32), c_void_p, c_int, c_int, c_int, c_int, c_int, _S],
     "fsraft_conv_wgrad_multi": [_PP, c_int, c_int, c_int, _PP, _IP, _IP, c_int, c_void_p, c_void_p, c_int, c_int, c_int, c_int, c_int, _S],
     "fsraft_conv_small_fwd": [c_void_p, c_int, c_int, c_void_p, c_void_p, c_void_p, c_int64, c_int64, c_int64, c_int, c_int, c_int, c_int, c_int, c_int, _S],
     "fsraft_conv_small_wgrad": [_PP, _PP, c_int, c_int, c_int, c_int, c_void_p, c_void_p, c_int, c_int, c_int, c_int, c_int, c_int, _S],
@@ -123,6 +126,9 @@
     "fsraft_conv_last_route": [c_int],
     "fsraft_set_wgrad_wide": [c_int],
     "fsraft_conv_wgrad_last_tile": [],
+    "fsraft_conv_last_ktiles": [c_int],
+    "fsraft_set_s2d_compact": [c_int],
+    "fsraft_s2d_compact_use": [c_int, c_int64, c_int, c_int],
     "fsraft_space_to_depth2": [c_void_p, c_void_p, c_int, c_int, c_int, c_int, c_int, _S],
     "fsraft_forward_interpolate": [c_void_p, c_void_p, c_int, c_int, _S],
     "fsraft_flow_metrics_scratch_bytes": [c_int, c_int, c_int],
diff --git a/flow_supervisor_amd/core/extractor.py b/flow_supervisor_amd/core/extractor.py
--- a/flow_supervisor_amd/core/extractor.py
+++ b/flow_supervisor_amd/core/extractor.py
@@ -257,18 +257,21 @@
             b = plan.pack([w3], [4 * C], 11, cin_full=C, s2d=True)
             a0 = plan.pack([w3], [4 * C], 0, cin_full=C, s2d=True) if (exact or N <= 32) else a
             b0 = plan.pack([w3], [4 * C], 1, cin_full=C, s2d=True) if (exact or 4 * C <= 32) else b
+            live = None if exact else ops.conv_ktot_s2d(C)
+            ac = plan.pack([w3], [4 * C], 10, cin_full=C, s2d=True, compact=True) if live is not None else None
             Ns, Cs = ws.shape[:2]
             c_ = plan.pack([ws], [Cs], 10)
             d_ = plan.pack([ws], [Cs], 11)
             c0 = plan.pack([ws], [Cs], 0) if (exact or Ns <= 32) else c_
             d0 = plan.pack([ws], [Cs], 1) if (exact or Cs <= 32) else d_
-            hs.append(((a0, a, b0, b), (c0, c_, d0, d_)))
+            hs.append(((a0, a, b0, b, ac), (c0, c_, d0, d_), live))
         out = plan.run()
         for (kind, m, key), h in zip(todo, hs):
             if kind == "conv":
                 m.__dict__["_fs_packs"] = (key,) + tuple(None if i is None else out[i] for i in h)
             else:
-                m.__dict__["_fs_pair_packs"] = (key, tuple(out[i] for i in h[0]), tuple(out[i] for i in h[1]))
+                m.__dict__["_fs_pair_packs"] = (key, tuple(None if i is None else out[i] for i in h[0]), tuple(out[i] for i in h[1]),
+                                                h[2])
 
 
 def _weight_packs(conv):
@@ -443,8 +446,12 @@
         N, Ns = w3.shape[0], wsc.shape[0]
         y1 = torch.empty(B, h, w, N, device=x.device, dtype=torch.float32)
         ys = torch.empty(B, h, w, Ns, device=x.device, dtype=torch.float32)
-        p, q = packs[1], packs[2]
-        ops.conv_forward([ops.V(xs, 4 * C)], p[0], None, B, h, w, 2, 2, N, [ops.Dst.nhwc(y1)], wpk_split=p[1])
+        p, q, live = packs[1], packs[2], packs[3]
+        if live is not None and ops.s2d_compact_use(0, B * h * w, C, N):
+            ops.conv_forward([ops.V(xs, 4 * C)], p[4], None, B, h, w, 2, 2, N, [ops.Dst.nhwc(y1)], wpk_split=p[4],
+                             tap_chunks=live[1], dense=(p[0], p[1]))
+        else:
+            ops.conv_forward([ops.V(xs, 4 * C)], p[0], None, B, h, w, 2, 2, N, [ops.Dst.nhwc(y1)], wpk_split=p[1])
         ops.conv_forward([ops.V(xs, C, 0)], q[0], None, B, h, w, 1, 1, Ns, [ops.Dst.nhwc(ys)], wpk_split=q[1])
         ctx.save_for_backward(xs, w3, wsc)
         ctx.packs = packs
@@ -462,15 +469,25 @@
         dx = dw3 = dwsc = None
         if ctx.needs_input_grad[0]:
             dxs = torch.empty(B, h, w, C4, device=xs.device, dtype=torch.float32)
-            ops.conv_forward([g1v], p[2], None, B, h, w, 2, 2, C4, [ops.Dst.nhwc(dxs)], wpk_split=p[3], pad=(0, 0))
+            if ctx.packs[3] is not None and N % 32 == 0 and ops.s2d_compact_use(1, B * h * w, C, N):
+                for n0, nw, taps in ops.s2d_dgrad_tiles(C):
+                    ops.conv_forward([g1v], p[3][n0:], None, B, h, w, 2, 2, nw, [ops.Dst.nhwc(dxs, n0)], wpk_split=p[3][n0:], pad=(0, 0),
+                                     tap_chunks=[(1 << (N // 32)) - 1] * taps, wpk_ld=p[3].shape[1], dense=(p[2][n0:], p[3][n0:]))
+            else:
+                ops.conv_forward([g1v], p[2], None, B, h, w, 2, 2, C4, [ops.Dst.nhwc(dxs)], wpk_split=p[3], pad=(0, 0))
             ops.conv_forward([gsv], q[2], None, B, h, w, 1, 1, C, [ops.Dst.nhwc(dxs, 0, 0, True)], wpk_split=q[3])
             dx = (dxs if ctx.pre else ops.space_to_depth2(dxs, inverse=True)).permute(0, 3, 1, 2)
         items = []
         if ctx.needs_input_grad[1]:
-            dwpk = ops.zeros(N, ops.conv_ktot([C4], 2, 2), device=xs.device)
-            ops.conv_wgrad(g1v, [ops.V(xs, C4)], dwpk, B, h, w, 2, 2)
+            live, done = ctx.packs[3], False
+            if live is not None and ops.s2d_compact_use(2, B * h * w, C, N):
+                dwpk = ops.zeros(N, live[0], device=xs.device)
+                done = ops.conv_wgrad_masked(g1v, ops.V(xs, C4), live[1], dwpk, B, h, w, 2, 2)
+            if not done:
+                dwpk = ops.zeros(N, ops.conv_ktot([C4], 2, 2), device=xs.device)
+                ops.conv_wgrad(g1v, [ops.V(xs, C4)], dwpk, B, h, w, 2, 2)
             dw3 = torch.empty(N, C, 3, 3, device=xs.device, dtype=torch.float32)
-            items.append((dwpk, [dw3], [C4], [0], C, 2, 2, 1.0, True))
+            items.append((dwpk, [dw3], [C4], [0], C, 2, 2, 1.0, "compact" if done else True))
         if ctx.needs_input_grad[2]:
             dwpk = ops.zeros(Ns, ops.conv_ktot([C], 1, 1), device=xs.device)
             ops.conv_wgrad(gsv, [ops.V(xs, C, 0)], dwpk, B, h, w, 1, 1)
diff --git a/flow_supervisor_amd/csrc/conv_common.hpp b/flow_supervisor_amd/csrc/conv_common.hpp
--- a/flow_supervisor_amd/csrc/conv_common.hpp
+++ b/flow_supervisor_amd/csrc/conv_common.hpp
@@ -37,6 +37,7 @@
 };
 __attribute__((visibility("hidden"))) extern ConvKnobs knob;
 __attribute__((visibility("hidden"))) extern __thread int t_route[2];
+__attribute__((visibility("hidden"))) extern __thread int t_ktiles[2];
 
 namespace {
 struct Src { const float* p; int C; int ld; };
@@ -45,6 +46,7 @@
 struct ConvArgs {
   Src src[3]; int nsrc;
   const float* wpk; int Ktot;
+  int wld;
   const float* bias;
   int B, H, W, KH, KW, N;
   int PH, PW;
@@ -129,6 +131,23 @@
   return k;
 }
 
+__host__ __device__ inline bool s2d_live(int tap, int sp) { return ((tap >> 1) | (sp >> 1)) && ((tap & 1) | (sp & 1)); }
+inline int s2d_ktot(int C, unsigned* mask) {
+  if (C < 32 || C % 32 != 0 || C > 256) return -1;
+  const int cpc = C / 32;
+  for (int t = 0; t < 4 && mask; ++t) {
+    mask[t] = 0;
+    for (int sp = 0; sp < 4; ++sp)
+      if (s2d_live(t, sp)) mask[t] |= ((1u << cpc) - 1u) << (sp * cpc);
+  }
+  return 9 * C;
+}
+inline int masked_ktiles(const unsigned* mask, int taps, int cpt) {
+  int n = 0;
+  for (int t = 0; t < taps; ++t) n += __builtin_popcount(mask[t] & (cpt >= 32 ? ~0u : (1u << cpt) - 1u));
+  return n;
+}
+
 template <class F>
 void with_epi(int epi, F&& f) {
   if (epi == EPI_PLAIN) f(std::integral_constant<int, EPI_PLAIN>{});
diff --git a/flow_supervisor_amd/csrc/conv_igemm.hip b/flow_supervisor_amd/csrc/conv_igemm.hip
--- a/flow_supervisor_amd/csrc/conv_igemm.hip
+++ b/flow_supervisor_amd/csrc/conv_igemm.hip
@@ -522,12 +522,12 @@
       tapmask[j] = mask; pofs[j] = m < M ? m : 0;
     }
     BufWeightLoader<Cfg> lb;
-    lb.base = uni_ptr(reinterpret_cast<const char*>(a.wpk) + (int64_t)n0 * a.Ktot * 4 + (int64_t)kt0 * 128);
+    lb.base = uni_ptr(reinterpret_cast<const char*>(a.wpk) + (int64_t)n0 * a.wld * 4 + (int64_t)kt0 * 128);
     lb.nbytes = 0x7fffffffu;
 #pragma unroll
     for (int j = 0; j < BufWeightLoader<Cfg>::NCH; ++j) {
       const int e = threadIdx.x + Cfg::NT * j;
-      lb.voff[j] = (e >> 3) < a.N - n0 ? (unsigned)((e >> 3) * a.Ktot * 4 + (e & 7) * 16) : FS_OOB;
+      lb.voff[j] = (e >> 3) < a.N - n0 ? (unsigned)((e >> 3) * a.wld * 4 + (e & 7) * 16) : FS_OOB;
     }
     if constexpr (BUF >= 2) {
       BufConvALoaderU<Cfg> la;
@@ -753,6 +753,9 @@
   return fs_launch_status();
 }
 
+thread_local const unsigned* t_kmask = nullptr;
+inline bool ktile_live(int tap, int c) { return !t_kmask || (t_kmask[tap] >> c & 1u); }
+
 bool build_ktab(const ConvArgs& a, ConvArgsT& t) {
   const int taps = a.KH * a.KW, KT = a.Ktot / 32;
   const int64_t M = (int64_t)a.B * a.H * a.W;
@@ -761,16 +764,19 @@
   for (int s = 0; s < a.nsrc; ++s) {
     const int C = a.src[s].C, ld = a.src[s].ld, cpt = (C + 31) / 32;
     if (M * ld * 4 >= (int64_t)FS_OOB) return false;
-    for (int i = 0; i < taps * cpt; ++i, ++kt) {
+    for (int i = 0; i < taps * cpt; ++i) {
         const int tap = i / cpt, c = i % cpt;
+        if (!ktile_live(tap, c)) continue;
+        if (kt >= KT) return false;
         const int64_t soff = ((int64_t)((tap / a.KW) * a.W + tap % a.KW) * ld + c * 32) * 4;
         if (soff % 16 != 0 || soff / 16 > 0xffff) return false;
         const int crem = C - c * 32 < 32 ? C - c * 32 : 32;
-        t.ktab[kt] = (unsigned)(soff / 16) | (unsigned)tap << 16 | (unsigned)s << 20 | (unsigned)crem << 22;
+        t.ktab[kt++] = (unsigned)(soff / 16) | (unsigned)tap << 16 | (unsigned)s << 20 | (unsigned)crem << 22;
       }
   }
   if (kt != KT) return false;
   t.a = a;
+  t_ktiles[0] = kt;
   return true;
 }
 
@@ -790,16 +796,20 @@
     const int C = a.src[s].C, cpt = (C + 31) / 32;
     const int64_t delta = (a.src[s].p - lo) * 4;
     for (int tap = 0; tap < taps; ++tap)
-      for (int c = 0; c < cpt; ++c, ++kt) {
+      for (int c = 0; c < cpt; ++c) {
+        if (!ktile_live(tap, c)) continue;
+        if (kt >= KT) return false;
         const int64_t soff = delta + ((int64_t)((tap / a.KW) * a.W + tap % a.KW) * ld + c * 32) * 4;
         if (soff + M * ld * 4 + 256 >= (int64_t)FS_OOB) return false;
         const int crem = C - c * 32 < 32 ? C - c * 32 : 32;
         t.ktab[2 * kt] = (unsigned)soff;
         t.ktab[2 * kt + 1] = (unsigned)tap | (unsigned)crem << 4;
+        ++kt;
       }
   }
   if (kt != KT) return false;
   t.a = a; t.ubase = base; t.uld = ld;
+  t_ktiles[0] = kt;
   return true;
 }
 
@@ -943,10 +953,12 @@
     with_epi(epi, [&](auto e) { hipLaunchKernelGGL((conv_igemm_split_kernel<Cfg, decltype(e)::value, 1>), grid, dim3(Cfg::NT), 0, s, t); });
     return fs_launch_status();
   }
+  if (t_kmask) return -1;
   if constexpr (Cfg::NT != 256) {
     return -1;
   } else {
   t_route[0] = route_split<Cfg>();
+  t_ktiles[0] = a.Ktot / 32;
   with_epi(epi, [&](auto e) { hipLaunchKernelGGL((conv_igemm_split_kernel<Cfg, decltype(e)::value>), grid, dim3(256), 0, s, a); });
   return fs_launch_status();
   }
@@ -974,7 +986,9 @@
 int launch_conv(const ConvArgs& a, int epi, hipStream_t s) {
   const int M = a.B * a.H * a.W;
   dim3 grid(ceil_div(a.N, Cfg::BN), ceil_div(M, Cfg::BM));
+  if (t_kmask) return -1;
   t_route[0] = route_gemm<Cfg>();
+  t_ktiles[0] = a.Ktot / 32;
   with_epi(epi, [&](auto e) { hipLaunchKernelGGL((conv_igemm_kernel<Cfg, decltype(e)::value>), grid, dim3(256), 0, s, a); });
   return fs_launch_status();
 }
@@ -997,8 +1011,51 @@
 }
 }
 
+namespace {
+int g_s2d_compact = 1;
+int conv_forward_routes(const fsraft_conv_desc* d, int ktot, int wld, hipStream_t stream);
+}
+
+extern "C" int fsraft_conv_ktot_s2d(int C, unsigned* tap_chunks) { return s2d_ktot(C, tap_chunks); }
+extern "C" int fsraft_set_s2d_compact(int mode) {
+  if (mode < 0 || mode > 2) return FS_ERR_ARG;
+  g_s2d_compact = mode;
+  return FS_OK;
+}
+extern "C" int fsraft_s2d_compact_use(int dir, int64_t M, int C, int N) {
+  if (g_s2d_compact == 0 || dir < 0 || dir > 2 || s2d_ktot(C, nullptr) < 0 || M < 1 || N <= 32) return 0;
+  if (knob.conv_split != 1 || knob.wgrad_split != 2 || !knob.wgrad_buf) return 0;
+  if (dir == 1 && N % 32 != 0) return 0;
+  if (g_s2d_compact == 2) return 1;
+  return dir != 1 && C >= 64 && C <= 96 && M >= 16384;
+}
+
 extern "C" int fsraft_conv_forward(const fsraft_conv_desc* d, hipStream_t stream) {
   if (!d || d->nsrc < 1 || d->nsrc > 3 || d->ndst < 1 || d->ndst > 3 || !d->wpk || d->N < 1) return FS_ERR_ARG;
+  t_route[0] = 0; t_ktiles[0] = 0;
+  const int taps = d->KH * d->KW;
+  bool masked = false;
+  for (int t = 0; t < 16; ++t) masked |= d->tap_chunks[t] != 0;
+  if (!masked) {
+    const int ktot = conv_ktot(d->srcC, d->nsrc, taps);
+    if (d->wpk_ld && d->wpk_ld != ktot) return FS_ERR_ARG;
+    return conv_forward_routes(d, ktot, ktot, stream);
+  }
+  if (d->nsrc != 1 || taps < 1 || taps > 15 || d->srcC[0] % 32 != 0 || d->srcC[0] > 1024) return FS_ERR_ARG;
+  const int cpt = d->srcC[0] / 32;
+  for (int t = 0; t < 16; ++t)
+    if ((t >= taps && d->tap_chunks[t]) || (cpt < 32 && d->tap_chunks[t] >> cpt)) return FS_ERR_ARG;
+  const int kt = masked_ktiles(d->tap_chunks, taps, cpt);
+  if (d->wpk_ld && (d->wpk_ld < kt * 32 || d->wpk_ld % 32 != 0)) return FS_ERR_ARG;
+  t_kmask = d->tap_chunks;
+  const int rc = conv_forward_routes(d, kt * 32, d->wpk_ld ? d->wpk_ld : kt * 32, stream);
+  t_kmask = nullptr;
+  if (rc < 0) { t_route[0] = 0; t_ktiles[0] = 0; return FS_ERR_ARG; }
+  return rc;
+}
+
+namespace {
+int conv_forward_routes(const fsraft_conv_desc* d, int ktot, int wld, hipStream_t stream) {
   const bool want_stats = t_stat.sum != nullptr && d->epi == EPI_PLAIN && d->ndst == 1 && !d->relu && d->alpha == 1.0f && !d->dst_acc[0] &&
                           !d->rmask[0] && !d->bias && d->dst_n0[0] == 0 && d->N % 4 == 0;
   if (d->ws && (((uintptr_t)d->ws & 15) || d->ws_floats < 0)) return FS_ERR_ARG;
@@ -1009,7 +1066,7 @@
   if (!fill_srcs(a.src, d->src, d->srcC, d->srcld, d->nsrc)) return FS_ERR_ARG;
   for (int s = 0; s < d->nsrc; ++s) if (d->srcC[s] < 1) return FS_ERR_ARG;
   a.nsrc = d->nsrc;
-  a.wpk = d->wpk; a.Ktot = conv_ktot(d->srcC, d->nsrc, d->KH * d->KW); a.bias = d->bias;
+  a.wpk = d->wpk; a.Ktot = ktot; a.wld = wld; a.bias = d->bias;
   a.B = d->B; a.H = d->H; a.W = d->W; a.KH = d->KH; a.KW = d->KW; a.N = d->N;
   a.PH = d->pad_h1 ? d->pad_h1 - 1 : d->KH / 2; a.PW = d->pad_w1 ? d->pad_w1 - 1 : d->KW / 2;
   if (a.PH < 0 || a.PH >= d->KH || a.PW < 0 || a.PW >= d->KW) return FS_ERR_ARG;
@@ -1032,7 +1089,7 @@
   if (d->epi == EPI_ZR && (!d->h || !d->aux1 || !d->aux2 || d->hid * 2 != d->N)) return FS_ERR_ARG;
   if (d->epi == EPI_Q && (!d->h || !d->z || !d->aux1)) return FS_ERR_ARG;
   if (d->epi != EPI_PLAIN && d->epi != EPI_ZR && d->epi != EPI_Q) return FS_ERR_ARG;
-  if (knob.conv_patch && knob.conv_patch64 && knob.conv_split == 1 && d->wpk_split && d->epi == EPI_PLAIN && d->KH == 3 && d->KW == 3 &&
+  if (knob.conv_patch && !t_kmask && knob.conv_patch64 && knob.conv_split == 1 && d->wpk_split && d->epi == EPI_PLAIN && d->KH == 3 && d->KW == 3 &&
       d->N > 32 && d->N <= 64 && (int64_t)d->B * d->H * d->W >= knob.conv_patch_min_m) {
     ConvArgs p = a;
     p.wpk = d->wpk_split;
@@ -1040,7 +1097,7 @@
     const int rc = launch_conv_patch(p, d->epi, stream);
     if (rc >= 0) { t_stat.done = want_stats; return rc; }
   }
-  if (knob.conv_halo && knob.conv_split == 1 && d->wpk_frag && d->epi == EPI_PLAIN && d->nsrc == 1 && d->KH == 3 && d->KW == 3 &&
+  if (knob.conv_halo && !t_kmask && knob.conv_split == 1 && d->wpk_frag && d->epi == EPI_PLAIN && d->nsrc == 1 && d->KH == 3 && d->KW == 3 &&
       a.PH == 1 && a.PW == 1 &&
       d->srcC[0] % 4 == 0 && d->srcC[0] > 32 && d->srcC[0] <= 64 && d->N <= 128 && d->N > 32 && d->ndst == 1 &&
       d->dst_cs[0] == 1 && d->dst_n0[0] == 0 && !(d->dst_acc[0] && d->relu) && !a.rmask[0] && d->alpha == 1.0f &&
@@ -1058,7 +1115,7 @@
   if (knob.conv_split && d->wpk_split && d->N > 32) {
     a.wpk = d->wpk_split;
     const bool narrow = knob.conv_buf != 0 || (int64_t)ceil_div(d->N, 128) * ceil_div(M, 128) < 400;
-    if (knob.conv_patch && knob.conv_split == 1 && d->KH * d->KW > 1 && d->N > 64 && M >= knob.conv_patch_min_m) {
+    if (knob.conv_patch && !t_kmask && knob.conv_split == 1 && d->KH * d->KW > 1 && d->N > 64 && M >= knob.conv_patch_min_m) {
       ConvArgs p = a;
       attach_stats(p, want_stats);
       const int rc = launch_conv_patch(p, d->epi, stream);
@@ -1091,6 +1148,7 @@
   if ((int64_t)ceil_div(d->N, 128) * ceil_div(M, 128) < 512) return launch_conv<CfgM64>(a, d->epi, stream);
   return launch_conv<Cfg128>(a, d->epi, stream);
 }
+}
 
 extern "C" int fsraft_conv_forward_stats(const fsraft_conv_desc* d, float* sum, float* sq, int slots, int* done, hipStream_t stream) {
   if (!sum || !sq || slots < 1 || !done) return FS_ERR_ARG;
diff --git a/flow_supervisor_amd/csrc/conv_pack.hip b/flow_supervisor_amd/csrc/conv_pack.hip
--- a/flow_supervisor_amd/csrc/conv_pack.hip
+++ b/flow_supervisor_amd/csrc/conv_pack.hip
@@ -107,8 +107,10 @@
   int cin = 0;
   for (int s = 0; s < j.nsrc; ++s) cin += j.srcC[s];
   const int m = j.mode % 10;
+  const bool compact = (j.flags & 4) != 0;
   int Ktot, rows;
   if (m == 1) { Ktot = taps * ((cout + 31) / 32 * 32); rows = cin; }
+  else if (compact) { Ktot = 9 * j.cin_full; rows = cout; }
   else { Ktot = 0; for (int s = 0; s < j.nsrc; ++s) Ktot += taps * ((j.srcC[s] + 31) / 32 * 32); rows = cout; }
   const int rows_out = (j.flags & 1) ? (rows + 31) / 32 * 32 : rows;
   const int64_t total = (int64_t)rows_out * Ktot;
@@ -128,15 +130,28 @@
       pack_store(j, Ktot, rows, n, k, v);
     } else {
       const int k0 = k;
-      int s = 0;
+      int s = 0, t, c;
+      bool ok;
+      if (compact) {
+        const int C = j.cin_full;
+        int slot = k / C, sp = 0;
+        for (t = 0; t < 4; ++t) {
+          for (sp = 0; sp < 4; ++sp)
+            if (s2d_live(t, sp) && slot-- == 0) break;
+          if (sp < 4) break;
+        }
+        c = sp * C + k % C;
+        ok = n < rows;
+      } else {
       for (; s < j.nsrc; ++s) {
         const int span = taps * ((j.srcC[s] + 31) / 32 * 32);
         if (k < span) break;
         k -= span;
       }
       const int cpad = (j.srcC[s] + 31) / 32 * 32;
-      const int t = k / cpad, c = k % cpad;
-      const bool ok = c < j.srcC[s] && n < rows;
+      t = k / cpad; c = k % cpad;
+      ok = c < j.srcC[s] && n < rows;
+      }
       float* q = ok ? pack_elem(j, n, s, c, t) : nullptr;
       if (m == 0) pack_store(j, Ktot, rows, n, k0, q ? *q : 0.f);
       else if (q) *q = j.accumulate ? *q + j.scale * j.wpk[e] : j.scale * j.wpk[e];
@@ -156,8 +171,9 @@
     if (m == 3) continue;
     if (j.nsrc < 1 || j.nsrc > 3 || j.kh < 1 || j.kw < 1 || j.cin_full < 1) return FS_ERR_ARG;
     if ((j.flags & 1) && m < 10) return FS_ERR_ARG;
-    if ((j.flags & 2) && (j.kh != 2 || j.kw != 2 || j.nsrc != 1 || j.srcC[0] != 4 * j.cin_full || j.srcOff[0] != 0)) return FS_ERR_ARG;
-    if (!(j.flags & 2)) for (int s = 0; s < j.nsrc; ++s) if (j.srcC[s] < 1 || j.srcOff[s] < 0 || j.srcOff[s] + j.srcC[s] > j.cin_full) return FS_ERR_ARG;
+    if ((j.flags & 4) && (m % 10 == 1 || (j.flags & 1) || s2d_ktot(j.cin_full, nullptr) < 0)) return FS_ERR_ARG;
+    if ((j.flags & 6) && (j.kh != 2 || j.kw != 2 || j.nsrc != 1 || j.srcC[0] != 4 * j.cin_full || j.srcOff[0] != 0)) return FS_ERR_ARG;
+    if (!(j.flags & 6)) for (int s = 0; s < j.nsrc; ++s) if (j.srcC[s] < 1 || j.srcOff[s] < 0 || j.srcOff[s] + j.srcC[s] > j.cin_full) return FS_ERR_ARG;
   }
   for (int i0 = 0; i0 < njobs; i0 += PACK_JOBS) {
     PackJobs tab{};
@@ -165,6 +181,7 @@
     int64_t most = 0;
     for (int i = 0; i < n; ++i) {
       tab.j[i] = jobs[i0 + i];
+      if (tab.j[i].flags & 4) tab.j[i].flags |= 2;
       const fsraft_pack_job& j = tab.j[i];
       int64_t cout = 0, cin = 0;
       for (int p = 0; p < j.npiece; ++p) cout += j.rows[p];
diff --git a/flow_supervisor_amd/csrc/conv_tuning.hip b/flow_supervisor_amd/csrc/conv_tuning.hip
--- a/flow_supervisor_amd/csrc/conv_tuning.hip
+++ b/flow_supervisor_amd/csrc/conv_tuning.hip
@@ -3,6 +3,7 @@
 
 ConvKnobs knob;
 __thread int t_route[2] = {0, 0};
+__thread int t_ktiles[2] = {0, 0};
 
 namespace {
 const struct { int key; int ConvKnobs::*member; } KNOB_TABLE[] = {
@@ -58,6 +59,9 @@
 extern "C" int fsraft_conv_last_route(int which) {
   return which == 0 || which == 1 ? t_route[which] : -1;
 }
+extern "C" int fsraft_conv_last_ktiles(int which) {
+  return which == 0 || which == 1 ? t_ktiles[which] : -1;
+}
 
 extern "C" int fsraft_set_arithmetic(int mode) {
   if (mode != 0 && mode != 1) return FS_ERR_ARG;
diff --git a/flow_supervisor_amd/csrc/conv_wgrad.hip b/flow_supervisor_amd/csrc/conv_wgrad.hip
--- a/flow_supervisor_amd/csrc/conv_wgrad.hip
+++ b/flow_supervisor_amd/csrc/conv_wgrad.hip
@@ -2,6 +2,7 @@
 
 namespace {
 
+constexpr int WGRAD_MAX_GRP = 32;
 struct WgradArgs {
   const float* dy; int ldy; int Cout;
   Src src[3]; int nsrc;
@@ -11,6 +12,8 @@
   float* dbias;
   int xcd_xt, xcd_yt, xcd_groups;
   int bx0, by0;
+  int ngrp;
+  unsigned grp[2 * WGRAD_MAX_GRP];
 };
 
 constexpr int WGRAD_MAX_SEG = 16;
@@ -157,9 +160,15 @@
   __device__ __forceinline__ int elem(int c) const { return e0 + 8 * (Cfg::BN / 4) * c; }
 };
 
-struct XGroup { int s, tap, ci0, kofs, cpad; };
+struct XGroup { int s, tap, ci0, kofs, lim; };
 template <int GW>
 __device__ __forceinline__ XGroup wgrad_xgroup(const WgradArgs& a, int t, int taps) {
+  if (a.ngrp > 0) {
+    const auto* g = (const unsigned __attribute__((address_space(4)))*)(
+        (const char __attribute__((address_space(4)))*)__builtin_amdgcn_kernarg_segment_ptr() + offsetof(WgradArgs, grp));
+    const unsigned g0 = g[2 * t], g1 = g[2 * t + 1];
+    return XGroup{0, (int)(g0 & 255u), (int)(g0 >> 8), (int)(g1 & 0xffffu), (int)(g1 >> 16)};
+  }
   int s = 0, kofs = 0;
   for (;; ++s) {
     const int ct = (a.src[s].C + GW - 1) / GW;
@@ -170,7 +179,7 @@
   const int C = s == 0 ? a.src[0].C : s == 1 ? a.src[1].C : a.src[2].C;
   const int ct = (C + GW - 1) / GW, cpad = ((C + 31) / 32) * 32;
   const int tap = t / ct, ci0 = (t % ct) * GW;
-  return XGroup{s, tap, ci0, kofs + tap * cpad + ci0, cpad};
+  return XGroup{s, tap, ci0, kofs + tap * cpad + ci0, cpad - ci0};
 }
 
 template <class Cfg, bool BUF = false, bool MULTI = false>
@@ -214,7 +223,7 @@
   const int64_t me = mb + a.kchunk < M ? mb + a.kchunk : M;
   if (mb >= M) return;
   const int coleft = ((a.Cout + 3) / 4) * 4 - co0;
-  const int cleft = ((sc.C + 3) / 4) * 4 - ci0;
+  const int cleft = min(((sc.C + 3) / 4) * 4 - ci0, gl.lim);
   const int dyy = tap / a.KW - a.KH / 2, dxx = tap % a.KW - a.KW / 2;
   const int KT = (int)((me - mb + 31) / 32);
   f32x16 acc[Cfg::TM][Cfg::TN];
@@ -291,7 +300,7 @@
 #pragma unroll
   for (int nt = 0; nt < Cfg::TN; ++nt) {
     const int n = acc_col<Cfg>(nt) & (GW - 1);
-    if (go.ci0 + n >= go.cpad) continue;
+    if (n >= go.lim) continue;
 #pragma unroll
     for (int mt = 0; mt < Cfg::TM; ++mt)
 #pragma unroll
@@ -495,10 +504,11 @@
   int64_t chunk;
 };
 
-WidePlan wide_plan(int Cout, const int* srcC, int nsrc, int taps, int64_t M, int nseg, int64_t chunk128) {
+WidePlan wide_plan(int Cout, const int* srcC, int nsrc, int taps, int64_t M, int nseg, int64_t chunk128, int listed = 0) {
   WidePlan p{};
   if (g_wgrad_wide == 0 || Cout <= 32) return p;
   for (int s = 0; s < nsrc; ++s) p.groups += taps * ceil_div(srcC[s], 128);
+  if (listed > 0) p.groups = listed;
   p.pairs = p.groups / 2;
   if (p.pairs == 0) return p;
   const int bm = Cout >= 256 ? 256 : 128;
@@ -559,11 +569,34 @@
 }
 extern "C" int fsraft_conv_wgrad_last_tile(void) { return t_wgrad_tile; }
 
+namespace {
+int conv_wgrad_routes(const float* dy, int ldy, int Cout, const float* const* src, const int* srcC, const int* srcld, int nsrc,
+                      const unsigned* mask, float* dwpk, float* dbias, int B, int H, int W, int KH, int KW, hipStream_t stream);
+}
+
 extern "C" int fsraft_conv_wgrad(const float* dy, int ldy, int Cout, const float* const* src, const int* srcC,
                                  const int* srcld, int nsrc, float* dwpk, float* dbias, int B, int H, int W, int KH,
                                  int KW, hipStream_t stream) {
+  return conv_wgrad_routes(dy, ldy, Cout, src, srcC, srcld, nsrc, nullptr, dwpk, dbias, B, H, W, KH, KW, stream);
+}
+
+extern "C" int fsraft_conv_wgrad_masked(const float* dy, int ldy, int Cout, const float* src, int srcC, int srcld,
+                                        const unsigned* tap_chunks, float* dwpk, int B, int H, int W, int KH, int KW,
+                                        hipStream_t stream) {
+  if (!tap_chunks) return conv_wgrad_routes(dy, ldy, Cout, &src, &srcC, &srcld, 1, nullptr, dwpk, nullptr, B, H, W, KH, KW, stream);
+  const int taps = KH * KW, cpt = srcC / 32;
+  t_route[1] = 0; t_wgrad_tile = 0; t_ktiles[1] = 0;
+  if (taps < 1 || taps > 15 || srcC < 32 || srcC % 32 != 0 || cpt > 32) return FS_ERR_ARG;
+  for (int t = 0; t < taps; ++t) if (cpt < 32 && tap_chunks[t] >> cpt) return FS_ERR_ARG;
+  if (masked_ktiles(tap_chunks, taps, cpt) < 1) return FS_ERR_ARG;
+  return conv_wgrad_routes(dy, ldy, Cout, &src, &srcC, &srcld, 1, tap_chunks, dwpk, nullptr, B, H, W, KH, KW, stream);
+}
+
+namespace {
+int conv_wgrad_routes(const float* dy, int ldy, int Cout, const float* const* src, const int* srcC, const int* srcld, int nsrc,
+                      const unsigned* mask, float* dwpk, float* dbias, int B, int H, int W, int KH, int KW, hipStream_t stream) {
   if (!dy || !src || !dwpk || nsrc < 1 || nsrc > 3 || ldy % 4 != 0) return FS_ERR_ARG;
-  t_route[1] = 0; t_wgrad_tile = 0;
+  t_route[1] = 0; t_wgrad_tile = 0; t_ktiles[1] = 0;
   WgradArgs a{};
   a.dy = dy; a.ldy = ldy; a.Cout = Cout;
   const bool small_m = Cout <= 32;
@@ -575,7 +608,24 @@
   a.nsrc = nsrc; a.dwpk = dwpk; a.Ktot = conv_ktot(srcC, nsrc, KH * KW);
   a.B = B; a.H = H; a.W = W; a.KH = KH; a.KW = KW;
   const int64_t M = (int64_t)B * H * W;
-  if (knob.wgrad_patch && knob.wgrad_patch1 && knob.wgrad_split != 0 && KH == 3 && KW == 3 && Cout > 32 && M >= knob.wgrad_patch1) {
+  if (mask) {
+    if (small_m || t64 || knob.wgrad_split != 2) return FS_ERR_ARG;
+    const int cpt = srcC[0] / 32;
+    int kt = 0;
+    for (int t = 0; t < KH * KW; ++t)
+      for (int c = 0; c < cpt;) {
+        if (!(mask[t] >> c & 1u)) { ++c; continue; }
+        int w = 0;
+        while (c + w < cpt && w < 4 && (mask[t] >> (c + w) & 1u)) ++w;
+        if (a.ngrp == WGRAD_MAX_GRP || kt * 32 > 0xffff) return FS_ERR_ARG;
+        a.grp[2 * a.ngrp] = (unsigned)t | (unsigned)(c * 32) << 8;
+        a.grp[2 * a.ngrp + 1] = (unsigned)(kt * 32) | (unsigned)(w * 32) << 16;
+        ++a.ngrp; kt += w; c += w;
+      }
+    xt128 = a.ngrp;
+    a.Ktot = kt * 32;
+  }
+  if (!mask && knob.wgrad_patch && knob.wgrad_patch1 && knob.wgrad_split != 0 && KH == 3 && KW == 3 && Cout > 32 && M >= knob.wgrad_patch1) {
     WgradArgsM m{};
     m.a = a; m.a.dbias = dbias;
     m.nseg = 1;
@@ -584,7 +634,7 @@
     const int rc = launch_wgrad_patch(m, stream);
     if (rc >= 0) return rc;
   }
-  if (knob.wgrad_pack && knob.wgrad_split != 0 && knob.wgrad_buf && nsrc == 1 && srcC[0] <= 96 && KH * KW > 1 &&
+  if (!mask && knob.wgrad_pack && knob.wgrad_split != 0 && knob.wgrad_buf && nsrc == 1 && srcC[0] <= 96 && KH * KW > 1 &&
       (int64_t)(32 * (WGRAD_PACK_WORDS - 2) + 2 * W + 2) * srcld[0] * 4 < 0x7fffffff) {
     const int cpad = ceil_div(srcC[0], 32) * 32;
     int tp = SWCfgPack::BN / cpad;
@@ -609,6 +659,8 @@
   dim3 grid(xt128, ytiles, zs);
   a.dbias = dbias;
   const bool wbuf = knob.wgrad_buf && chunk <= 32 * (WGRAD_MASK_WORDS - 2) && (int64_t)chunk * 4 * 2048 < 0x7fffffff;
+  if (mask && !wbuf) return FS_ERR_ARG;
+  if (!small_m && !t64 && knob.wgrad_split != 0) t_ktiles[1] = a.Ktot / 32;
   if (!small_m && !t64 && knob.wgrad_split == 1) {
     t_route[1] = 4; t_wgrad_tile = 128 << 16 | 128;
     if (wbuf) hipLaunchKernelGGL((conv_wgrad_split_kernel<SWCfg128, true>), grid, dim3(256), 0, stream, a);
@@ -619,7 +671,7 @@
     t_route[1] = 5;
     t_wgrad_tile = 128 << 16 | 128;
     if (wbuf) {
-      const WidePlan p = wide_plan(Cout, srcC, nsrc, KH * KW, M, 1, chunk);
+      const WidePlan p = wide_plan(Cout, srcC, nsrc, KH * KW, M, 1, chunk, a.ngrp);
       if (p.bm) return launch_wide<false>(a, p, Cout, M, 1, chunk, 0, stream);
     }
     if (wbuf)hipLaunchKernelGGL((conv_wgrad_split_kernel<SWCfg128S, true>), grid, dim3(256), 0, stream, a);
@@ -633,6 +685,7 @@
   else if (t64) hipLaunchKernelGGL((conv_wgrad_kernel<WCfg6464>), grid, dim3(256), 0, stream, a);
   else hipLaunchKernelGGL((conv_wgrad_kernel<WCfg128>), grid, dim3(256), 0, stream, a);
   return fs_launch_status();
+}
 }
 
 extern "C" int fsraft_conv_wgrad_multi(const float* const* dy, int nseg, int ldy, int Cout, const float* const* src,
@@ -668,12 +721,14 @@
     }
     a.nsrc = nsrc; a.dwpk = dwpk; a.Ktot = conv_ktot(srcC, nsrc, KH * KW);
     a.B = B; a.H = H; a.W = W; a.KH = KH; a.KW = KW; a.dbias = dbias;
+    t_ktiles[1] = 0;
     if (knob.wgrad_patch && KH * KW > 1) {
       m.nseg = n;
       const int rc = launch_wgrad_patch(m, stream);
       if (rc == 0) continue;
       if (rc > 0) return rc;
     }
+    t_ktiles[1] = a.Ktot / 32;
     const int ytiles = ceil_div(Cout, 128);
     const int64_t chunk = wgrad_chunk(knob.wgrad_blocks_multi, (int64_t)xt128 * ytiles * n, M, WGRAD_MASK_WORDS);
     if ((int64_t)chunk * 4 * 2048 >= 0x7fffffff) return FS_ERR_ARG;
diff --git a/flow_supervisor_amd/ops.py b/flow_supervisor_amd/ops.py
--- a/flow_supervisor_amd/ops.py
+++ b/flow_supervisor_amd/ops.py
@@ -994,6 +994,34 @@
     return _lib().fsraft_conv_ktot(L.int_array(srcC), len(srcC), KH, KW)
 
 
+def s2d_live_slots():
+    ax = {(0, 1), (1, 0), (1, 1)}
+    return [(t, sp) for t in range(4) for sp in range(4) if (t >> 1, sp >> 1) in ax and (t & 1, sp & 1) in ax]
+
+
+def conv_ktot_s2d(C):
+    m = (ctypes.c_uint32 * 4)()
+    k = _lib().fsraft_conv_ktot_s2d(int(C), m)
+    return None if k < 0 else (k, tuple(m))
+
+
+def s2d_compact_use(direction, M, C, N):
+    return bool(_lib().fsraft_s2d_compact_use(direction, M, C, N))
+
+
+def s2d_dgrad_tiles(C):
+    live, tiles = s2d_live_slots(), []
+    for n0 in range(0, 4 * C, 128):
+        n1 = min(n0 + 128, 4 * C)
+        sps = range(n0 // C, (n1 - 1) // C + 1)
+        taps = max(3 - t for t, sp in live if sp in sps) + 1
+        if tiles and tiles[-1][2] == taps:
+            tiles[-1] = (tiles[-1][0], tiles[-1][1] + n1 - n0, taps)
+        else:
+            tiles.append((n0, n1 - n0, taps))
+    return tiles
+
+
 def pack_weight(w, srcC, mode):
     L.require_cuda_f32(w)
     w = w.contiguous()
@@ -1032,7 +1060,7 @@
         self.keep.append(ws)
         return j
 
-    def pack(self, ws, srcC, mode, srcOff=None, kh=None, kw=None, cin_full=None, frag=False, s2d=False):
+    def pack(self, ws, srcC, mode, srcOff=None, kh=None, kw=None, cin_full=None, frag=False, s2d=False, compact=False):
         w0 = ws[0]
         cin_full = w0.shape[1] if cin_full is None else cin_full
         kh = (2 if s2d else w0.shape[2]) if kh is None else kh
@@ -1045,7 +1073,10 @@
             rows, kt = sum(srcC), conv_ktot([cout], kh, kw)
         if frag:
             rows = (rows + 31) // 32 * 32
-        j = self._job(ws, cin_full, kh, kw, srcC, srcOff, mode, (1 if frag else 0) | (2 if s2d else 0))
+        if compact:
+            assert s2d and mode % 10 == 0 and not frag
+            kt = conv_ktot_s2d(cin_full)[0]
+        j = self._job(ws, cin_full, kh, kw, srcC, srcOff, mode, (1 if frag else 0) | (2 if s2d else 0) | (4 if compact else 0))
         self.jobs.append((j, self.total, (rows, kt)))
         self.total += (rows * kt + 63) // 64 * 64
         return len(self.jobs) - 1
@@ -1081,7 +1112,7 @@
     arr = (L.PackJob * len(items))()
     plan = PackPlan(device)
     for i, (dwpk, gs, srcC, srcOff, cin_full, kh, kw, scale, s2d) in enumerate(items):
-        j = plan._job(gs, cin_full, kh, kw, srcC, srcOff, 2, 2 if s2d else 0, scale)
+        j = plan._job(gs, cin_full, kh, kw, srcC, srcOff, 2, 6 if s2d == "compact" else 2 if s2d else 0, scale)
         j.wpk = dwpk.data_ptr()
         arr[i] = j
     L.check(_lib().fsraft_pack_conv_weights(arr, len(items), L.stream()), "unpack_conv_weights")
@@ -1175,7 +1206,8 @@
 
 
 def conv_forward(srcs, wpk, bias, B, H, W, KH, KW, N, dsts, relu=False, alpha=1.0, epi=0, h=None, z=None,
-                 aux1=None, aux2=None, hid=0, wpk_split=None, pre=None, wpk_frag=None, pad=None, stats=None):
+                 aux1=None, aux2=None, hid=0, wpk_split=None, pre=None, wpk_frag=None, pad=None, stats=None, tap_chunks=None,
+                 dense=None, wpk_ld=0):
     d = L.ConvDesc()
     for i, v in enumerate(srcs):
         d.src[i] = v.ptr; d.srcC[i] = v.C; d.srcld[i] = v.ld
@@ -1212,7 +1244,24 @@
     t = TIMER
     e0 = t.begin() if t else None
     carried = None
-    if stats is not None:
+    live = None
+    if tap_chunks is not None:
+        assert stats is None and len(srcs) == 1
+        for i, m in enumerate(tap_chunks):
+            d.tap_chunks[i] = m
+        d.wpk_ld = wpk_ld
+        live = sum(bin(m).count("1") for m in tap_chunks)
+        rc = _lib().fsraft_conv_forward(ctypes.byref(d), L.stream())
+        if rc == 1 and dense is not None:
+            for i in range(16):
+                d.tap_chunks[i] = 0
+            d.wpk_ld = 0
+            d.wpk = dense[0].data_ptr()
+            d.wpk_split = dense[1].data_ptr() if dense[1] is not None else None
+            live = None
+            rc = _lib().fsraft_conv_forward(ctypes.byref(d), L.stream())
+        L.check(rc, "conv_forward")
+    elif stats is not None:
         done = ctypes.c_int(0)
         L.check(_lib().fsraft_conv_forward_stats(ctypes.byref(d), L.ptr(stats[0]), L.ptr(stats[1]), stats.shape[1] // B, ctypes.byref(done),
                                                  L.stream()), "conv_forward_stats")
@@ -1221,8 +1270,9 @@
         L.check(_lib().fsraft_conv_forward(ctypes.byref(d), L.stream()), "conv_forward")
     if t:
         cin = sum(v.C for v in srcs)
-        t.end("conv_igemm", e0, 2.0 * B * H * W * N * cin * KH * KW, 4.0 * B * H * W * (cin + N),
-              tag=f"{B}x{H}x{W} {KH}x{KW} {'+'.join(str(v.C) for v in srcs)}->{N} epi{epi}{' relu' if relu else ''}{' masked' if any(ds.mask is not None for ds in dsts) else ''}")
+        kdim = cin * KH * KW if live is None else 32 * live
+        t.end("conv_igemm", e0, 2.0 * B * H * W * N * kdim, 4.0 * B * H * W * (cin + N),
+              tag=f"{B}x{H}x{W} {KH}x{KW} {'+'.join(str(v.C) for v in srcs)}->{N} epi{epi}{' relu' if relu else ''}{' masked' if any(ds.mask is not None for ds in dsts) else ''}{' live' if live is not None else ''}")
     return carried
 
 
@@ -1237,6 +1287,21 @@
         cin = sum(v.C for v in srcs)
         TIMER.end("conv_wgrad", e0w, 2.0 * B * H * W * dy.C * cin * KH * KW, 4.0 * B * H * W * (cin + dy.C),
                   tag=f"{B}x{H}x{W} {KH}x{KW} {'+'.join(str(v.C) for v in srcs)}->{dy.C} x1")
+
+
+def conv_wgrad_masked(dy, src, tap_chunks, dwpk, B, H, W, KH, KW):
+    e0w = TIMER.begin() if TIMER else None
+    m = (ctypes.c_uint32 * len(tap_chunks))(*tap_chunks)
+    rc = _lib().fsraft_conv_wgrad_masked(ctypes.c_void_p(dy.ptr), dy.ld, dy.C, ctypes.c_void_p(src.ptr), src.C, src.ld, m,
+                                         L.ptr(dwpk), B, H, W, KH, KW, L.stream())
+    if rc == 1:
+        return False
+    L.check(rc, "conv_wgrad_masked")
+    if TIMER:
+        live = sum(bin(v).count("1") for v in tap_chunks)
+        TIMER.end("conv_wgrad", e0w, 2.0 * B * H * W * dy.C * 32 * live, 4.0 * B * H * W * (src.C + dy.C),
+                  tag=f"{B}x{H}x{W} {KH}x{KW} {src.C}->{dy.C} x1 live")
+    return True
 
 
 def conv_wgrad_multi(dys, srcs, dwpk, B, H, W, KH, KW, dbias=None):
diff --git a/include/fsraft.h b/include/fsraft.h
--- a/include/fsraft.h
+++ b/include/fsraft.h
@@ -102,14 +102,19 @@
   const float* wpk_frag;
   int pad_h1, pad_w1;
   float* ws; int64_t ws_floats;
+  unsigned tap_chunks[16];
+  int wpk_ld;
 } fsraft_conv_desc;
 
 int fsraft_conv_ktot(const int* srcC, int nsrc, int KH, int KW);
+int fsraft_conv_ktot_s2d(int C, unsigned* tap_chunks);
 int fsraft_conv_forward(const fsraft_conv_desc* d, hipStream_t stream);
 int fsraft_conv_forward_stats(const fsraft_conv_desc* d, float* sum, float* sq, int slots, int* done, hipStream_t stream);
 int fsraft_conv_wgrad(const float* dy, int ldy, int Cout, const float* const* src, const int* srcC,
                       const int* srcld, int nsrc, float* dwpk, float* dbias, int B, int H, int W, int KH, int KW,
                       hipStream_t stream);
+int fsraft_conv_wgrad_masked(const float* dy, int ldy, int Cout, const float* src, int srcC, int srcld, const unsigned* tap_chunks,
+                             float* dwpk, int B, int H, int W, int KH, int KW, hipStream_t stream);
 int fsraft_conv_wgrad_multi(const float* const* dy, int nseg, int ldy, int Cout, const float* const* src,
                             const int* srcC, const int* srcld, int nsrc, float* dwpk, float* dbias, int B, int H, int W,
                             int KH, int KW, hipStream_t stream);
diff --git a/include/fsraft_tuning.h b/include/fsraft_tuning.h
--- a/include/fsraft_tuning.h
+++ b/include/fsraft_tuning.h
@@ -40,6 +40,9 @@
 int fsraft_conv_last_route(int which);
 int fsraft_set_wgrad_wide(int mode);
 int fsraft_conv_wgrad_last_tile(void);
+int fsraft_conv_last_ktiles(int which);
+int fsraft_set_s2d_compact(int mode);
+int fsraft_s2d_compact_use(int dir, int64_t M, int C, int N);
 int fsraft_set_build_split(int on);
 int fsraft_set_build_kernel(int which);
 int fsraft_set_lookup_policy(int aux);
```

After: 116.3 image-pairs/s (median of 6 runs). Within noise of the previous version (+0.7%).
